# zyddnys/manga-image-translator

Measured on AMD Instinct MI355X. Metric: pages/sec end-to-end (detect+OCR+inpaint), 2048x1456, higher is better.
Workload: dtype f32

## Files before the change

include/mit_hip.h:

```cpp
#ifndef MIT_HIP_H
#define MIT_HIP_H

#include <stdint.h>

#ifdef __cplusplus
extern "C" {
#endif

#define MIT_ABI_VERSION 20
#define MIT_MAX_TAPS 64

enum MitAct {
    MIT_ACT_NONE = 0,
    MIT_ACT_RELU = 1,
    MIT_ACT_LEAKY = 2,
    MIT_ACT_SILU = 3,
    MIT_ACT_SIGMOID = 4,
    MIT_ACT_GELU = 5
};
#define MIT_ACT_POST_FIRST 0x100

enum MitPad {
    MIT_PAD_ZERO = 0,
    MIT_PAD_REFLECT = 1
};

typedef struct MitTensorMap {
    float *base;
    int64_t zs1, zs0, bs, ys, xs;
    int64_t nhi;
    int32_t nsplit;
    int32_t _pad;
} MitTensorMap;

typedef struct MitConvGemm {
    const float *a;
    int64_t a_zs1, a_zs0, a_bs, a_ys, a_xs;
    int32_t NB, Hi, Wi, Cin;
    int32_t Ho, Wo, sy, sx;
    int32_t ntaps, pad_mode;
    int8_t tap_dy[MIT_MAX_TAPS];
    int8_t tap_dx[MIT_MAX_TAPS];
    int32_t tap_off[MIT_MAX_TAPS];
    const float *w;
    int64_t w_zs1, w_zs0, ldw;
    int32_t Kw, Nw;
    int32_t N;
    int32_t Z, zdiv;
    MitTensorMap c, pre, post;
    const float *scale, *bias;
    int32_t act;
    float act_alpha;
    const uint16_t *w_split;
    int64_t ws_zs0;
    const int32_t *lut_rows;
    const float *lut1, *lut2;
    int64_t lut_ld;
    int32_t nprod;
    int32_t _pad1;
} MitConvGemm;

const char *mit_last_error(void);
int mit_abi_version(void);
const char *mit_source_digest(void);

int mit_device_count(int *count);
int mit_device_name(int device, char *buf, int buflen);

int mit_conv_gemm(const MitConvGemm *desc, void *stream);
int mit_conv_gemm_cfg(const MitConvGemm *desc, int cfg, void *stream);
const char *mit_conv_gemm_config_name(int cfg);
int mit_conv_gemm_plan(const MitConvGemm *desc, int cfg, int32_t *tile, int32_t *nb_run);
const char *mit_conv_gemm_config_kernel(int cfg);

int mit_gemm_split_pack(const float *w_dev, int64_t w_zs, int nz, int Kw, int64_t ldw, uint16_t *out_dev, void *stream);
int mit_gemm_mode_set(int mode);
int mit_gemm_mode_get(void);
int64_t mit_gemm_split_min_tiles(int64_t n);

typedef struct MitPGemm {
    const uint16_t *a_planes;
    int64_t a_zs;
    int64_t lda;
    const uint16_t *w_planes;
    int64_t w_zs;
    int64_t ldw;
    int32_t M, N, K, Z;
    float *c;
    int64_t ldc, c_zs;
    const float *pre;
    int64_t ld_pre, pre_zs;
    const float *post;
    int64_t ld_post, post_zs;
    uint16_t *c_planes;
    int64_t ld_cp, cp_zs;
    const float *scale, *bias;
    int32_t act;
    float act_alpha;
    int32_t nprod;
    int32_t tile;
} MitPGemm;
int mit_pgemm(const MitPGemm *desc, void *stream);
const char *mit_pgemm_tile_name(int tile);
int mit_pgemm_supported(const MitPGemm *desc);
int mit_split_planes(const float *x_dev, int64_t ldx, int R, int K, uint16_t *planes_dev, int64_t ld, void *stream);
int mit_join_planes(const uint16_t *planes_dev, int64_t ld, int R, int K, float *x_dev, int64_t ldx, void *stream);

int mit_conv_small_cout(const float *in_dev, int64_t in_pixstride, int64_t in_planestride, const float *w4_dev, const float *w_pairs_dev, const float *bias_dev, float *out_dev,
                        int64_t out_pixstride, int B, int H, int W, int Cin, int Cout, int k, int pad_mode, int act,
                        float act_alpha, void *stream);

int mit_convnext_mlp_supported(int C);
int mit_convnext_mlp(const float *x_dev, int64_t ldx, int M, int C, const uint16_t *w1_planes_dev, const float *b1_dev,
                     const uint16_t *w2perm_planes_dev, int64_t ldn2, const float *scale2_dev, const float *bias2_dev,
                     const float *post_dev, int64_t ldp, float *out_dev, int64_t ldo, void *stream);

int mit_wino43_input(const float *x_dev, int64_t x_bs, int64_t x_ys, int64_t x_xs, float *v_dev, int B, int H, int W, int C,
                     int pad_mode, void *stream);
int mit_wino43_output(const float *m_dev, float *y_dev, int64_t y_bs, int64_t y_ys, int64_t y_xs, const float *post_dev,
                      int64_t p_bs, int64_t p_ys, int64_t p_xs, const float *scale_dev, const float *bias_dev, int B, int H,
                      int W, int N, int act, float alpha, void *stream);

typedef struct MitProfStat {
    int64_t launches;
    double ms, exec_flops, alg_flops;
} MitProfStat;
int mit_prof_enable(int on);
int mit_prof_tag_next(double alg_flops);
int mit_prof_read(MitProfStat *stats, int max_cfgs, int *n_cfgs);
int mit_prof_dump(const char *path);
typedef struct MitProfKernelStat {
    char name[48];
    int64_t launches;
    double ms, alg_bytes, alg_flops;
} MitProfKernelStat;
int mit_prof_kernels_read(MitProfKernelStat *stats, int max_stats, int *n_stats);

int mit_resize_u8(const uint8_t *src_dev, int B, int H, int W, int C, uint8_t *dst_dev, int dh, int dw, int mode, const int *yidx_dev,
                  const uint16_t *ycoef_dev, const int *xidx_dev, const uint16_t *xcoef_dev, void *stream);
int mit_resample_pil_u8(const uint8_t *src_dev, int B, int H, int W, int C, uint8_t *dst_dev, int n_out, int axis, const int *bounds_dev,
                        const int *coef_dev, int ksize, void *stream);
int mit_bilateral_u8c3(const uint8_t *src_dev, uint8_t *dst_dev, int B, int H, int W, int radius, int ntaps, const int *tap_ofs_dev,
                       const float *tap_w_dev, const float *color_w_dev, void *stream);
int mit_select_u8(const uint8_t *mask_dev, int thr, const uint8_t *a_dev, const uint8_t *b_dev, uint8_t *out_dev, int64_t npix, int C,
                  void *stream);

typedef struct MitRefineWindow {
    int x1, y1, x2, y2;
} MitRefineWindow;
typedef struct MitRefineCand {
    int kind;
    int lo, hi;
    int invert;
} MitRefineCand;
int64_t mit_ctd_refine_workspace_bytes(const MitRefineWindow *windows, int n);
int mit_ctd_refine_hist(const uint8_t *page_dev, const uint8_t *pred_dev, int H, int W, const MitRefineWindow *windows, int n, int *hist_host,
                        void *workspace_dev, int64_t workspace_bytes, void *stream);
int mit_ctd_refine_scores(const uint8_t *page_dev, const uint8_t *pred_dev, int H, int W, const MitRefineWindow *windows, int n,
                          const MitRefineCand *cands_host, uint64_t *sums_host, void *workspace_dev, int64_t workspace_bytes, void *stream);
int mit_ctd_refine_merge(const uint8_t *page_dev, const uint8_t *pred_dev, int H, int W, const MitRefineWindow *windows, int n,
                         const MitRefineCand *order_host, uint8_t *out_dev, void *workspace_dev, int64_t workspace_bytes, void *stream);


typedef struct MitCrfCrop {
    int x, y, w, h;
} MitCrfCrop;

typedef struct MitDilateJob {
    int32_t sx, sy, sw, sh;
    int32_t dx, dy, dw, dh;
    int32_t k, spitch;
    int64_t src_off;
} MitDilateJob;
int mit_mask_dilate_jobs(const uint8_t *src_dev, const MitDilateJob *jobs_host, int n_jobs, uint8_t *dst_dev, int H, int W, int merge,
                         MitDilateJob *jobs_dev, void *stream);
int mit_binarize_u8(uint8_t *buf_dev, int64_t n, void *stream);

int64_t mit_densecrf_workspace_bytes(const MitCrfCrop *crops, int n_crops);
int mit_densecrf_refine(const uint8_t *page_dev, int H, int W, const MitCrfCrop *crops, int n_crops, const uint8_t *mask_dev,
                        uint8_t *out_dev, float *q_dev, float sxy_gauss, float w_gauss, float sxy_bilateral, float srgb_bilateral,
                        float w_bilateral, int iterations, const float *unary_lut_dev, void *workspace_dev, int64_t workspace_bytes,
                        void *stream);


int mit_fft_cols(const float *in_dev, int64_t in_bs, int64_t in_ts, int64_t in_hs, float *out_dev, int64_t out_bs,
                 int64_t out_ts, int64_t out_hs, const float *twiddle_dev, int B, int h, int64_t ncols, int inverse, float scale,
                 void *stream);

int mit_rfft_rows_supported(int w);
int mit_rfft_rows(const float *in_dev, int64_t in_bs, int64_t in_hs, int64_t in_ws, float *out_dev, int64_t out_bs, int64_t out_ts,
                  int64_t out_hs, int64_t out_ks, const float *tables_dev, int B, int h, int w, int C, float scale, void *stream);
int mit_irfft_rows(const float *in_dev, int64_t in_bs, int64_t in_ts, int64_t in_hs, int64_t in_ks, float *out_dev, int64_t out_bs,
                   int64_t out_hs, int64_t out_ws, const float *res_dev, int64_t res_bs, int64_t res_hs, int64_t res_ws,
// ... 244 lines not shown
```

manga_image_translator_amd/csrc/conv_gemm.hip:

```cpp
#include "conv_gemm_table.h"
#include <atomic>

using namespace mitcg;

namespace {

int64_t max_a_offset(const MitConvGemm &p) {
    if (p.a_bs < 0 || p.a_ys < 0 || p.a_xs < 0) return -1;
    int tmax = 0;
    for (int t = 0; t < p.ntaps; ++t) {
        if (p.tap_off[t] < 0) return -1;
        if (p.tap_off[t] > tmax) tmax = p.tap_off[t];
    }
    return (int64_t)(p.NB - 1) * p.a_bs + (int64_t)(p.Hi - 1) * p.a_ys + (int64_t)(p.Wi - 1) * p.a_xs + p.Cin + tmax;
}
bool fast_eligible(const MitConvGemm &p, int BK) {
    if (p.Cin % BK || p.ntaps > FAST_MAX_TAPS) return false;
    const int64_t maxoff = max_a_offset(p);
    return maxoff >= 0 && maxoff < 0x7fffffffLL;
}

bool split_eligible(const MitConvGemm &p, int BK) {
    if (!p.w_split || (reinterpret_cast<uintptr_t>(p.w_split) & 15) || (p.ws_zs0 & 7)) return false;
    if (p.w_zs1 != 0 || (p.Kw & 7) || p.ntaps * p.Cin > p.Kw) return false;
// ... 94 lines not shown
}

extern "C" int mit_prof_enable(int on) {
    std::lock_guard<std::mutex> lk(g_probe_mu);
    for (auto &r : g_probe) {
        (void)hipEventDestroy(r.start);
        (void)hipEventDestroy(r.stop);
    }
    g_probe.clear();
    g_probe_on = on != 0;
    mit_probe_reset(on != 0);
    return 0;
}

extern "C" int mit_prof_tag_next(double alg_flops) {
    g_next_alg_flops = alg_flops;
    return 0;
}

extern "C" int mit_prof_dump(const char *path) {
    if (!path) return mit_set_error("mit_prof_dump: null path");
    std::lock_guard<std::mutex> lk(g_probe_mu);
    FILE *f = fopen(path, "w");
    if (!f) return mit_set_error("mit_prof_dump: cannot open %s", path);
    fprintf(f, "tile,M,N,K,taps,Z,act,ms,exec_flops,alg_flops\n");
    for (auto &r : g_probe) {
        float ms = 0.f;
        if (hipEventSynchronize(r.stop) != hipSuccess || hipEventElapsedTime(&ms, r.start, r.stop) != hipSuccess) {
            fclose(f);
            return mit_set_error("mit_prof_dump: event query failed");
        }
        fprintf(f, "%s,%d,%d,%d,%d,%d,%d,%.6f,%.0f,%.0f\n", kCfgs[r.cfg].name, r.M, r.N, r.K, r.ntaps, r.Z, r.act, ms, r.exec_flops,
                r.alg_flops);
    }
    fclose(f);
    return 0;
}

extern "C" int mit_prof_read(MitProfStat *stats, int max_cfgs, int *n_cfgs) {
    if (!stats || !n_cfgs) return mit_set_error("mit_prof_read: null");
    std::lock_guard<std::mutex> lk(g_probe_mu);
    const int n = max_cfgs < kNumCfgs ? max_cfgs : kNumCfgs;
    for (int i = 0; i < n; ++i) {
        stats[i].launches = 0;
        stats[i].ms = stats[i].exec_flops = stats[i].alg_flops = 0.0;
    }
    for (auto &r : g_probe) {
        MIT_CHECK_HIP(hipEventSynchronize(r.stop));
        float ms = 0.f;
        MIT_CHECK_HIP(hipEventElapsedTime(&ms, r.start, r.stop));
        if (r.cfg < n) {
            stats[r.cfg].launches += 1;
            stats[r.cfg].ms += ms;
            stats[r.cfg].exec_flops += r.exec_flops;
            stats[r.cfg].alg_flops += r.alg_flops;
        }
    }
    *n_cfgs = n;
    return 0;
}

extern "C" const char *mit_conv_gemm_config_name(int cfg) {
    if (cfg < 0 || cfg >= kNumCfgs) return nullptr;
    return kCfgs[cfg].name;
}

extern "C" const char *mit_conv_gemm_config_kernel(int cfg) {
    if (cfg < 0 || cfg >= kNumCfgs) return nullptr;
    return kCfgs[cfg].kernel;
}

namespace {
bool map_vec_ok(const MitTensorMap &m, bool split_ok = false) {
    if (m.nsplit != 0 && !(split_ok && !(m.nsplit & 3) && !(m.nhi & 3))) return false;
    return !(reinterpret_cast<uintptr_t>(m.base) & 15) && !((m.zs1 | m.zs0 | m.bs | m.ys | m.xs) & 3);
}
bool vec_epilogue_ok(const MitConvGemm &p) {
    if ((p.N & 3) || !map_vec_ok(p.c, true)) return false;
    if (p.pre.base && !map_vec_ok(p.pre)) return false;
    if (p.post.base && !map_vec_ok(p.post)) return false;
    if (p.lut_rows && ((p.lut_ld & 3) || (reinterpret_cast<uintptr_t>(p.lut1) & 15) || (reinterpret_cast<uintptr_t>(p.lut2) & 15))) return false;
    return !(reinterpret_cast<uintptr_t>(p.scale) & 15) && !(reinterpret_cast<uintptr_t>(p.bias) & 15);
}

int validate(const MitConvGemm *d, MitConvGemm &p) {
    if (!d) return mit_set_error("mit_conv_gemm: null descriptor");
    p = *d;
    if (p.act & MIT_ACT_VEC_OK) return mit_set_error("mit_conv_gemm: reserved activation bits set");
    if (vec_epilogue_ok(p)) p.act |= MIT_ACT_VEC_OK;
    if (!p.a || !p.w || !p.c.base) return mit_set_error("mit_conv_gemm: null operand");
    if (p.Cin <= 0 || (p.Cin & 3)) return mit_set_error("mit_conv_gemm: Cin must be a positive multiple of 4 (got %d)", p.Cin);
    if ((p.ldw & 3) || (p.Nw & 3)) return mit_set_error("mit_conv_gemm: ldw/Nw must be multiples of 4 (ldw=%lld Nw=%d)", (long long)p.ldw, p.Nw);
    if (p.ntaps <= 0 || p.ntaps > MIT_MAX_TAPS) return mit_set_error("mit_conv_gemm: ntaps %d out of range", p.ntaps);
    if (p.NB <= 0 || p.Ho <= 0 || p.Wo <= 0 || p.N <= 0 || p.Z <= 0 || p.zdiv <= 0)
        return mit_set_error("mit_conv_gemm: empty problem");
    if ((reinterpret_cast<uintptr_t>(p.a) & 15) || (reinterpret_cast<uintptr_t>(p.w) & 15))
        return mit_set_error("mit_conv_gemm: operands must be 16-byte aligned");
    if ((p.a_xs & 3) || (p.a_ys & 3) || (p.a_bs & 3) || (p.a_zs0 & 3) || (p.a_zs1 & 3) || (p.w_zs0 & 3) || (p.w_zs1 & 3))
        return mit_set_error("mit_conv_gemm: strides must be multiples of 4 elements");
    for (int t = 0; t < p.ntaps; ++t)
        if (p.tap_off[t] & 3) return mit_set_error("mit_conv_gemm: tap_off must be multiples of 4");
    if (p.pad_mode == MIT_PAD_REFLECT) {
        for (int t = 0; t < p.ntaps; ++t) {
            int ady = p.tap_dy[t] < 0 ? -p.tap_dy[t] : p.tap_dy[t];
            int adx = p.tap_dx[t] < 0 ? -p.tap_dx[t] : p.tap_dx[t];
            if (ady >= p.Hi || adx >= p.Wi) return mit_set_error("mit_conv_gemm: reflect pad larger than input");
        }
    }
    if ((int64_t)p.NB * p.Ho * p.Wo > 0x7fffffffLL) return mit_set_error("mit_conv_gemm: M too large");
    if (p.lut_rows) {
        if (!p.lut1 || !p.lut2 || p.lut_ld < p.N) return mit_set_error("mit_conv_gemm: lut_rows needs lut1, lut2 and lut_ld >= N");
        if (p.Z != 1) return mit_set_error("mit_conv_gemm: the row-lookup epilogue is for Z == 1 launches");
        if (p.lut_ld > 0x7fff) return mit_set_error("mit_conv_gemm: lut_ld too large (row offsets are 16-bit row x lut_ld in 32 bits)");
    }
    if (p.Z > 65535) return mit_set_error("mit_conv_gemm: Z too large");
    if (p.nprod != 0 && p.nprod != 1) return mit_set_error("mit_conv_gemm: nprod must be 0 (the GEMM mode) or 1 (one bf16 product) (got %d)", p.nprod);
    if (p.nprod == 1 && !p.w_split) return mit_set_error("mit_conv_gemm: nprod = 1 needs w_split (mit_gemm_split_pack): there is no fp32 fallback for a requested precision");
    return 0;
}

int images_per_run(const MitConvGemm &p) {
    if (p.Z != 1 || p.NB <= 1) return p.NB;
    MitConvGemm q = p;
    q.NB = 1;
    const bool want_buf = (gemm_mode_now() == 6 || p.nprod == 1) && p.w_split != nullptr && split_eligible(p, 16) && buf_eligible(q);
    auto run_ok = [&](const MitConvGemm &r) { return fast_eligible(r, 16) && (!want_buf || buf_eligible(r)); };
    if (p.Cin % 16 != 0 || p.ntaps > FAST_MAX_TAPS || p.a_bs <= 0 || run_ok(p) || !fast_eligible(q, 16)) return p.NB;
    int nb = p.NB;
    while (nb > 1) {
        q.NB = nb;
        if (run_ok(q)) break;
        nb = (nb + 1) / 2;
    }
    return nb;
}
MitConvGemm run_of(const MitConvGemm &p, int b0, int nb) {
    MitConvGemm r = p;
    r.NB = nb;
    r.a += (int64_t)b0 * p.a_bs;
    r.c.base += (int64_t)b0 * p.c.bs;
    if (p.pre.base) r.pre.base += (int64_t)b0 * p.pre.bs;
    if (p.post.base) r.post.base += (int64_t)b0 * p.post.bs;
    if (p.lut_rows) r.lut_rows += (int64_t)b0 * p.Ho * p.Wo;
    return r;
}

int plan_run(const MitConvGemm &p, int cfg, int *tile) {
    const int64_t M = (int64_t)p.NB * p.Ho * p.Wo;
    if (p.nprod == 1) {
        if (!split_eligible(p, 16))
            return mit_set_error("mit_conv_gemm: nprod = 1 needs the split tiles' preconditions (Cin %% 16 == 0, <= %d taps, 32-bit element offsets, 16-byte aligned w_split with w_zs1 == 0 and Kw %% 8 == 0): there is no fp32 fallback for a requested precision", FAST_MAX_TAPS);
        if (cfg >= 0 && cfg < kNumCfgs && kCfgs[cfg].nprod() != 1) return mit_set_error("mit_conv_gemm: nprod = 1 with tile %s, which is not a one-product tile", kCfgs[cfg].name);
    }
    if (cfg < 0) cfg = pick_cfg(p, M);
    if (cfg >= kNumCfgs) return mit_set_error("mit_conv_gemm: bad cfg %d", cfg);
    const CfgEntry &c = kCfgs[cfg];
    const bool fast = c.family == TileFamily::fast, split = c.family == TileFamily::split, gemv = c.family == TileFamily::gemv;
    if (p.lut_rows) {
        if (!fast && !split)
            return mit_set_error("mit_conv_gemm: the row-lookup epilogue (lut_rows) needs a fast or split tile (Cin %% 16 == 0, <= %d taps); this launch takes %s", FAST_MAX_TAPS, c.name);
        if (!(p.act & MIT_ACT_VEC_OK)) return mit_set_error("mit_conv_gemm: lut_rows needs the float4 epilogue (N %% 4 == 0, 16-byte aligned maps, tables and lut_ld %% 4 == 0)");
        if (p.post.base) return mit_set_error("mit_conv_gemm: lut_rows together with a post residual is not implemented");
        if ((p.act & 0xff) != MIT_ACT_NONE && (p.act & 0xff) != MIT_ACT_RELU) return mit_set_error("mit_conv_gemm: lut_rows is implemented for act none / relu");
    }
    if (gemv && (!gemv_eligible(p, c.lanes_per_row()) || p.N > c.BN))
        return mit_set_error("mit_conv_gemm: cfg %s needs N <= %d, Z == 1, unsplit maps and Cin %% %d == 0", c.name, c.BN, 4 * c.lanes_per_row());
    if (split && !split_eligible(p, c.BK))
        return mit_set_error("mit_conv_gemm: cfg %s needs w_split (mit_gemm_split_pack, 16-byte aligned, w_zs1 == 0, Kw %% 8 == 0) and the fast tiles' preconditions", c.name);
    if (fast && !fast_eligible(p, c.BK))
        return mit_set_error("mit_conv_gemm: cfg %s needs Cin %% %d == 0, <= %d taps and 32-bit element offsets", c.name, c.BK, FAST_MAX_TAPS);
    if ((M + c.BM - 1) / c.BM * ((p.N + c.BN - 1) / c.BN) > 0x7fffffffLL) return mit_set_error("mit_conv_gemm: grid too large");
    *tile = cfg;
    return 0;
}

int launch_run(const MitConvGemm &p, int cfg, hipStream_t hs) {
    const CfgEntry &c = kCfgs[cfg];
    const int M = p.NB * p.Ho * p.Wo;
    const int MT = (M + c.BM - 1) / c.BM;
    const int NT = (p.N + c.BN - 1) / c.BN;
    const int Ktot = p.ntaps * p.Cin;
    const int KT = (Ktot + c.BK - 1) / c.BK;
    const double tagged = g_next_alg_flops;
    g_next_alg_flops = -1.0;
    if (g_probe_on) {
        std::lock_guard<std::mutex> lk(g_probe_mu);
        ProbeRec r;
        MIT_CHECK_HIP(hipEventCreate(&r.start));
        MIT_CHECK_HIP(hipEventCreate(&r.stop));
        r.cfg = cfg;
        r.exec_flops = 2.0 * (double)M * p.N * Ktot * p.Z;
        r.alg_flops = tagged >= 0.0 ? tagged : r.exec_flops;
        r.M = M, r.N = p.N, r.K = Ktot, r.ntaps = p.ntaps, r.Z = p.Z, r.act = p.act;
        MIT_CHECK_HIP(hipEventRecord(r.start, hs));
        c.launch(p, M, MT, NT, KT, hs);
        MIT_CHECK_HIP(hipEventRecord(r.stop, hs));
        g_probe.push_back(r);
    } else {
        c.launch(p, M, MT, NT, KT, hs);
    }
    hipError_t e = hipGetLastError();
    if (e != hipSuccess) return mit_set_error("mit_conv_gemm: launch failed: %s", hipGetErrorString(e));
    return 0;
}
}

extern "C" int mit_conv_gemm_plan(const MitConvGemm *d, int cfg, int32_t *tile, int32_t *nb_run) {
    if (!tile || !nb_run) return mit_set_error("mit_conv_gemm_plan: null output");
    MitConvGemm p;
    if (int rc = validate(d, p)) return rc;
    if (cfg < 0)
        for (int pass = 0; pass < 2; ++pass) {
            const int nb = images_per_run(p);
            if (nb < p.NB) p = run_of(p, 0, nb);
        }
    int t = -1;
    if (int rc = plan_run(p, cfg, &t)) return rc;
    *tile = t, *nb_run = p.NB;
    return 0;
}

extern "C" int mit_conv_gemm_cfg(const MitConvGemm *d, int cfg, void *stream) {
    MitConvGemm p;
    if (int rc = validate(d, p)) return rc;
    hipStream_t hs = reinterpret_cast<hipStream_t>(stream);
    int tile = -1;
    const int nb1 = cfg < 0 ? images_per_run(p) : p.NB;
    if (nb1 == p.NB) {
        if (int rc = plan_run(p, cfg, &tile)) return rc;
        return launch_run(p, tile, hs);
    }
    for (int b1 = 0; b1 < p.NB; b1 += nb1) {
        const MitConvGemm r1 = run_of(p, b1, p.NB - b1 < nb1 ? p.NB - b1 : nb1);
        const int nb2 = images_per_run(r1);
        for (int b2 = 0; b2 < r1.NB; b2 += nb2) {
            const MitConvGemm r2 = run_of(r1, b2, r1.NB - b2 < nb2 ? r1.NB - b2 : nb2);
            g_next_alg_flops = -1.0;
            if (int rc = plan_run(r2, -1, &tile)) return rc;
            if (int rc = launch_run(r2, tile, hs)) return rc;
        }
    }
    return 0;
}

extern "C" int mit_conv_gemm(const MitConvGemm *d, void *stream) { return mit_conv_gemm_cfg(d, -1, stream); }

extern "C" int mit_gemm_mode_set(int mode) {
    if (mode != 0 && mode != 6 && mode != 9) return mit_set_error("mit_gemm_mode_set: mode must be 0, 6 or 9 (got %d)", mode);
    g_gemm_mode.store(mode, std::memory_order_relaxed);
    return 0;
}

extern "C" int mit_gemm_mode_get(void) { return gemm_mode_now(); }

extern "C" int64_t mit_gemm_split_min_tiles(int64_t n) {
    const int64_t prev = split_min_now();
    if (n >= 0) g_split_min.store(n, std::memory_order_relaxed);
    return prev;
}

extern "C" int mit_gemm_split_pack(const float *w_dev, int64_t w_zs, int nz, int Kw, int64_t ldw, uint16_t *out_dev, void *stream) {
    if (!w_dev || !out_dev) return mit_set_error("mit_gemm_split_pack: null pointer");
    if (nz <= 0 || Kw <= 0 || (Kw & 7) || ldw <= 0 || (ldw & 3) || ldw > 0x7fffffffLL)
        return mit_set_error("mit_gemm_split_pack: need nz > 0, Kw %% 8 == 0, ldw %% 4 == 0 (nz=%d Kw=%d ldw=%lld)", nz, Kw, (long long)ldw);
    if ((reinterpret_cast<uintptr_t>(out_dev) & 15)) return mit_set_error("mit_gemm_split_pack: output must be 16-byte aligned");
    const int64_t total = (int64_t)nz * (Kw >> 3) * ldw;
    hipLaunchKernelGGL(gemm_split_pack_kernel, dim3((unsigned)((total + 255) / 256)), dim3(256), 0, reinterpret_cast<hipStream_t>(stream),
                       w_dev, w_zs, Kw >> 3, (int)ldw, out_dev, total);
    hipError_t e = hipGetLastError();
    if (e != hipSuccess) return mit_set_error("mit_gemm_split_pack: launch failed: %s", hipGetErrorString(e));
    return 0;
}
```

manga_image_translator_amd/csrc/conv_gemm_kernels.h:

```cpp
#pragma once

#include <hip/hip_runtime.h>
#include <stdint.h>
#include <stdio.h>
#include <stdlib.h>
#include <mutex>
#include <type_traits>
#include <vector>
#include "../../include/mit_hip.h"
#include "common.h"

typedef float f32x16 __attribute__((ext_vector_type(16)));
typedef float f32x4 __attribute__((ext_vector_type(4)));
namespace mitcg {

struct RowOff {
    int64_t c, pre, post;
};
struct LutOff {
    int32_t t1, t2;
};

__device__ __forceinline__ float gelu_fast(float v) {
    const float x = v * 0.70710678118654752440f;
    const float ax = fabsf(x);
    const float t = __builtin_amdgcn_rcpf(__builtin_fmaf(0.3275911f, ax, 1.f));
    float q = 1.061405429f;
    q = __builtin_fmaf(q, t, -1.453152027f);
    q = __builtin_fmaf(q, t, 1.421413741f);
    q = __builtin_fmaf(q, t, -0.284496736f);
    q = __builtin_fmaf(q, t, 0.254829592f);
    q *= t;
    const float e = __builtin_amdgcn_exp2f(ax * ax * -1.44269504088896340736f);
    const float erf_abs = 1.f - q * e;
    const float hx = 0.5f * v;
    return hx + hx * copysignf(erf_abs, x);
}

template <int ACT>
__device__ __forceinline__ float apply_act(float v, float alpha) {
    if (ACT == MIT_ACT_RELU) return v > 0.f ? v : 0.f;
    if (ACT == MIT_ACT_LEAKY) return v > 0.f ? v : v * alpha;
    if (ACT == MIT_ACT_SILU) return v / (1.f + expf(-v));
    if (ACT == MIT_ACT_SIGMOID) return 1.f / (1.f + expf(-v));
    if (ACT == MIT_ACT_GELU) return gelu_fast(v);
    return v;
}

template <int TM, int TN, int ACT, bool HAS_POST>
__device__ __forceinline__ void epilogue_store(const MitConvGemm &p, f32x16 (&acc)[TM][TN], const RowOff *rowoff, const int n0,
                                               const int wm0, const int wn0, const int tid) {
    const int lane = tid & 63;
    const int li = lane & 31;
    const int lh = lane >> 5;
    const bool has_pre = p.pre.base != nullptr;
    const bool post_first = (p.act & MIT_ACT_POST_FIRST) != 0;
#pragma unroll
    for (int ni = 0; ni < TN; ++ni) {
        const int n = n0 + wn0 + ni * 32 + li;
        if (n >= p.N) continue;
        const float sc = p.scale ? p.scale[n] : 1.f;
        const float bi = p.bias ? p.bias[n] : 0.f;
        int64_t ncol_c = n, ncol_pre = n, ncol_post = n;
        if (p.c.nsplit) ncol_c = (int64_t)(n / p.c.nsplit) * p.c.nhi + (n % p.c.nsplit);
        if (has_pre && p.pre.nsplit) ncol_pre = (int64_t)(n / p.pre.nsplit) * p.pre.nhi + (n % p.pre.nsplit);
        if (HAS_POST && p.post.nsplit) ncol_post = (int64_t)(n / p.post.nsplit) * p.post.nhi + (n % p.post.nsplit);
#pragma unroll
        for (int mi = 0; mi < TM; ++mi) {
#pragma unroll
            for (int r = 0; r < 16; ++r) {
                const int row = wm0 + mi * 32 + (r & 3) + 8 * (r >> 2) + 4 * lh;
                const RowOff ro = rowoff[row];
                if (ro.c < 0) continue;
                float v = acc[mi][ni][r];
                if (has_pre) v += p.pre.base[ro.pre + ncol_pre];
                v = v * sc + bi;
                if (HAS_POST && post_first) v += p.post.base[ro.post + ncol_post];
                v = apply_act<ACT>(v, p.act_alpha);
                if (HAS_POST && !post_first) v += p.post.base[ro.post + ncol_post];
                p.c.base[ro.c + ncol_c] = v;
            }
        }
    }
}

constexpr int EPI_PITCH = 36;
#define MIT_ACT_VEC_OK 0x200

template <int TM, int TN, int ACT, bool HAS_POST, bool HAS_LUT = false>
__device__ __forceinline__ void epilogue_store_vec(const MitConvGemm &p, f32x16 (&acc)[TM][TN], const RowOff *rowoff, float *tbuf,
                                                   const int n0, const int wm0, const int wn0, const int tid, const LutOff *lutoff = nullptr) {
    const int lane = tid & 63;
    const int li = lane & 31;
    const int lh = lane >> 5;
    const int vr = lane >> 3, vc = (lane & 7) * 4;
    const bool has_pre = p.pre.base != nullptr;
    const bool post_first = (p.act & MIT_ACT_POST_FIRST) != 0;
#pragma unroll
    for (int ni = 0; ni < TN; ++ni) {
        const int n = n0 + wn0 + ni * 32 + vc;
        const bool n_ok = n < p.N;
        const int64_t nc = p.c.nsplit ? (int64_t)(n / p.c.nsplit) * p.c.nhi + (n % p.c.nsplit) : (int64_t)n;
        f32x4 sc = {1.f, 1.f, 1.f, 1.f}, bi = {0.f, 0.f, 0.f, 0.f};
        if (n_ok && p.scale) sc = *reinterpret_cast<const f32x4 *>(p.scale + n);
        if (n_ok && p.bias) bi = *reinterpret_cast<const f32x4 *>(p.bias + n);
#pragma unroll
        for (int mi = 0; mi < TM; ++mi) {
#pragma unroll
            for (int r = 0; r < 16; ++r) tbuf[((r & 3) + 8 * (r >> 2) + 4 * lh) * EPI_PITCH + li] = acc[mi][ni][r];
            asm volatile("s_waitcnt lgkmcnt(0)" ::: "memory");
#pragma unroll
            for (int j = 0; j < 4; ++j) {
                const int rl = vr + 8 * j;
                f32x4 v = *reinterpret_cast<const f32x4 *>(tbuf + rl * EPI_PITCH + vc);
                const RowOff ro = rowoff[wm0 + mi * 32 + rl];
                if (ro.c < 0 || !n_ok) continue;
                if (has_pre) v += *reinterpret_cast<const f32x4 *>(p.pre.base + ro.pre + n);
                v = v * sc + bi;
                f32x4 pv = {0.f, 0.f, 0.f, 0.f};
                if (HAS_POST) pv = *reinterpret_cast<const f32x4 *>(p.post.base + ro.post + n);
                if (HAS_POST && post_first) v += pv;
                v.x = apply_act<ACT>(v.x, p.act_alpha);
                v.y = apply_act<ACT>(v.y, p.act_alpha);
                v.z = apply_act<ACT>(v.z, p.act_alpha);
                v.w = apply_act<ACT>(v.w, p.act_alpha);
                if (HAS_POST && !post_first) v += pv;
                if (HAS_LUT) {
                    const LutOff lo = lutoff[wm0 + mi * 32 + rl];
                    v += *reinterpret_cast<const f32x4 *>(p.lut1 + lo.t1 + n);
                    v += *reinterpret_cast<const f32x4 *>(p.lut2 + lo.t2 + n);
                }
                *reinterpret_cast<f32x4 *>(p.c.base + ro.c + nc) = v;
            }
            asm volatile("" ::: "memory");
        }
    }
}

template <int BM, int TM, int TN, int SMEM_FLOATS = 0, int NTHR = 256>
__device__ __forceinline__ void epilogue(const MitConvGemm &p, f32x16 (&acc)[TM][TN], float *smem, const int M, const int m0,
                                         const int n0, const int wm0, const int wn0, const int z1, const int z0,
                                         const int HoWo, const int tid) {
    RowOff *rowoff = reinterpret_cast<RowOff *>(smem);
    for (int r = tid; r < BM; r += NTHR) {
        const int m = m0 + r;
        RowOff ro = {-1, 0, 0};
        if (m < M) {
            const int nb = m / HoWo;
            const int rem = m - nb * HoWo;
            const int oy = rem / p.Wo;
            const int ox = rem - oy * p.Wo;
            ro.c = z1 * p.c.zs1 + z0 * p.c.zs0 + (int64_t)nb * p.c.bs + (int64_t)oy * p.c.ys + (int64_t)ox * p.c.xs;
            ro.pre = z1 * p.pre.zs1 + z0 * p.pre.zs0 + (int64_t)nb * p.pre.bs + (int64_t)oy * p.pre.ys +
                     (int64_t)ox * p.pre.xs;
            ro.post = z1 * p.post.zs1 + z0 * p.post.zs0 + (int64_t)nb * p.post.bs + (int64_t)oy * p.post.ys +
                      (int64_t)ox * p.post.xs;
        }
        rowoff[r] = ro;
    }
    constexpr int ROWOFF_FLOATS = (BM * (int)sizeof(RowOff) + 15) / 16 * 4;
    constexpr int LUT_FLOATS = BM * (int)sizeof(LutOff) / 4;
    constexpr int NWAVES = NTHR / 64;
    constexpr bool VEC_FITS = SMEM_FLOATS >= ROWOFF_FLOATS + NWAVES * 32 * EPI_PITCH + LUT_FLOATS;
    LutOff *lutoff = reinterpret_cast<LutOff *>(smem + ROWOFF_FLOATS + NWAVES * 32 * EPI_PITCH);
    const bool lut = VEC_FITS && p.lut_rows != nullptr;
    if (VEC_FITS && lut) {
        for (int r = tid; r < BM; r += NTHR) {
            const int m = m0 + r;
            const unsigned int packed = m < M ? (unsigned int)p.lut_rows[m] : 0u;
            lutoff[r] = LutOff{(int32_t)((packed & 0xffffu) * (unsigned int)p.lut_ld), (int32_t)((packed >> 16) * (unsigned int)p.lut_ld)};
        }
    }
    __syncthreads();

    const bool has_post = p.post.base != nullptr;
    float *tbuf = smem + ROWOFF_FLOATS + (tid >> 6) * (32 * EPI_PITCH);
    const bool vec = VEC_FITS && (p.act & MIT_ACT_VEC_OK);
    if (VEC_FITS && vec && lut) {
        if ((p.act & 0xff) == MIT_ACT_RELU) epilogue_store_vec<TM, TN, MIT_ACT_RELU, false, true>(p, acc, rowoff, tbuf, n0, wm0, wn0, tid, lutoff);
        else epilogue_store_vec<TM, TN, MIT_ACT_NONE, false, true>(p, acc, rowoff, tbuf, n0, wm0, wn0, tid, lutoff);
        return;
    }
#define MIT_EPI(A)                                                                                   \
    if (VEC_FITS && vec) {                                                                           \
        if (has_post) epilogue_store_vec<TM, TN, A, true>(p, acc, rowoff, tbuf, n0, wm0, wn0, tid); \
        else epilogue_store_vec<TM, TN, A, false>(p, acc, rowoff, tbuf, n0, wm0, wn0, tid);         \
    } else if (has_post) epilogue_store<TM, TN, A, true>(p, acc, rowoff, n0, wm0, wn0, tid);      \
    else epilogue_store<TM, TN, A, false>(p, acc, rowoff, n0, wm0, wn0, tid)
    switch (p.act & 0xff) {
        case MIT_ACT_RELU: MIT_EPI(MIT_ACT_RELU); break;
        case MIT_ACT_LEAKY: MIT_EPI(MIT_ACT_LEAKY); break;
        case MIT_ACT_SILU: MIT_EPI(MIT_ACT_SILU); break;
        case MIT_ACT_SIGMOID: MIT_EPI(MIT_ACT_SIGMOID); break;
        case MIT_ACT_GELU: MIT_EPI(MIT_ACT_GELU); break;
        default: MIT_EPI(MIT_ACT_NONE); break;
    }
#undef MIT_EPI
}

template <int BM, int BN, int BK, int WAVES_M, int WAVES_N>
__global__ __launch_bounds__(256) void conv_gemm_kernel(const MitConvGemm p, const int M, const int MT,
                                                          const int NT, const int KT) {
    constexpr int WM = BM / WAVES_M;
    constexpr int WN = BN / WAVES_N;
    constexpr int TM = WM / 32;
    constexpr int TN = WN / 32;
    static_assert(WAVES_M * WAVES_N == 4, "4 waves");
    static_assert(TM >= 1 && TN >= 1, "wave tile");
    constexpr int KQ = BK / 4;
    constexpr int A_ITERS = BM * KQ / 256;
    constexpr int A_MSTEP = 256 / KQ;
    constexpr int NQ = BN / 4;
    constexpr int B_ITERS = (BK * NQ + 255) / 256;
    constexpr int B_KSTEP = 256 / NQ;
    constexpr bool B_PARTIAL = (BK * NQ) < 256;
    static_assert(A_ITERS >= 1 && (BM * KQ) % 256 == 0, "A tile must fill the workgroup");
    constexpr int LDA = BM + (BK == 16 ? 2 : 1);
    constexpr int LDB = BN + 4;
    constexpr int A_TILE = BK * LDA;
    constexpr int B_TILE = BK * LDB;

    extern __shared__ __attribute__((aligned(16))) float smem[];
    float *As = smem;
    float *Bs = smem + 2 * A_TILE;
    int *tapinfo = reinterpret_cast<int *>(smem + 2 * A_TILE + 2 * B_TILE);

    const int tid = threadIdx.x;
    const int lane = tid & 63;
    const int wave = tid >> 6;
    const int li = lane & 31;
    const int lh = lane >> 5;

    const int nwg = MT * NT;
    int bid = blockIdx.x;
    {
        const int xcd = bid & 7, q = nwg >> 3, r = nwg & 7;
        bid = (xcd < r ? xcd * (q + 1) : r * (q + 1) + (xcd - r) * q) + (bid >> 3);
    }
    const int mt = bid / NT, nt = bid - mt * NT;
    const int m0 = mt * BM, n0 = nt * BN;
    const int z = blockIdx.y;
    const int z1 = z / p.zdiv, z0 = z - z1 * p.zdiv;

    const float *__restrict__ a_base = p.a + z1 * p.a_zs1 + z0 * p.a_zs0;
    const float *__restrict__ w_base = p.w + z1 * p.w_zs1 + z0 * p.w_zs0;

    for (int t = tid; t < p.ntaps; t += 256) {
        tapinfo[2 * t] = (int(p.tap_dy[t]) & 0xffff) | (int(p.tap_dx[t]) << 16);
        tapinfo[2 * t + 1] = p.tap_off[t];
    }

    const int aq = tid % KQ;
    const int am = tid / KQ;
    int64_t a_rowbase[A_ITERS];
    int a_iy0[A_ITERS], a_ix0[A_ITERS];
    const int HoWo = p.Ho * p.Wo;
#pragma unroll
    for (int i = 0; i < A_ITERS; ++i) {
        const int m = m0 + am + i * A_MSTEP;
        if (m < M) {
            const int nb = m / HoWo;
            const int rem = m - nb * HoWo;
            const int oy = rem / p.Wo;
            const int ox = rem - oy * p.Wo;
            a_rowbase[i] = (int64_t)nb * p.a_bs;
            a_iy0[i] = oy * p.sy;
            a_ix0[i] = ox * p.sx;
        } else {
            a_rowbase[i] = 0;
            a_iy0[i] = -(1 << 28);
            a_ix0[i] = 0;
        }
    }
    const int bn4 = tid % NQ;
    const int bk = tid / NQ;
    const bool b_ncol_ok = (n0 + bn4 * 4) < p.Nw;

    const int Ktot = p.ntaps * p.Cin;

    f32x4 a_reg[A_ITERS];
    f32x4 b_reg[B_ITERS];

    __syncthreads();

    auto load_tile = [&](int kt) {
        const int kk = kt * BK + aq * 4;
        const bool kvalid = kk < Ktot;
        int tap = 0, ci = 0, dy = 0, dx = 0, toff = 0;
        if (kvalid) {
            tap = kk / p.Cin;
            ci = kk - tap * p.Cin;
            const int packed = tapinfo[2 * tap];
            dy = (int)(short)(packed & 0xffff);
            dx = packed >> 16;
            toff = tapinfo[2 * tap + 1];
        }
#pragma unroll
        for (int i = 0; i < A_ITERS; ++i) {
            int iy = a_iy0[i] + dy;
            int ix = a_ix0[i] + dx;
            bool ok = kvalid && (a_iy0[i] >= 0);
            if (p.pad_mode == MIT_PAD_REFLECT) {
                iy = iy < 0 ? -iy : (iy >= p.Hi ? 2 * p.Hi - 2 - iy : iy);
                ix = ix < 0 ? -ix : (ix >= p.Wi ? 2 * p.Wi - 2 - ix : ix);
            } else {
                ok = ok && iy >= 0 && iy < p.Hi && ix >= 0 && ix < p.Wi;
            }
            f32x4 v = {0.f, 0.f, 0.f, 0.f};
            if (ok) {
                const float *ptr = a_base + a_rowbase[i] + (int64_t)iy * p.a_ys + (int64_t)ix * p.a_xs + toff + ci;
                v = *reinterpret_cast<const f32x4 *>(ptr);
            }
            a_reg[i] = v;
        }
#pragma unroll
        for (int i = 0; i < B_ITERS; ++i) {
            const int k = kt * BK + bk + i * B_KSTEP;
            f32x4 v = {0.f, 0.f, 0.f, 0.f};
            if (b_ncol_ok && k < p.Kw && (!B_PARTIAL || bk < BK)) {
                const float *ptr = w_base + (int64_t)k * p.ldw + n0 + bn4 * 4;
                v = *reinterpret_cast<const f32x4 *>(ptr);
            }
            b_reg[i] = v;
        }
    };

    auto store_tile = [&](int buf) {
        float *as = As + buf * A_TILE;
#pragma unroll
        for (int i = 0; i < A_ITERS; ++i) {
            const int ml = am + i * A_MSTEP;
#pragma unroll
            for (int j = 0; j < 4; ++j) as[(aq * 4 + j) * LDA + ml] = a_reg[i][j];
        }
        float *bs = Bs + buf * B_TILE;
#pragma unroll
        for (int i = 0; i < B_ITERS; ++i) {
            const int kl = bk + i * B_KSTEP;
            if (!B_PARTIAL || bk < BK) *reinterpret_cast<f32x4 *>(bs + kl * LDB + bn4 * 4) = b_reg[i];
        }
    };

    f32x16 acc[TM][TN];
#pragma unroll
    for (int mi = 0; mi < TM; ++mi)
#pragma unroll
        for (int ni = 0; ni < TN; ++ni)
#pragma unroll
            for (int r = 0; r < 16; ++r) acc[mi][ni][r] = 0.f;

    const int wm0 = (wave / WAVES_N) * WM;
    const int wn0 = (wave % WAVES_N) * WN;

    load_tile(0);
    store_tile(0);
    __syncthreads();

    for (int kt = 0; kt < KT; ++kt) {
        const int cur = kt & 1;
        if (kt + 1 < KT) load_tile(kt + 1);
        const float *as = As + cur * A_TILE + lh * LDA + wm0 + li;
        const float *bs = Bs + cur * B_TILE + lh * LDB + wn0 + li;
#pragma unroll
        for (int ks = 0; ks < BK / 2; ++ks) {
            float af[TM], bf[TN];
#pragma unroll
            for (int mi = 0; mi < TM; ++mi) af[mi] = as[(2 * ks) * LDA + mi * 32];
#pragma unroll
            for (int ni = 0; ni < TN; ++ni) bf[ni] = bs[(2 * ks) * LDB + ni * 32];
#pragma unroll
            for (int mi = 0; mi < TM; ++mi)
#pragma unroll
                for (int ni = 0; ni < TN; ++ni)
                    acc[mi][ni] = __builtin_amdgcn_mfma_f32_32x32x2f32(af[mi], bf[ni], acc[mi][ni], 0, 0, 0);
        }
        if (kt + 1 < KT) store_tile(cur ^ 1);
        __syncthreads();
    }

    epilogue<BM, TM, TN, 2 * A_TILE + 2 * B_TILE>(p, acc, smem, M, m0, n0, wm0, wn0, z1, z0, HoWo, (int)threadIdx.x);
}

constexpr int FAST_MAX_TAPS = 16;

template <int BM, int BN, int BK, int WAVES_M, int WAVES_N, int MINW, int VAR>
__global__ __launch_bounds__(256, MINW) void conv_gemm_fast_kernel(const MitConvGemm p, const int M, const int MT,
                                                               const int NT, const int KT) {
    constexpr int WM = BM / WAVES_M;
    constexpr int WN = BN / WAVES_N;
    constexpr int TM = WM / 32;
    constexpr int TN = WN / 32;
    static_assert(WAVES_M * WAVES_N == 4, "4 waves");
    static_assert(TM >= 1 && TN >= 1, "wave tile");
    static_assert(VAR == 4, "schedule");
    constexpr int KQ = BK / 4;
    constexpr int A_ITERS = BM * KQ / 256;
    constexpr int A_MSTEP = 256 / KQ;
    constexpr int NQ = BN / 4;
    constexpr int B_ITERS = (BK * NQ + 255) / 256;
    constexpr int B_KSTEP = 256 / NQ;
    constexpr bool B_PARTIAL = (BK * NQ) < 256;
    static_assert(A_ITERS >= 1 && (BM * KQ) % 256 == 0, "A tile must fill the workgroup");
    static_assert(B_PARTIAL || (BK * NQ) % 256 == 0, "B tile must fill the workgroup or fit in one pass");
    constexpr int LDA = BM + (BK == 16 ? 2 : 1);
    constexpr int LDB = BN + 4;
    constexpr int A_TILE = BK * LDA;
    constexpr int B_TILE = BK * LDB;

    extern __shared__ __attribute__((aligned(16))) float smem[];
    float *As = smem;
    float *Bs = smem + 2 * A_TILE;
    int *rowtab = reinterpret_cast<int *>(smem + 2 * A_TILE + 2 * B_TILE);

    const int tid = threadIdx.x;
    const int lane = tid & 63;
    const int wave = tid >> 6;
    const int li = lane & 31;
    const int lh = lane >> 5;

    const int nwg = MT * NT;
    int bid = blockIdx.x;
    {
        const int xcd = bid & 7, q = nwg >> 3, r = nwg & 7;
        bid = (xcd < r ? xcd * (q + 1) : r * (q + 1) + (xcd - r) * q) + (bid >> 3);
    }
    const int mt = bid / NT, nt = bid - mt * NT;
    const int m0 = mt * BM, n0 = nt * BN;
    const int z = blockIdx.y;
    const int z1 = z / p.zdiv, z0 = z - z1 * p.zdiv;
    const int HoWo = p.Ho * p.Wo;

    const float *__restrict__ a_base = p.a + z1 * p.a_zs1 + z0 * p.a_zs0;
    const float *__restrict__ w_base = p.w + z1 * p.w_zs1 + z0 * p.w_zs0;

    for (int idx = tid; idx < p.ntaps * BM; idx += 256) {
        const int t = idx / BM, r = idx - t * BM;
        const int m = m0 + r;
        int off = -1;
        if (m < M) {
            const int nb = m / HoWo;
            const int rem = m - nb * HoWo;
            const int oy = rem / p.Wo;
            const int ox = rem - oy * p.Wo;
            int iy = oy * p.sy + p.tap_dy[t];
            int ix = ox * p.sx + p.tap_dx[t];
            bool ok = true;
            if (p.pad_mode == MIT_PAD_REFLECT) {
                iy = iy < 0 ? -iy : (iy >= p.Hi ? 2 * p.Hi - 2 - iy : iy);
                ix = ix < 0 ? -ix : (ix >= p.Wi ? 2 * p.Wi - 2 - ix : ix);
            } else {
                ok = iy >= 0 && iy < p.Hi && ix >= 0 && ix < p.Wi;
            }
            if (ok) off = (int)((int64_t)nb * p.a_bs + (int64_t)iy * p.a_ys + (int64_t)ix * p.a_xs + p.tap_off[t]);
        }
        rowtab[idx] = off;
    }

    const int aq = tid % KQ;
    const int am = tid / KQ;
    const int bn4 = tid % NQ;
    const int bk = tid / NQ;
    const bool b_ncol_ok = (n0 + bn4 * 4) < p.Nw && (!B_PARTIAL || bk < BK);
    const float *__restrict__ a_thr = a_base + aq * 4;
    const float *__restrict__ w_thr = w_base + n0 + bn4 * 4;

    f32x4 a_reg[A_ITERS];
    f32x4 b_reg[B_ITERS];

    __syncthreads();

    int ld_tap = 0, ld_ci0 = 0;
    int a_off[A_ITERS];
    const float *__restrict__ w_row = w_thr + (int64_t)bk * p.ldw;
    const int64_t w_kstep = (int64_t)B_KSTEP * p.ldw, w_tstep = (int64_t)BK * p.ldw;
    auto load_tile = [&](int kt) {
        const int *rt = rowtab + ld_tap * BM + am;
        const float *ak = a_thr + ld_ci0;
        if (ld_ci0 == 0) {
#pragma unroll
            for (int i = 0; i < A_ITERS; ++i) a_off[i] = rt[i * A_MSTEP];
        }
#pragma unroll
        for (int i = 0; i < A_ITERS; ++i) {
            const int off = a_off[i];
            f32x4 v = {0.f, 0.f, 0.f, 0.f};
            if (off >= 0) v = *reinterpret_cast<const f32x4 *>(ak + off);
            a_reg[i] = v;
        }
#pragma unroll
        for (int i = 0; i < B_ITERS; ++i) {
            const int k = kt * BK + bk + i * B_KSTEP;
            f32x4 v = {0.f, 0.f, 0.f, 0.f};
            if (b_ncol_ok && k < p.Kw) v = *reinterpret_cast<const f32x4 *>(w_row + i * w_kstep);
            b_reg[i] = v;
        }
        w_row += w_tstep;
        ld_ci0 += BK;
        if (ld_ci0 >= p.Cin) {
            ld_ci0 = 0;
            ++ld_tap;
        }
    };

    auto store_tile = [&](int buf) {
        float *as = As + buf * A_TILE;
#pragma unroll
        for (int i = 0; i < A_ITERS; ++i) {
            const int ml = am + i * A_MSTEP;
#pragma unroll
            for (int j = 0; j < 4; ++j) as[(aq * 4 + j) * LDA + ml] = a_reg[i][j];
        }
        float *bs = Bs + buf * B_TILE;
#pragma unroll
        for (int i = 0; i < B_ITERS; ++i) {
            const int kl = bk + i * B_KSTEP;
            if (!B_PARTIAL || bk < BK) *reinterpret_cast<f32x4 *>(bs + kl * LDB + bn4 * 4) = b_reg[i];
        }
    };

    f32x16 acc[TM][TN];
#pragma unroll
    for (int mi = 0; mi < TM; ++mi)
#pragma unroll
        for (int ni = 0; ni < TN; ++ni)
#pragma unroll
            for (int r = 0; r < 16; ++r) acc[mi][ni][r] = 0.f;
// ... 166 lines not shown
```

manga_image_translator_amd/csrc/conv_gemm_split.h:

```cpp
#pragma once
#include "bf16_split.h"

namespace mitcg {


template <int BK>
__device__ __forceinline__ constexpr int split_swz(int kh) { return kh * (64 / BK); }

template <int BM, int BN, int BK, int WAVES_M, int WAVES_N, int MINW, int NPROD, int VAR>
__global__ __launch_bounds__(256, MINW) void conv_gemm_split_kernel(const MitConvGemm p, const int M, const int MT, const int NT,
                                                                  const int KT) {
    constexpr int WM = BM / WAVES_M;
    constexpr int WN = BN / WAVES_N;
    constexpr int TM = WM / 32;
    constexpr int TN = WN / 32;
    static_assert(WAVES_M * WAVES_N == 4 && TM >= 1 && TN >= 1, "wave tile");
    static_assert(BK == 16 || BK == 32, "K-tile of one or two bf16 MFMA steps");
    static_assert(NPROD == 1 || NPROD == 3 || NPROD == 6 || NPROD == 9, "plane pairs");
    constexpr int NPL = NPROD == 1 ? 1 : 3;
    constexpr int KH = BK / 8;
    constexpr int KS = BK / 16;
    constexpr int KQ = BK / 4;
    constexpr int A_ITERS = BM * KQ / 256;
    constexpr int A_MSTEP = 256 / KQ;
    static_assert(A_ITERS >= 1 && (BM * KQ) % 256 == 0, "A tile must fill the workgroup");
    constexpr bool PIPE = (VAR & 1) != 0;
    static_assert(PIPE == ((VAR & 128) != 0), "the pipelined schedule is the stepped one (VAR 1 + 128)");
    constexpr bool ORD = (VAR & 256) != 0;
    constexpr bool BUF = (VAR & 2048) != 0;
    static_assert((VAR & ~(1 | 128 | 256 | 2048)) == 0, "VAR bits");
    constexpr int SA = BM, SB = BN;
    constexpr int A_TILE = NPL * KH * SA, B_TILE = NPL * KH * SB;
    constexpr int B_CPP = KH * BN;
    constexpr int B_CELLS = NPL * B_CPP;
    constexpr int B_ITERS = (B_CELLS + 255) / 256;

    extern __shared__ __attribute__((aligned(16))) float smem[];
    u32x4 *As = reinterpret_cast<u32x4 *>(smem);
    u32x4 *Bs = As + 2 * A_TILE;
    int *rowtab = reinterpret_cast<int *>(Bs + 2 * B_TILE);

    const int tid = threadIdx.x;
    const int lane = tid & 63;
    const int wave = __builtin_amdgcn_readfirstlane(tid >> 6);
    const int li = lane & 31;
    const int lh = lane >> 5;

    const int nwg = MT * NT;
    int cur_tile;
    {
        const int v = blockIdx.x, xcd = v & 7, q = nwg >> 3, r = nwg & 7;
        cur_tile = (xcd < r ? xcd * (q + 1) : r * (q + 1) + (xcd - r) * q) + (v >> 3);
    }
    int m0 = 0, n0 = 0;
    const int z = blockIdx.y;
    const int z1 = z / p.zdiv, z0 = z - z1 * p.zdiv;
    const int HoWo = p.Ho * p.Wo;

    const float *__restrict__ a_base = p.a + z1 * p.a_zs1 + z0 * p.a_zs0;
    const u32x4 *__restrict__ ws = reinterpret_cast<const u32x4 *>(p.w_split + z0 * p.ws_zs0);
    const int K8 = p.Kw >> 3;
    const int ldn = (int)p.ldw;

    const int aq = tid % KQ;
    const int am = tid / KQ;
    const float *__restrict__ a_thr = a_base + aq * 4;
    const __amdgpu_buffer_rsrc_t ra = __builtin_amdgcn_make_buffer_rsrc(const_cast<float *>(a_base), 0, 0x80000000u, 0x00020000);
    const __amdgpu_buffer_rsrc_t rw = __builtin_amdgcn_make_buffer_rsrc(const_cast<u32x4 *>(ws), 0, 0x80000000u, 0x00020000);
    const int aq16 = aq * 16;
    constexpr bool B_UNI = B_CPP == 256;
    constexpr int B_IDX = B_UNI ? 1 : B_ITERS;
    int b_src[B_IDX], b_dst[B_IDX];
    bool b_ok[B_IDX];
    auto bsrc = [&](const int i) { return B_UNI ? b_src[0] + i * K8 * ldn : b_src[B_UNI ? 0 : i]; };
    auto bdst = [&](const int i) { return B_UNI ? b_dst[0] + i * KH * SB : b_dst[B_UNI ? 0 : i]; };
    auto bok = [&](const int i) { return b_ok[B_UNI ? 0 : i]; };
    int ld_tap = 0, ld_ci0 = 0, ld_k8 = 0;
    auto setup_tile = [&](const int t) {
        const int mt = t / NT, nt = t - mt * NT;
        m0 = mt * BM;
        n0 = nt * BN;
        for (int idx = tid; idx < p.ntaps * BM; idx += 256) {
            const int tp = idx / BM, r = idx - tp * BM;
            const int m = m0 + r;
            int off = -1;
            if (m < M) {
                const int nb = m / HoWo;
                const int rem = m - nb * HoWo;
                const int oy = rem / p.Wo;
                const int ox = rem - oy * p.Wo;
                int iy = oy * p.sy + p.tap_dy[tp];
                int ix = ox * p.sx + p.tap_dx[tp];
                bool ok = true;
                if (p.pad_mode == MIT_PAD_REFLECT) {
                    iy = iy < 0 ? -iy : (iy >= p.Hi ? 2 * p.Hi - 2 - iy : iy);
                    ix = ix < 0 ? -ix : (ix >= p.Wi ? 2 * p.Wi - 2 - ix : ix);
                } else {
                    ok = iy >= 0 && iy < p.Hi && ix >= 0 && ix < p.Wi;
                }
                if (ok) off = (int)((int64_t)nb * p.a_bs + (int64_t)iy * p.a_ys + (int64_t)ix * p.a_xs + p.tap_off[tp]);
            }
            rowtab[idx] = BUF ? (off < 0 ? (int)0x80000000u : off * 4) : off;
        }
#pragma unroll
        for (int i = 0; i < B_IDX; ++i) {
            const int c = tid + i * 256;
            const int pl = c / B_CPP, rem = c - pl * B_CPP;
            const int kh = rem / BN, n = rem - kh * BN;
            b_ok[i] = c < B_CELLS && (n0 + n) < ldn;
            b_src[i] = (pl * K8 + kh) * ldn + n0 + n;
            b_dst[i] = (pl * KH + kh) * SB + n;
        }
        ld_tap = ld_ci0 = ld_k8 = 0;
    };
    setup_tile(cur_tile);

    f32x4 a_reg[A_ITERS];
    u32x4 b_reg[B_ITERS];
    int a_off[A_ITERS];

    __syncthreads();

    auto load_tile = [&]() {
        const int *rt = rowtab + ld_tap * BM + am;
#pragma unroll
        for (int i = 0; i < A_ITERS; ++i) a_off[i] = rt[i * A_MSTEP];
        const float *ak = a_thr + ld_ci0;
#pragma unroll
        for (int i = 0; i < A_ITERS; ++i) {
            if (BUF) a_reg[i] = __builtin_bit_cast(f32x4, __builtin_amdgcn_raw_buffer_load_b128(ra, a_off[i] + aq16, ld_ci0 * 4, 0));
            else a_reg[i] = *reinterpret_cast<const f32x4 *>(ak + (a_off[i] < 0 ? 0 : a_off[i]));
        }
        const u32x4 *wk = ws + (int64_t)ld_k8 * ldn;
#pragma unroll
        for (int i = 0; i < B_ITERS; ++i) {
            if (BUF) b_reg[i] = __builtin_amdgcn_raw_buffer_load_b128(rw, bok(i) ? bsrc(i) * 16 : -1, ld_k8 * ldn * 16, 0);
            else b_reg[i] = wk[bok(i) ? bsrc(i) : 0];
        }
        ld_k8 += KH;
        ld_ci0 += BK;
        const bool wrap = ld_ci0 >= p.Cin;
        ld_ci0 = wrap ? 0 : ld_ci0;
        ld_tap += wrap ? 1 : 0;
    };
    auto store_tile = [&](int buf) {
        u32x2 *as2 = reinterpret_cast<u32x2 *>(As + buf * A_TILE);
        const int kh = aq >> 1, half = aq & 1;
#pragma unroll
        for (int i = 0; i < A_ITERS; ++i) {
            const int ml = (am + i * A_MSTEP) ^ split_swz<BK>(kh);
            u32x2 h, m, l;
            const f32x4 zero = {0.f, 0.f, 0.f, 0.f};
            const f32x4 v = !BUF && a_off[i] < 0 ? zero : a_reg[i];
            if (NPL == 1) {
                as2[(kh * SA + ml) * 2 + half] = u32x2{pack_bf16(v.x, v.y), pack_bf16(v.z, v.w)};
                continue;
            }
            split3(v, h, m, l);
            as2[((0 * KH + kh) * SA + ml) * 2 + half] = h;
            as2[((1 * KH + kh) * SA + ml) * 2 + half] = m;
            as2[((2 * KH + kh) * SA + ml) * 2 + half] = l;
        }
        u32x4 *bs = Bs + buf * B_TILE;
#pragma unroll
        for (int i = 0; i < B_ITERS; ++i)
            if ((i + 1) * 256 <= B_CELLS || tid + i * 256 < B_CELLS) bs[bdst(i)] = b_reg[i];
    };

    f32x16 acc[TM][TN];

    const int wm0 = (wave / WAVES_N) * WM;
    const int wn0 = (wave % WAVES_N) * WN;

// ... 174 lines not shown
```

manga_image_translator_amd/csrc/conv_small_cout.hip:

```cpp

#include <hip/hip_runtime.h>
#include <stdint.h>
#include <stdlib.h>
#include "../../include/mit_hip.h"
#include "common.h"

typedef float f32x4 __attribute__((ext_vector_type(4)));

namespace {

constexpr int TW = 32, TH = 8, CCH = 16;

__device__ __forceinline__ float act_fn(float v, int act, float alpha) {
    switch (act) {
        case MIT_ACT_RELU: return v > 0.f ? v : 0.f;
        case MIT_ACT_LEAKY: return v > 0.f ? v : v * alpha;
        case MIT_ACT_SIGMOID: return 1.f / (1.f + expf(-v));
        default: return v;
    }
}

template <int K>
__global__ __launch_bounds__(256) void conv_small_cout_kernel(const float *__restrict__ in, int64_t in_pix, const f32x4 *__restrict__ w4,
                                                               const float *__restrict__ bias, float *__restrict__ out,
                                                               int64_t out_pix, int H, int W, int Cin, int Cout, int reflect,
                                                               int act, float alpha) {
    constexpr int R = K / 2;
    constexpr int HW_ = TW + 2 * R, HH_ = TH + 2 * R;
    __shared__ f32x4 tile[CCH / 4][HH_][HW_];
    const int tx = threadIdx.x & (TW - 1), ty = threadIdx.x / TW;
    const int x0 = blockIdx.x * TW, y0 = blockIdx.y * TH, b = blockIdx.z;
    const float *ib = in + (int64_t)b * H * W * in_pix;
    f32x4 acc = {0.f, 0.f, 0.f, 0.f};
    for (int c0 = 0; c0 < Cin; c0 += CCH) {
        __syncthreads();
        for (int i = threadIdx.x; i < (CCH / 4) * HH_ * HW_; i += 256) {
            const int q = i % (CCH / 4);
            const int p = i / (CCH / 4);
            const int px = p % HW_, py = p / HW_;
            int yy = y0 + py - R, xx = x0 + px - R;
            bool ok = true;
            if (reflect) {
                yy = yy < 0 ? -yy : (yy >= H ? 2 * H - 2 - yy : yy);
                xx = xx < 0 ? -xx : (xx >= W ? 2 * W - 2 - xx : xx);
                ok = yy >= 0 && yy < H && xx >= 0 && xx < W;
            } else {
                ok = yy >= 0 && yy < H && xx >= 0 && xx < W;
            }
            f32x4 v = {0.f, 0.f, 0.f, 0.f};
            if (ok) v = *reinterpret_cast<const f32x4 *>(ib + ((int64_t)yy * W + xx) * in_pix + c0 + q * 4);
            tile[q][py][px] = v;
        }
        __syncthreads();
#pragma unroll 1
        for (int ky = 0; ky < K; ++ky) {
#pragma unroll
            for (int kx = 0; kx < K; ++kx) {
                const f32x4 *wt = w4 + (int64_t)(ky * K + kx) * Cin + c0;
#pragma unroll
                for (int q = 0; q < CCH / 4; ++q) {
                    const f32x4 v = tile[q][ty + ky][tx + kx];
#pragma unroll
                    for (int e = 0; e < 4; ++e) {
                        const f32x4 ww = wt[q * 4 + e];
                        acc.x = fmaf(v[e], ww.x, acc.x);
                        acc.y = fmaf(v[e], ww.y, acc.y);
                        acc.z = fmaf(v[e], ww.z, acc.z);
                        acc.w = fmaf(v[e], ww.w, acc.w);
                    }
                }
            }
        }
    }
    const int x = x0 + tx, y = y0 + ty;
    if (x < W && y < H) {
        float *o = out + (((int64_t)b * H + y) * W + x) * out_pix;
        for (int n = 0; n < Cout; ++n) o[n] = act_fn(acc[n] + (bias ? bias[n] : 0.f), act, alpha);
    }
}

typedef float f32x2 __attribute__((ext_vector_type(2)));

constexpr int TW3 = 64, TH3 = 16;

template <int K>
__global__ __launch_bounds__(256) void conv_small_cout3_kernel(const float *__restrict__ in, int64_t in_pix, int64_t in_plane ,
                                                                const f32x2 *__restrict__ wq ,
                                                                const float *__restrict__ bias, float *__restrict__ out,
                                                                int64_t out_pix, int H, int W, int Cin, int Cout, int reflect,
                                                                int act, float alpha) {
    constexpr int R = K / 2;
    constexpr int TR = TH3 + 2 * R;
    constexpr int HW_ = TW3 + 2 * R;
    constexpr int HALF = HW_ / 2;
    __shared__ f32x4 tile[TR][HW_];
    const int tx = threadIdx.x & 31, ty = threadIdx.x >> 5;
    const int x0 = blockIdx.x * TW3, y0 = blockIdx.y * TH3, b = blockIdx.z;
    const float *ib = in + (int64_t)b * H * W * in_pix;
    f32x2 acc[2][2][3];
#pragma unroll
    for (int r = 0; r < 2; ++r)
#pragma unroll
        for (int j = 0; j < 2; ++j)
#pragma unroll
            for (int n = 0; n < 3; ++n) acc[r][j][n] = f32x2{0.f, 0.f};
    constexpr int ITEMS = (TR * HW_ + 255) / 256;
    for (int g0 = 0; g0 < Cin; g0 += 16) {
        f32x4 rg[ITEMS][4];
#pragma unroll
        for (int it = 0; it < ITEMS; ++it) {
            const int i = threadIdx.x + it * 256;
            const int ly = i / HW_, lx = i - ly * HW_;
            int yy = y0 + ly - R, xx = x0 + lx - R;
            if (reflect) {
                yy = yy < 0 ? -yy : (yy >= H ? 2 * H - 2 - yy : yy);
                xx = xx < 0 ? -xx : (xx >= W ? 2 * W - 2 - xx : xx);
            }
            const bool ok = i < TR * HW_ && xx >= 0 && xx < W && yy >= 0 && yy < H;
            const float *pa = ib + ((int64_t)yy * W + xx) * in_pix + (in_plane ? (int64_t)(g0 >> 4) * in_plane : (int64_t)g0);
#pragma unroll
            for (int q = 0; q < 4; ++q) {
                rg[it][q] = f32x4{0.f, 0.f, 0.f, 0.f};
                if (ok) rg[it][q] = *reinterpret_cast<const f32x4 *>(pa + q * 4);
            }
        }
#pragma unroll
        for (int q = 0; q < 4; ++q) {
            const int s4 = (g0 >> 2) + q;
            __syncthreads();
#pragma unroll
            for (int it = 0; it < ITEMS; ++it) {
                const int i = threadIdx.x + it * 256;
                if (i < TR * HW_) {
                    const int ly = i / HW_, lx = i - ly * HW_;
                    tile[ly][(lx >> 1) + (lx & 1) * HALF] = rg[it][q];
                }
            }
            __syncthreads();
#pragma unroll 1
            for (int ky = 0; ky < K; ++ky) {
                f32x4 win[2][K + 1];
#pragma unroll
                for (int r = 0; r < 2; ++r)
#pragma unroll
                    for (int i = 0; i <= K; ++i) win[r][i] = tile[ty + r * (TH3 / 2) + ky][tx + (i >> 1) + (i & 1) * HALF];
#pragma unroll
                for (int kx = 0; kx < K; ++kx) {
                    const f32x2 *wt = wq + ((int64_t)(ky * K + kx) * (Cin >> 2) + s4) * 8;
                    const f32x2 w00 = wt[0], w01 = wt[1], w10 = wt[2], w11 = wt[3], w20 = wt[4], w21 = wt[5];
#pragma unroll
                    for (int r = 0; r < 2; ++r)
#pragma unroll
                        for (int j = 0; j < 2; ++j) {
                            const f32x4 v = win[r][kx + j];
                            const f32x2 lo = {v.x, v.y}, hi = {v.z, v.w};
                            acc[r][j][0] = __builtin_elementwise_fma(lo, w00, acc[r][j][0]);
                            acc[r][j][1] = __builtin_elementwise_fma(lo, w10, acc[r][j][1]);
                            acc[r][j][2] = __builtin_elementwise_fma(lo, w20, acc[r][j][2]);
                            acc[r][j][0] = __builtin_elementwise_fma(hi, w01, acc[r][j][0]);
                            acc[r][j][1] = __builtin_elementwise_fma(hi, w11, acc[r][j][1]);
                            acc[r][j][2] = __builtin_elementwise_fma(hi, w21, acc[r][j][2]);
                        }
                }
            }
        }
    }
#pragma unroll
    for (int j = 0; j < 2; ++j) {
        const int x = x0 + 2 * tx + j;
#pragma unroll
        for (int r = 0; r < 2; ++r) {
            const int y = y0 + ty + r * (TH3 / 2);
            if (x < W && y < H) {
                float *o = out + (((int64_t)b * H + y) * W + x) * out_pix;
                for (int n = 0; n < Cout; ++n) o[n] = act_fn((acc[r][j][n].x + acc[r][j][n].y) + (bias ? bias[n] : 0.f), act, alpha);
            }
        }
    }
}

typedef __attribute__((address_space(3))) void lds_void_t;
typedef __attribute__((address_space(1))) const void gbl_cvoid_t;

template <int K>
__global__ __launch_bounds__(256, 4) void conv_small_cout3_dma_kernel(const float *__restrict__ in, int64_t in_plane ,
                                                                      const f32x2 *__restrict__ wq, const float *__restrict__ bias, float *__restrict__ out,
                                                                      int64_t out_pix, int H, int W, int Cin, int Cout, int act, float alpha, int parity_major) {
    constexpr int R = K / 2;
    constexpr int TR = TH3 + 2 * R, HW_ = TW3 + 2 * R, HALF = HW_ / 2;
    constexpr int CELLS = TR * HW_, PIECES = (CELLS + 63) / 64, PPW = (PIECES + 3) / 4, BUF_CELLS = PPW * 4 * 64;
    __shared__ f32x4 tile[BUF_CELLS];
    const int tx = threadIdx.x & 31, ty = threadIdx.x >> 5;
    const int lane = threadIdx.x & 63, wave = __builtin_amdgcn_readfirstlane(threadIdx.x >> 6);
    const int x0 = blockIdx.x * TW3, y0 = blockIdx.y * TH3, b = blockIdx.z;
    int src_off[PPW];
#pragma unroll
    for (int j = 0; j < PPW; ++j) {
        int c = (wave * PPW + j) * 64 + lane;
        c = c < CELLS ? c : CELLS - 1;
        const int ly = c / HW_, slot = c - ly * HW_;
        const int lx = slot < HALF ? 2 * slot : 2 * (slot - HALF) + 1;
        int yy = y0 + ly - R, xx = x0 + lx - R;
        yy = yy < 0 ? -yy : (yy >= H ? 2 * H - 2 - yy : yy);
        xx = xx < 0 ? -xx : (xx >= W ? 2 * W - 2 - xx : xx);
        yy = yy < 0 ? 0 : (yy >= H ? H - 1 : yy);
        xx = xx < 0 ? 0 : (xx >= W ? W - 1 : xx);
        src_off[j] = parity_major ? ((((yy & 1) * 2 + (xx & 1)) * (H >> 1) + (yy >> 1)) * (W >> 1) + (xx >> 1)) * 4 : (yy * W + xx) * 4;
    }
    f32x2 acc[2][2][3];
#pragma unroll
    for (int r = 0; r < 2; ++r)
#pragma unroll
        for (int j = 0; j < 2; ++j)
#pragma unroll
            for (int n = 0; n < 3; ++n) acc[r][j][n] = f32x2{0.f, 0.f};
    const float *ib = in + (int64_t)b * H * W * 4;
    for (int s4 = 0; s4 < (Cin >> 2); ++s4) {
        const float *pl = ib + (int64_t)s4 * in_plane;
        __syncthreads();
#pragma unroll
        for (int j = 0; j < PPW; ++j)
            __builtin_amdgcn_global_load_lds((gbl_cvoid_t *)(pl + src_off[j]), (lds_void_t *)(tile + (wave * PPW + j) * 64), 16, 0, 0);
        __syncthreads();
#pragma unroll 1
        for (int ky = 0; ky < K; ++ky) {
            f32x4 win[2][K + 1];
#pragma unroll
            for (int r = 0; r < 2; ++r)
#pragma unroll
                for (int i = 0; i <= K; ++i) win[r][i] = tile[(ty + r * (TH3 / 2) + ky) * HW_ + tx + (i >> 1) + (i & 1) * HALF];
#pragma unroll
            for (int kx = 0; kx < K; ++kx) {
                const f32x2 *wt = wq + ((int64_t)(ky * K + kx) * (Cin >> 2) + s4) * 8;
                const f32x2 w00 = wt[0], w01 = wt[1], w10 = wt[2], w11 = wt[3], w20 = wt[4], w21 = wt[5];
#pragma unroll
                for (int r = 0; r < 2; ++r)
#pragma unroll
                    for (int j = 0; j < 2; ++j) {
                        const f32x4 v = win[r][kx + j];
                        const f32x2 lo = {v.x, v.y}, hi = {v.z, v.w};
                        acc[r][j][0] = __builtin_elementwise_fma(lo, w00, acc[r][j][0]);
                        acc[r][j][1] = __builtin_elementwise_fma(lo, w10, acc[r][j][1]);
                        acc[r][j][2] = __builtin_elementwise_fma(lo, w20, acc[r][j][2]);
                        acc[r][j][0] = __builtin_elementwise_fma(hi, w01, acc[r][j][0]);
                        acc[r][j][1] = __builtin_elementwise_fma(hi, w11, acc[r][j][1]);
                        acc[r][j][2] = __builtin_elementwise_fma(hi, w21, acc[r][j][2]);
                    }
            }
        }
    }
#pragma unroll
    for (int j = 0; j < 2; ++j) {
        const int x = x0 + 2 * tx + j;
#pragma unroll
        for (int r = 0; r < 2; ++r) {
            const int y = y0 + ty + r * (TH3 / 2);
            if (x < W && y < H) {
                float *o = out + (((int64_t)b * H + y) * W + x) * out_pix;
                for (int n = 0; n < Cout; ++n) o[n] = act_fn((acc[r][j][n].x + acc[r][j][n].y) + (bias ? bias[n] : 0.f), act, alpha);
            }
        }
    }
}

}

extern "C" int mit_conv_small_cout(const float *in_dev, int64_t in_pixstride, int64_t in_planestride, const float *w4_dev, const float *w_pairs_dev, const float *bias_dev,
                                   float *out_dev, int64_t out_pixstride, int B, int H, int W, int Cin, int Cout, int k,
                                   int pad_mode, int act, float act_alpha, void *stream) {
    if (!in_dev || !w4_dev || !out_dev) return mit_set_error("mit_conv_small_cout: null pointer");
    if (Cout < 1 || Cout > 4) return mit_set_error("mit_conv_small_cout: 1 <= Cout <= 4 required (got %d)", Cout);
    if (Cin <= 0 || (Cin % CCH)) return mit_set_error("mit_conv_small_cout: Cin must be a multiple of %d (got %d)", CCH, Cin);
    if (B <= 0 || H <= 0 || W <= 0 || B > 65535) return mit_set_error("mit_conv_small_cout: bad size");
    if ((in_pixstride & 3) || (reinterpret_cast<uintptr_t>(in_dev) & 15) || (reinterpret_cast<uintptr_t>(w4_dev) & 15) || (reinterpret_cast<uintptr_t>(w_pairs_dev) & 31))
        return mit_set_error("mit_conv_small_cout: input pixels and weights must be 16-byte aligned");
    if (pad_mode == MIT_PAD_REFLECT && (k / 2 >= H || k / 2 >= W)) return mit_set_error("mit_conv_small_cout: reflect pad larger than input");
    const int parity_major = in_planestride < 0;
    if (parity_major) in_planestride = -in_planestride;
    const bool planes4 = in_planestride != 0 && in_pixstride == 4;
    if (parity_major && (!planes4 || (H & 1) || (W & 1))) return mit_set_error("mit_conv_small_cout: parity-major planes need 4-channel planes of even height and width");
    if (in_planestride && ((in_planestride & 3) || (in_pixstride < 16 && !planes4) || !(Cout <= 3 && w_pairs_dev)))
        return mit_set_error("mit_conv_small_cout: planar input (16- or 4-channel planes) needs the packed kernel (Cout <= 3 with w_pairs), pixel stride 4 or >= 16 and a plane stride %% 4 == 0");
    if (planes4 && (pad_mode != MIT_PAD_REFLECT || (int64_t)H * W * 4 > 0x7fffffffLL))
        return mit_set_error("mit_conv_small_cout: 4-channel planes need reflect padding and H * W * 4 < 2^31");
    dim3 grid(mit_div_up(W, TW), mit_div_up(H, TH), B), block(256);
    hipStream_t s = reinterpret_cast<hipStream_t>(stream);
    const f32x4 *w4 = reinterpret_cast<const f32x4 *>(w4_dev);
    const int refl = pad_mode == MIT_PAD_REFLECT;
    MitProbeScope probe(Cout <= 3 && w_pairs_dev ? (k == 7 ? "conv_small_cout3_kernel<7>" : k == 5 ? "conv_small_cout3_kernel<5>" : "conv_small_cout3_kernel<3>")
                                                                    : (k == 7 ? "conv_small_cout_kernel<7>" : k == 5 ? "conv_small_cout_kernel<5>" : "conv_small_cout_kernel<3>"), s, 4.0 * (double)B * H * W * (Cin + Cout), 2.0 * k * k * (double)Cin * Cout * (double)B * H * W);
    if (Cout <= 3 && w_pairs_dev) {
        dim3 grid3(mit_div_up(W, TW3), mit_div_up(H, TH3), B);
        const f32x2 *wp = reinterpret_cast<const f32x2 *>(w_pairs_dev);
        if (Cin & 3) return mit_set_error("mit_conv_small_cout: Cin %% 4");
        if (planes4) {
            switch (k) {
                case 3: hipLaunchKernelGGL(conv_small_cout3_dma_kernel<3>, grid3, block, 0, s, in_dev, in_planestride, wp, bias_dev, out_dev, out_pixstride, H, W, Cin, Cout, act, act_alpha, parity_major); break;
                case 5: hipLaunchKernelGGL(conv_small_cout3_dma_kernel<5>, grid3, block, 0, s, in_dev, in_planestride, wp, bias_dev, out_dev, out_pixstride, H, W, Cin, Cout, act, act_alpha, parity_major); break;
                case 7: hipLaunchKernelGGL(conv_small_cout3_dma_kernel<7>, grid3, block, 0, s, in_dev, in_planestride, wp, bias_dev, out_dev, out_pixstride, H, W, Cin, Cout, act, act_alpha, parity_major); break;
                default: return mit_set_error("mit_conv_small_cout: k must be 3, 5 or 7 (got %d)", k);
            }
            MIT_CHECK_LAUNCH("mit_conv_small_cout");
            return 0;
        }
        switch (k) {
            case 3: hipLaunchKernelGGL(conv_small_cout3_kernel<3>, grid3, block, 0, s, in_dev, in_pixstride, in_planestride, wp, bias_dev, out_dev, out_pixstride, H, W, Cin, Cout, refl, act, act_alpha); break;
            case 5: hipLaunchKernelGGL(conv_small_cout3_kernel<5>, grid3, block, 0, s, in_dev, in_pixstride, in_planestride, wp, bias_dev, out_dev, out_pixstride, H, W, Cin, Cout, refl, act, act_alpha); break;
            case 7: hipLaunchKernelGGL(conv_small_cout3_kernel<7>, grid3, block, 0, s, in_dev, in_pixstride, in_planestride, wp, bias_dev, out_dev, out_pixstride, H, W, Cin, Cout, refl, act, act_alpha); break;
            default: return mit_set_error("mit_conv_small_cout: k must be 3, 5 or 7 (got %d)", k);
        }
        MIT_CHECK_LAUNCH("mit_conv_small_cout");
        return 0;
    }
    switch (k) {
        case 3: hipLaunchKernelGGL(conv_small_cout_kernel<3>, grid, block, 0, s, in_dev, in_pixstride, w4, bias_dev, out_dev, out_pixstride, H, W, Cin, Cout, refl, act, act_alpha); break;
        case 5: hipLaunchKernelGGL(conv_small_cout_kernel<5>, grid, block, 0, s, in_dev, in_pixstride, w4, bias_dev, out_dev, out_pixstride, H, W, Cin, Cout, refl, act, act_alpha); break;
        case 7: hipLaunchKernelGGL(conv_small_cout_kernel<7>, grid, block, 0, s, in_dev, in_pixstride, w4, bias_dev, out_dev, out_pixstride, H, W, Cin, Cout, refl, act, act_alpha); break;
        default: return mit_set_error("mit_conv_small_cout: k must be 3, 5 or 7 (got %d)", k);
    }
    MIT_CHECK_LAUNCH("mit_conv_small_cout");
    return 0;
}
```

manga_image_translator_amd/lama.py:

```python
from __future__ import annotations

import ctypes as C
import math
from typing import Dict, Optional, Tuple

import numpy as np
import torch

from . import lib as _lib
from . import ops
from .ops import ACT_NONE, ACT_RELU, ACT_SIGMOID, PAD_REFLECT, PAD_ZERO, bn_params, conv_gemm_desc, launch_conv_gemm, tensor_map

LOCAL_C, GLOBAL_C, SPEC_C = 128, 384, 192
MPE_S = 256


def _cat_bn(sd, p1, p2):
    a, b = bn_params(sd, p1), bn_params(sd, p2)
    return tuple(torch.cat([x, y]) for x, y in zip(a[:4], b[:4])) + (a[4],)



def dft_matrices(h: int, w: int):
    wk = w // 2 + 1
# ... 58 lines not shown
        rows.append((s0, ws))
    maxt = max(len(ws) for _, ws in rows)
    start = np.array([s for s, _ in rows], dtype=np.int32)
    cnt = np.array([len(ws) for _, ws in rows], dtype=np.int32)
    wts = np.zeros((n_dst, maxt), dtype=np.float64)
    for d, (_, ws) in enumerate(rows):
        wts[d, :len(ws)] = ws
    return start, cnt, wts, maxt


def _nearest_map(n_dst: int, n_src: int) -> np.ndarray:
    return np.minimum(np.floor(np.arange(n_dst) * (n_src / n_dst)).astype(np.int64), n_src - 1).astype(np.int32)


class _RowPackedStem:

    K, PAD, WIN = 7, 3, 8

    def __init__(self, conv: "ops.Conv2d", weight: torch.Tensor, device):
        Cout, Cin, kh, kw = weight.shape
        if (kh, kw) != (self.K, self.K) or Cin > 4:
            raise ValueError("row-packed stem: 7x7 kernels with <= 4 input channels only")
        w = torch.zeros(self.K, self.WIN, 4, Cout, dtype=torch.float32)
        w[:, :self.K, :Cin] = weight.detach().to(torch.float32).permute(2, 3, 1, 0)
        self.w, self.Kp, self.Np = ops.pack_weight_kn(w.reshape(self.K * self.WIN * 4, Cout), device)
        self.Cout, self.scale, self.bias, self.act = Cout, conv.scale, conv.bias, conv.act

    def padded_shape(self, B, H, W):
        return (B, H + 2 * self.PAD, W + self.WIN, 4)

    def __call__(self, xp: torch.Tensor, out: torch.Tensor, lut: Optional[Tuple[torch.Tensor, torch.Tensor, torch.Tensor]] = None):
        B, Hp, Wp, _ = xp.shape
        H, W = Hp - 2 * self.PAD, Wp - self.WIN
        d = conv_gemm_desc(
            a=xp, NB=B, Hi=Hp, Wi=W, Cin=self.WIN * 4, a_strides=(Hp * Wp * 4, Wp * 4, 4), Ho=H, Wo=W, sy=1, sx=1,
            taps=[(ky, 0, 0) for ky in range(self.K)], pad_mode=PAD_ZERO, w=self.w, ldw=self.Np, Kw=self.Kp, Nw=self.Np,
            N=self.Cout, c=tensor_map(out), scale=self.scale, bias=self.bias, act=self.act)
        if lut is not None:
            rows, t1, t2 = lut
            if rows.dtype != torch.int32 or rows.numel() != B * H * W or t1.shape[1] != self.Cout or t2.shape[1] != self.Cout:
                raise ValueError("row-packed stem: bad lookup tables")
            d.lut_rows, d.lut1, d.lut2, d.lut_ld = rows.data_ptr(), t1.data_ptr(), t2.data_ptr(), self.Cout
        launch_conv_gemm(d)


class _FFC:

    def __init__(self, sd, p, device, winograd=True):
        w_l = torch.cat([sd[p + ".ffc.convl2l.weight"], sd[p + ".ffc.convg2l.weight"]], dim=1)
        self.winograd = winograd
        self._direct = None
        self._direct_src = (sd[p + ".ffc.convl2l.weight"], sd[p + ".ffc.convg2l.weight"], sd[p + ".ffc.convl2g.weight"],
                            bn_params(sd, p + ".bn_l"), device) if winograd else None
        if winograd:
            self.to_l = ops.WinogradConv3x3(w_l, None, pad_mode=PAD_REFLECT, bn=bn_params(sd, p + ".bn_l"), act=ACT_RELU, device=device)
            self.l2g = ops.WinogradConv3x3(sd[p + ".ffc.convl2g.weight"], None, pad_mode=PAD_REFLECT, device=device)
        else:
            self.to_l = ops.Conv2d(w_l, None, padding=1, pad_mode=PAD_REFLECT, bn=bn_params(sd, p + ".bn_l"), act=ACT_RELU,
                                   device=device)
            self.l2g = ops.Conv2d(sd[p + ".ffc.convl2g.weight"], None, padding=1, pad_mode=PAD_REFLECT, device=device)
        st = p + ".ffc.convg2g"
        self.st_in = ops.Conv2d(sd[st + ".conv1.0.weight"], None, bn=bn_params(sd, st + ".conv1.1"), act=ACT_RELU, device=device)
        wf = sd[st + ".fu.conv_layer.weight"].reshape(SPEC_C, 2, SPEC_C, 2)
        wf = wf.permute(3, 2, 1, 0).reshape(2 * SPEC_C, 2 * SPEC_C)
        self.fu_w, self.fu_Kp, self.fu_Np = ops.pack_weight_kn(wf, device)
        g, b, m, v, eps = bn_params(sd, st + ".fu.bn")
        perm = lambda t: t.reshape(SPEC_C, 2).t().reshape(-1)
        sc, bi = ops.fold_bn(perm(g), perm(b), perm(m), perm(v), eps)
        self.fu_scale, self.fu_bias = sc.to(device), bi.to(device)
        self.st_out = ops.Conv2d(sd[st + ".conv2.weight"], None, bn=bn_params(sd, p + ".bn_g"), act=ACT_RELU, device=device)

    def direct(self):
        if not self.winograd:
            return self.to_l, self.l2g
        if self._direct is None:
            w_l2l, w_g2l, w_l2g, bn_l, device = self._direct_src
            self._direct = (ops.Conv2d(torch.cat([w_l2l, w_g2l], dim=1), None, padding=1, pad_mode=PAD_REFLECT, bn=bn_l, act=ACT_RELU,
                                       device=device),
                            ops.Conv2d(w_l2g, None, padding=1, pad_mode=PAD_REFLECT, device=device))
            self._direct_src = None
        return self._direct


class LamaEngine(ops.Engine):

    def __init__(self, gen_sd: Dict[str, torch.Tensor], mpe_sd: Optional[Dict[str, torch.Tensor]] = None,
                 n_blocks: int = 9, device="cuda", fft_h: bool = True, winograd: bool = True, fft_w: bool = True,
                 row_packed_stem: bool = True):
        super().__init__(device)
        self.winograd = winograd
        self.fft_h = fft_h
        self.fft_w = fft_w
        self.n_blocks = n_blocks
        sd, dev = gen_sd, self.device
        self.stem = ops.Conv2d(sd["model.1.ffc.convl2l.weight"], None, padding=3, pad_mode=PAD_REFLECT,
                               bn=bn_params(sd, "model.1.bn_l"), act=ACT_RELU, device=dev)
        self.stem_packed = _RowPackedStem(self.stem, sd["model.1.ffc.convl2l.weight"], dev) if row_packed_stem else None
        self.down1 = ops.Conv2d(sd["model.2.ffc.convl2l.weight"], None, stride=2, padding=1, pad_mode=PAD_REFLECT,
                                bn=bn_params(sd, "model.2.bn_l"), act=ACT_RELU, device=dev)
        self.down2 = ops.Conv2d(sd["model.3.ffc.convl2l.weight"], None, stride=2, padding=1, pad_mode=PAD_REFLECT,
                                bn=bn_params(sd, "model.3.bn_l"), act=ACT_RELU, device=dev)
        w3 = torch.cat([sd["model.4.ffc.convl2l.weight"], sd["model.4.ffc.convl2g.weight"]], dim=0)
        self.down3 = ops.Conv2d(w3, None, stride=2, padding=1, pad_mode=PAD_REFLECT,
                                bn=_cat_bn(sd, "model.4.bn_l", "model.4.bn_g"), act=ACT_RELU, device=dev)
        self.blocks = [(_FFC(sd, f"model.{5 + i}.conv1", dev, winograd), _FFC(sd, f"model.{5 + i}.conv2", dev, winograd))
                       for i in range(n_blocks)]
        base = 5 + n_blocks + 1
        self.ups = []
        for i in range(3):
            p = base + 3 * i
            self.ups.append(ops.ConvTranspose2d(sd[f"model.{p}.weight"], sd[f"model.{p}.bias"], stride=2, padding=1,
                                                output_padding=1, bn=bn_params(sd, f"model.{p + 1}"), act=ACT_RELU, device=dev))
        p = base + 10
        self.out_conv = ops.ConvSmallCout(sd[f"model.{p}.weight"], sd[f"model.{p}.bias"], pad_mode=PAD_REFLECT,
                                          act=ACT_SIGMOID, device=dev)
        self.mpe = None
        if mpe_sd is not None:
            self.mpe = dict(emb=mpe_sd["rel_pos_emb.weight"].to(torch.float32).to(dev).contiguous(),
                            dirw=mpe_sd["direct_emb.weight"].to(torch.float32).to(dev).contiguous(),
                            alpha5=float(mpe_sd["alpha5"]), alpha6=float(mpe_sd["alpha6"]))
            emb, dirw = self.mpe["emb"].cpu(), self.mpe["dirw"].cpu()
            a5, a6 = torch.tensor(self.mpe["alpha5"], dtype=torch.float32), torch.tensor(self.mpe["alpha6"], dtype=torch.float32)
            t2 = torch.zeros(16, dirw.shape[1], dtype=torch.float32)
            for bits in range(16):
                acc = torch.zeros(dirw.shape[1], dtype=torch.float32)
                for k in range(4):
                    if bits & (1 << k):
                        acc = acc + dirw[k]
                t2[bits] = acc * a6
            self.mpe["lut1"], self.mpe["lut2"] = (emb * a5).contiguous().to(dev), t2.contiguous().to(dev)
        self.planar_tail = 4
        self.mpe_in_stem = True
        self._tw: Dict[int, torch.Tensor] = {}
        self._tw_rows: Dict[int, torch.Tensor] = {}
        self._dft = ops.ShapeCache(4)
        self._mpe_tabs = ops.ShapeCache(4)

    def release_workspace(self):
        super().release_workspace()
        self._dft.clear()
        self._mpe_tabs.clear()

    def _dft_mats(self, h, w):
        return self._dft.get((h, w), lambda: tuple(m.to(self.device) for m in dft_matrices(h, w)))

    def _twiddles(self, h):
        if h not in self._tw:
            ang = 2.0 * np.pi * np.arange(h // 2) / h
            self._tw[h] = torch.from_numpy(np.stack([np.cos(ang), np.sin(ang)], 1).astype(np.float32)).to(self.device).contiguous()
        return self._tw[h]

    def _row_tables(self, w):
        if w not in self._tw_rows:
            self._tw_rows[w] = rfft_row_tables(w).to(self.device)
        return self._tw_rows[w]

    def _fft_h(self, src, dst, dst_strides, B, h, ncols, plane, inverse):
        _lib.check(_lib.load().mit_fft_cols(src.data_ptr(), 2 * plane, plane, ncols, dst.data_ptr(), *dst_strides,
                                            self._twiddles(h).data_ptr(), B, h, ncols, int(inverse), 1.0 / math.sqrt(h),
                                            C.c_void_p(ops.current_stream())), "mit_fft_cols")

    def _mpe_tables(self, H, W):
        def make():
            ys, yc, yw, ymax = _area_taps(H, MPE_S)
            xs, xc, xw, xmax = _area_taps(W, MPE_S)
            dev = self.device
            t = lambda a: torch.from_numpy(np.ascontiguousarray(a)).to(dev)
            return dict(ys=t(ys), yc=t(yc), yw=t(yw), ymax=ymax, xs=t(xs), xc=t(xc), xw=t(xw), xmax=xmax,
                        ymap=t(_nearest_map(H, MPE_S)), xmap=t(_nearest_map(W, MPE_S)))

        return self._mpe_tabs.get((H, W), make)

# ... 32 lines not shown
            launch_conv_gemm(conv_gemm_desc(
                a=F1, NB=1, Hi=2, Wi=wk, Cin=F1.shape[1], a_strides=(0, wk * F1.shape[1], F1.shape[1]), Ho=2, Wo=wk, sy=1,
                sx=1, taps=one, pad_mode=PAD_ZERO, w=t1, ldw=Cc, Kw=w, Nw=Cc, N=Cc, c=cm, Z=B * h, zdiv=h,
                w_zs=(h * w * Cc, w * Cc)))
        self._dbg_put("fu1_rfft_rows", Y)
        if use_fft:
            self._fft_h(Y, Zf, (2 * plane, plane, wk * Cc), B, h, wk * Cc, plane, False)
        else:
            cm = ops.MitTensorMap()
            cm.base, cm.zs1, cm.zs0, cm.bs, cm.ys, cm.xs = Zf.data_ptr(), 0, 2 * plane, 0, 0, wk * Cc
            tag()
            launch_conv_gemm(conv_gemm_desc(
                a=G2, NB=1, Hi=1, Wi=2 * h, Cin=G2.shape[1], a_strides=(0, 0, G2.shape[1]), Ho=1, Wo=2 * h, sy=1, sx=1, taps=one,
                pad_mode=PAD_ZERO, w=Y, ldw=wk * Cc, Kw=2 * h, Nw=wk * Cc, N=wk * Cc, c=cm, Z=B, zdiv=1 << 30,
                w_zs=(0, 2 * plane)))
        self._dbg_put("fu2_fft_cols", Zf)
        cm = ops.MitTensorMap()
        cm.base, cm.zs1, cm.zs0, cm.bs, cm.ys, cm.xs = Z2.data_ptr(), 0, 0, 2 * plane, wk * Cc, Cc
        cm.nsplit, cm.nhi = Cc, plane
        launch_conv_gemm(conv_gemm_desc(
            a=Zf, NB=B, Hi=h, Wi=wk, Cin=Cc, a_strides=(2 * plane, wk * Cc, Cc), Ho=h, Wo=wk, sy=1, sx=1,
            taps=[(0, 0, 0), (0, 0, plane)], pad_mode=PAD_ZERO, w=ffc.fu_w, ldw=ffc.fu_Np, Kw=ffc.fu_Kp, Nw=ffc.fu_Np,
            N=2 * Cc, c=cm, scale=ffc.fu_scale, bias=ffc.fu_bias, act=ACT_RELU, nprod=nprod))
        self._dbg_put("fu3_spectral_conv", Z2)
        if use_fft:
            self._fft_h(Z2, U, (2 * plane, wk * Cc, 2 * wk * Cc), B, h, wk * Cc, plane, True)
        else:
            cm = ops.MitTensorMap()
            cm.base, cm.zs1, cm.zs0, cm.bs, cm.ys, cm.xs = U.data_ptr(), 0, 2 * plane, 0, wk * Cc, 2 * wk * Cc
            tag()
            launch_conv_gemm(conv_gemm_desc(
                a=G2i, NB=1, Hi=2, Wi=h, Cin=G2i.shape[1], a_strides=(0, h * G2i.shape[1], G2i.shape[1]), Ho=2, Wo=h, sy=1, sx=1, taps=one,
                pad_mode=PAD_ZERO, w=Z2, ldw=wk * Cc, Kw=2 * h, Nw=wk * Cc, N=wk * Cc, c=cm, Z=B, zdiv=1 << 30,
                w_zs=(0, 2 * plane)))
        self._dbg_put("fu4_ifft_cols", U)
        if use_fft_w:
            _lib.check(lib.mit_irfft_rows(U.data_ptr(), 2 * plane, wk * Cc, 2 * wk * Cc, Cc, t2.data_ptr(), h * w * Cc, w * Cc,
                                          Cc, t1.data_ptr(), h * w * Cc, w * Cc, Cc, self._row_tables(w).data_ptr(), B, h, w, Cc,
                                          1.0 / math.sqrt(w), st), "mit_irfft_rows")
            return
        cm = ops.MitTensorMap()
        cm.base, cm.zs1, cm.zs0, cm.bs, cm.ys, cm.xs = t2.data_ptr(), 0, w * Cc, 0, 0, Cc
        pm = ops.MitTensorMap()
        pm.base, pm.zs1, pm.zs0, pm.bs, pm.ys, pm.xs = t1.data_ptr(), 0, w * Cc, 0, 0, Cc
        tag()
        launch_conv_gemm(conv_gemm_desc(
            a=Fi, NB=1, Hi=1, Wi=w, Cin=Fi.shape[1], a_strides=(0, 0, Fi.shape[1]), Ho=1, Wo=w, sy=1, sx=1, taps=one,
            pad_mode=PAD_ZERO, w=U, ldw=Cc, Kw=2 * wk, Nw=Cc, N=Cc, c=cm, post=pm, Z=B * h, zdiv=1 << 30,
            w_zs=(0, 2 * wk * Cc)))

    def _ffc(self, ffc: _FFC, x: torch.Tensor, out: torch.Tensor, residual: Optional[torch.Tensor], nprod: int = 0):
        B, h, w, _ = x.shape
        x_l, x_g = x[..., :LOCAL_C], x[..., LOCAL_C:]
        res_l = None if residual is None else residual[..., :LOCAL_C]
        res_g = None if residual is None else residual[..., LOCAL_C:]
        P = self._buf("ffc_P", B, h, w, GLOBAL_C)
        if nprod:
            to_l, l2g = ffc.direct()
            to_l(x, out=out[..., :LOCAL_C], post=res_l, nprod=nprod)
            l2g(x_l, out=P, nprod=nprod)
        elif ffc.winograd:
            T = ops.WinogradConv3x3.tiles(B, h, w)
            V = self._buf("wino_v", 36, T, LOCAL_C + GLOBAL_C)
            ffc.to_l.transform_input(x, V)
            self._dbg_put("w1_wino_input", V)
            ffc.to_l.gemm_output(V, self._buf("wino_ml", 36, T, LOCAL_C), out[..., :LOCAL_C], post=res_l)
            self._dbg_put("w2_wino_products_l", self._buf("wino_ml", 36, T, LOCAL_C))
            self._dbg_put("w3_out_local", out[..., :LOCAL_C])
            ffc.l2g.gemm_output(V, self._buf("wino_mg", 36, T, GLOBAL_C), P)
            self._dbg_put("w4_wino_products_g", self._buf("wino_mg", 36, T, GLOBAL_C))
            self._dbg_put("w5_P", P)
        else:
            ffc.to_l(x, out=out[..., :LOCAL_C], post=res_l)
            ffc.l2g(x_l, out=P)
        t1 = self._buf("ffc_t1", B, h, w, SPEC_C)
        t2 = self._buf("ffc_t2", B, h, w, SPEC_C)
        ffc.st_in(x_g, out=t1, nprod=nprod)
        self._dbg_put("s1_st_in", t1)
        self._fourier_unit(ffc, t1, t2, nprod)
        self._dbg_put("fu5_irfft_rows_plus_t1", t2)
        ffc.st_out(t2, out=out[..., LOCAL_C:], pre=P, post=res_g, nprod=nprod)
        self._dbg_put("s2_out_global", out[..., LOCAL_C:])

    @torch.no_grad()
    def forward(self, img_u8: torch.Tensor, mask_u8: torch.Tensor, taps: Optional[dict] = None, composite: bool = True,
                precision: str = "fp32") -> torch.Tensor:
        if precision not in ("fp32", "bf16"):
            raise ValueError(f"LamaEngine.forward: precision must be 'fp32' or 'bf16' (got {precision!r})")
        nprod = 1 if precision == "bf16" else 0
        if img_u8.dtype != torch.uint8 or mask_u8.dtype != torch.uint8:
            raise TypeError("LamaEngine.forward expects uint8 page and mask tensors")
        if img_u8.dim() != 4 or img_u8.shape[-1] != 3 or tuple(mask_u8.shape) != tuple(img_u8.shape[:3]):
            raise ValueError(f"bad shapes: page {tuple(img_u8.shape)}, mask {tuple(mask_u8.shape)}")
        B, H, W, _ = img_u8.shape
        if H % 8 or W % 8:
            raise ValueError("LamaEngine.forward: H and W must be multiples of 8 (the plugin resizes first, :67-79)")
        img_u8, mask_u8 = img_u8.contiguous(), mask_u8.contiguous()
        lib = _lib.load()
        st = C.c_void_p(ops.current_stream())
        s64 = self._buf("full64", B, H, W, 64)
        packed = self.stem_packed is not None and H > 3 and W > 3
        lut = None
        if self.mpe is not None:
            tb = self._mpe_tables(H, W)
            hole = self._buf("mpe_hole", B, MPE_S, MPE_S, dtype=torch.uint8)
            rel = self._buf("mpe_rel", B, MPE_S, MPE_S, dtype=torch.uint8)
            dr = self._buf("mpe_dir", B, MPE_S, MPE_S, dtype=torch.uint8)
            _lib.check(lib.mit_lama_mpe_index(mask_u8.data_ptr(), B, H, W, tb["ys"].data_ptr(), tb["yc"].data_ptr(),
                                              tb["yw"].data_ptr(), tb["ymax"], tb["xs"].data_ptr(), tb["xc"].data_ptr(),
                                              tb["xw"].data_ptr(), tb["xmax"], hole.data_ptr(), rel.data_ptr(),
                                              dr.data_ptr(), st), "mit_lama_mpe_index")
            if packed and self.mpe_in_stem:
                rows = self._buf("mpe_rows", B * H * W, dtype=torch.int32)
                _lib.check(lib.mit_lama_mpe_rows(mask_u8.data_ptr(), rel.data_ptr(), dr.data_ptr(), tb["ymap"].data_ptr(),
                                                 tb["xmap"].data_ptr(), rows.data_ptr(), B, H, W, st), "mit_lama_mpe_rows")
                lut = (rows, self.mpe["lut1"], self.mpe["lut2"])
        if packed:
            xp = self._buf("in4p", *self.stem_packed.padded_shape(B, H, W))
            _lib.check(lib.mit_lama_prep_padded(img_u8.data_ptr(), mask_u8.data_ptr(), xp.data_ptr(), B, H, W, 3, xp.shape[2], st),
                       "mit_lama_prep_padded")
            self.stem_packed(xp, s64, lut=lut)
        else:
            x4 = self._buf("in4", B, H, W, 4)
            _lib.check(lib.mit_lama_prep(img_u8.data_ptr(), mask_u8.data_ptr(), x4.data_ptr(), B, H, W, st), "mit_lama_prep")
            self.stem(x4, out=s64)
        if self.mpe is not None:
            if lut is None:
                _lib.check(lib.mit_lama_mpe_add(s64.data_ptr(), mask_u8.data_ptr(), rel.data_ptr(), dr.data_ptr(),
                                                tb["ymap"].data_ptr(), tb["xmap"].data_ptr(), self.mpe["emb"].data_ptr(),
                                                self.mpe["dirw"].data_ptr(), self.mpe["alpha5"], self.mpe["alpha6"], B, H, W,
                                                st), "mit_lama_mpe_add")
            if taps is not None:
                taps["mpe_rel"], taps["mpe_dir"], taps["mpe_hole"] = rel.clone(), dr.clone(), hole.clone()
        if taps is not None:
            taps["stem"] = s64.clone()
        d1 = self._buf("d1", B, H // 2, W // 2, 128)
        self.down1(s64, out=d1, nprod=nprod)
        d2 = self._buf("d2", B, H // 4, W // 4, 256)
        self.down2(d1, out=d2, nprod=nprod)
        h, w = H // 8, W // 8
        X = self._buf("X", B, h, w, 512)
        T = self._buf("Xtmp", B, h, w, 512)
        self.down3(d2, out=X, nprod=nprod)
        if taps is not None:
            taps["down"] = X.clone()
        for i, (c1, c2) in enumerate(self.blocks):
            self._ffc(c1, X, T, None, nprod)
            self._ffc(c2, T, X, X, nprod)
            if taps is not None:
                taps[f"block{i}"] = X.clone()
        u1 = self._buf("d2", B, H // 4, W // 4, 256)
        self.ups[0](X, out=u1, nprod=nprod)
        u2 = self._buf("d1", B, H // 2, W // 2, 128)
        self.ups[1](u1, out=u2, nprod=nprod)
        pred = self._buf("pred", B, H, W, 3)
        if self.planar_tail:
            P = self.planar_tail
            pm = P == 4 and H % 2 == 0 and W % 2 == 0
            u3 = self._buf("full64", 64 // P, B, H, W, P)
            self.ups[2](u2, out=u3, planes=64 // P, parity_major=pm, nprod=nprod)
            self.out_conv(u3, out=pred, parity_major=pm)
        else:
            u3 = self._buf("full64", B, H, W, 64)
            self.ups[2](u2, out=u3, nprod=nprod)
            self.out_conv(u3, out=pred)
        if taps is not None:
            taps["pred"] = pred.clone()
        out = torch.empty(B, H, W, 3, dtype=torch.uint8, device=self.device)
        _lib.check(lib.mit_lama_post(pred.data_ptr(), 3, img_u8.data_ptr(), mask_u8.data_ptr(), out.data_ptr(), B, H, W,
                                     int(composite), st), "mit_lama_post")
        return out

    def flops_per_page(self, H: int, W: int) -> float:
        px = H * W
        conv = 2.0 * px * (49 * 4 * 64 + 49 * 64 * 3)
        conv += 2.0 * (px / 4) * 9 * 64 * 128 + 2.0 * (px / 16) * 9 * 128 * 256 + 2.0 * (px / 64) * 9 * 256 * 512
        per_ffc = 2.0 * (px / 64) * (9 * (128 * 128 + 384 * 128 + 128 * 384) + 384 * 192 + 192 * 384)
        per_ffc += 2.0 * (px / 64) * ((W // 8 // 2 + 1) / (W // 8)) * 384 * 384
        conv += per_ffc * 2 * self.n_blocks
        conv += 2.0 * (px / 64) * 9 * 512 * 256 + 2.0 * (px / 16) * 9 * 256 * 128 + 2.0 * (px / 4) * 9 * 128 * 64
        return conv
```

manga_image_translator_amd/lib.py:

```python
from __future__ import annotations

import ctypes as C
from pathlib import Path

MIT_MAX_TAPS = 64
MIT_ABI_VERSION = 20

ACT_NONE, ACT_RELU, ACT_LEAKY, ACT_SILU, ACT_SIGMOID, ACT_GELU = range(6)
ACT_POST_FIRST = 0x100
PAD_ZERO, PAD_REFLECT = 0, 1


class MitTensorMap(C.Structure):
    _fields_ = [
        ("base", C.c_void_p),
        ("zs1", C.c_int64),
        ("zs0", C.c_int64),
        ("bs", C.c_int64),
        ("ys", C.c_int64),
        ("xs", C.c_int64),
        ("nhi", C.c_int64),
        ("nsplit", C.c_int32),
        ("_pad", C.c_int32),
    ]


class MitConvGemm(C.Structure):
    _fields_ = [
        ("a", C.c_void_p),
        ("a_zs1", C.c_int64),
        ("a_zs0", C.c_int64),
        ("a_bs", C.c_int64),
        ("a_ys", C.c_int64),
        ("a_xs", C.c_int64),
        ("NB", C.c_int32),
        ("Hi", C.c_int32),
        ("Wi", C.c_int32),
        ("Cin", C.c_int32),
        ("Ho", C.c_int32),
        ("Wo", C.c_int32),
        ("sy", C.c_int32),
        ("sx", C.c_int32),
        ("ntaps", C.c_int32),
        ("pad_mode", C.c_int32),
        ("tap_dy", C.c_int8 * MIT_MAX_TAPS),
        ("tap_dx", C.c_int8 * MIT_MAX_TAPS),
        ("tap_off", C.c_int32 * MIT_MAX_TAPS),
        ("w", C.c_void_p),
        ("w_zs1", C.c_int64),
        ("w_zs0", C.c_int64),
        ("ldw", C.c_int64),
        ("Kw", C.c_int32),
        ("Nw", C.c_int32),
        ("N", C.c_int32),
        ("Z", C.c_int32),
        ("zdiv", C.c_int32),
        ("c", MitTensorMap),
        ("pre", MitTensorMap),
        ("post", MitTensorMap),
        ("scale", C.c_void_p),
        ("bias", C.c_void_p),
        ("act", C.c_int32),
        ("act_alpha", C.c_float),
        ("w_split", C.c_void_p),
        ("ws_zs0", C.c_int64),
        ("lut_rows", C.c_void_p),
        ("lut1", C.c_void_p),
        ("lut2", C.c_void_p),
        ("lut_ld", C.c_int64),
        ("nprod", C.c_int32),
        ("_pad1", C.c_int32),
    ]


class MitPGemm(C.Structure):
    _fields_ = [
        ("a_planes", C.c_void_p), ("a_zs", C.c_int64), ("lda", C.c_int64),
        ("w_planes", C.c_void_p), ("w_zs", C.c_int64), ("ldw", C.c_int64),
        ("M", C.c_int32), ("N", C.c_int32), ("K", C.c_int32), ("Z", C.c_int32),
        ("c", C.c_void_p), ("ldc", C.c_int64), ("c_zs", C.c_int64),
        ("pre", C.c_void_p), ("ld_pre", C.c_int64), ("pre_zs", C.c_int64),
        ("post", C.c_void_p), ("ld_post", C.c_int64), ("post_zs", C.c_int64),
        ("c_planes", C.c_void_p), ("ld_cp", C.c_int64), ("cp_zs", C.c_int64),
        ("scale", C.c_void_p), ("bias", C.c_void_p),
        ("act", C.c_int32), ("act_alpha", C.c_float), ("nprod", C.c_int32), ("tile", C.c_int32),
    ]


class MitXposTables(C.Structure):
    _fields_ = [("cos_t", C.c_void_p), ("sin_t", C.c_void_p), ("scale_t", C.c_void_p), ("iscale_t", C.c_void_p),
                ("imax", C.c_int32), ("pmax", C.c_int32)]


class MitLinear(C.Structure):
    _fields_ = [("w", C.c_void_p), ("scale", C.c_void_p), ("bias", C.c_void_p), ("ldw", C.c_int64), ("K", C.c_int32),
                ("N", C.c_int32), ("Kp", C.c_int32), ("Np", C.c_int32), ("w_split", C.c_void_p)]


class MitOcrDecoderLayer(C.Structure):
    _fields_ = [("ln1_w", C.c_void_p), ("ln1_b", C.c_void_p), ("ln2_w", C.c_void_p), ("ln2_b", C.c_void_p),
                ("ln3_w", C.c_void_p), ("ln3_b", C.c_void_p), ("qkv", MitLinear), ("out", MitLinear), ("q2", MitLinear),
                ("out2", MitLinear), ("ff1", MitLinear), ("ff2", MitLinear)]


class MitOcr48Decoder(C.Structure):
    _fields_ = [("layers", MitOcrDecoderLayer * 5), ("embd", C.c_void_p), ("pred1", MitLinear), ("pred", MitLinear),
                ("color1", MitLinear), ("color_heads", MitLinear), ("xpos", MitXposTables), ("dict_size", C.c_int32),
                ("_pad", C.c_int32)]


class MitOcr48DecodeArgs(C.Structure):
    _fields_ = [("N", C.c_int32), ("L", C.c_int32), ("mem_k", C.c_void_p), ("mem_v", C.c_void_p), ("mem_len", C.c_void_p),
                ("max_seq_length", C.c_int32), ("start_tok", C.c_int32), ("end_tok", C.c_int32), ("max_finished", C.c_int32),
                ("suppress_eos", C.c_int32), ("workspace", C.c_void_p), ("workspace_bytes", C.c_int64),
                ("res_tok", C.c_void_p), ("res_len", C.c_void_p), ("res_prob", C.c_void_p), ("res_row", C.c_void_p),
                ("colors", C.c_void_p), ("trace_logits", C.c_void_p), ("trace_hist", C.c_void_p), ("steps_run", C.c_int32)]


class MitOcr32Decoder(C.Structure):
    _fields_ = [("layers", MitOcrDecoderLayer * 2), ("embd", C.c_void_p), ("pe", C.c_void_p), ("pred1", MitLinear), ("pred", MitLinear),
                ("color1", MitLinear), ("color_heads", MitLinear), ("dict_size", C.c_int32), ("pe_len", C.c_int32)]


class MitOcr32DecodeArgs(C.Structure):
    _fields_ = [("N", C.c_int32), ("L", C.c_int32), ("mem_k", C.c_void_p), ("mem_v", C.c_void_p), ("mem_len", C.c_void_p),
                ("max_seq_length", C.c_int32), ("start_tok", C.c_int32), ("end_tok", C.c_int32), ("max_finished", C.c_int32),
                ("workspace", C.c_void_p), ("workspace_bytes", C.c_int64), ("res_tok", C.c_void_p), ("res_len", C.c_void_p),
                ("res_prob", C.c_void_p), ("colors", C.c_void_p), ("res_src", C.c_void_p), ("trace_logits", C.c_void_p),
                ("trace_hist", C.c_void_p), ("steps_run", C.c_int32), ("form", C.c_int32)]


class MitProfStat(C.Structure):
    _fields_ = [("launches", C.c_int64), ("ms", C.c_double), ("exec_flops", C.c_double), ("alg_flops", C.c_double)]


class MitProfKernelStat(C.Structure):
    _fields_ = [("name", C.c_char * 48), ("launches", C.c_int64), ("ms", C.c_double), ("alg_bytes", C.c_double),
                ("alg_flops", C.c_double)]


class MitWarpLine(C.Structure):
    _fields_ = [("minv", C.c_double * 9), ("page", C.c_int32), ("x1", C.c_int32), ("y1", C.c_int32), ("cw", C.c_int32),
                ("ch", C.c_int32), ("dw", C.c_int32), ("dh", C.c_int32), ("vertical", C.c_int32), ("out_row", C.c_int32),
                ("_pad", C.c_int32)]


class MitCrfCrop(C.Structure):
    _fields_ = [("x", C.c_int32), ("y", C.c_int32), ("w", C.c_int32), ("h", C.c_int32)]


class MitDilateJob(C.Structure):
    _fields_ = [("sx", C.c_int32), ("sy", C.c_int32), ("sw", C.c_int32), ("sh", C.c_int32), ("dx", C.c_int32), ("dy", C.c_int32),
                ("dw", C.c_int32), ("dh", C.c_int32), ("k", C.c_int32), ("spitch", C.c_int32), ("src_off", C.c_int64)]


class MitMaskRun(C.Structure):
    _fields_ = [("y", C.c_int32), ("x0", C.c_int32), ("x1", C.c_int32), ("comp", C.c_int32)]


class MitRefineWindow(C.Structure):
    _fields_ = [("x1", C.c_int32), ("y1", C.c_int32), ("x2", C.c_int32), ("y2", C.c_int32)]


class MitRefineCand(C.Structure):
    _fields_ = [("kind", C.c_int32), ("lo", C.c_int32), ("hi", C.c_int32), ("invert", C.c_int32)]


class MitRaggedSeg(C.Structure):
    _fields_ = [("pixel_start", C.c_int64), ("group_start", C.c_int64), ("B", C.c_int32), ("H", C.c_int32), ("W", C.c_int32),
                ("_pad", C.c_int32)]


SYMBOLS = {
    "mit_last_error": (C.c_char_p, []),
    "mit_abi_version": (C.c_int, []),
    "mit_source_digest": (C.c_char_p, []),
    "mit_device_count": (C.c_int, [C.POINTER(C.c_int)]),
    "mit_device_name": (C.c_int, [C.c_int, C.c_char_p, C.c_int]),
    "mit_conv_gemm": (C.c_int, [C.POINTER(MitConvGemm), C.c_void_p]),
    "mit_conv_gemm_cfg": (C.c_int, [C.POINTER(MitConvGemm), C.c_int, C.c_void_p]),
    "mit_conv_gemm_config_name": (C.c_char_p, [C.c_int]),
    "mit_conv_gemm_plan": (C.c_int, [C.POINTER(MitConvGemm), C.c_int, C.POINTER(C.c_int32), C.POINTER(C.c_int32)]),
    "mit_conv_gemm_config_kernel": (C.c_char_p, [C.c_int]),
    "mit_gemm_split_pack": (C.c_int, [C.c_void_p, C.c_int64, C.c_int, C.c_int, C.c_int64, C.c_void_p, C.c_void_p]),
    "mit_gemm_mode_set": (C.c_int, [C.c_int]),
    "mit_gemm_mode_get": (C.c_int, []),
    "mit_gemm_split_min_tiles": (C.c_int64, [C.c_int64]),
    "mit_conv_small_cout": (C.c_int, [C.c_void_p, C.c_int64, C.c_int64, C.c_void_p, C.c_void_p, C.c_void_p, C.c_void_p, C.c_int64, C.c_int, C.c_int,
                                      C.c_int, C.c_int, C.c_int, C.c_int, C.c_int, C.c_int, C.c_float, C.c_void_p]),
    "mit_convnext_mlp_supported": (C.c_int, [C.c_int]),
    "mit_convnext_mlp": (C.c_int, [C.c_void_p, C.c_int64, C.c_int, C.c_int, C.c_void_p, C.c_void_p, C.c_void_p, C.c_int64, C.c_void_p, C.c_void_p,
                                   C.c_void_p, C.c_int64, C.c_void_p, C.c_int64, C.c_void_p]),
    "mit_prof_enable": (C.c_int, [C.c_int]),
    "mit_prof_tag_next": (C.c_int, [C.c_double]),
    "mit_prof_read": (C.c_int, [C.POINTER(MitProfStat), C.c_int, C.POINTER(C.c_int)]),
    "mit_prof_dump": (C.c_int, [C.c_char_p]),
    "mit_prof_kernels_read": (C.c_int, [C.POINTER(MitProfKernelStat), C.c_int, C.POINTER(C.c_int)]),
    "mit_wino43_input": (C.c_int, [C.c_void_p, C.c_int64, C.c_int64, C.c_int64, C.c_void_p, C.c_int, C.c_int, C.c_int, C.c_int, C.c_int,
                                   C.c_void_p]),
    "mit_wino43_output": (C.c_int, [C.c_void_p, C.c_void_p, C.c_int64, C.c_int64, C.c_int64, C.c_void_p, C.c_int64, C.c_int64, C.c_int64,
                                    C.c_void_p, C.c_void_p, C.c_int, C.c_int, C.c_int, C.c_int, C.c_int, C.c_float, C.c_void_p]),
    "mit_ocr_warp_lines": (C.c_int, [C.c_void_p, C.c_int, C.c_int, C.c_void_p, C.c_int, C.c_void_p, C.c_int, C.c_int,
                                     C.c_void_p]),
    "mit_fft_cols": (C.c_int, [C.c_void_p, C.c_int64, C.c_int64, C.c_int64, C.c_void_p, C.c_int64, C.c_int64, C.c_int64,
                               C.c_void_p, C.c_int, C.c_int, C.c_int64, C.c_int, C.c_float, C.c_void_p]),
    "mit_rfft_rows_supported": (C.c_int, [C.c_int]),
    "mit_rfft_rows": (C.c_int, [C.c_void_p, C.c_int64, C.c_int64, C.c_int64, C.c_void_p, C.c_int64, C.c_int64, C.c_int64, C.c_int64,
                                C.c_void_p, C.c_int, C.c_int, C.c_int, C.c_int, C.c_float, C.c_void_p]),
    "mit_irfft_rows": (C.c_int, [C.c_void_p, C.c_int64, C.c_int64, C.c_int64, C.c_int64, C.c_void_p, C.c_int64, C.c_int64, C.c_int64,
                                 C.c_void_p, C.c_int64, C.c_int64, C.c_int64, C.c_void_p, C.c_int, C.c_int, C.c_int, C.c_int,
                                 C.c_float, C.c_void_p]),
    "mit_bilateral_u8c3": (C.c_int, [C.c_void_p, C.c_void_p, C.c_int, C.c_int, C.c_int, C.c_int, C.c_int, C.c_void_p, C.c_void_p,
                                     C.c_void_p, C.c_void_p]),
    "mit_mask_dilate_jobs": (C.c_int, [C.c_void_p, C.c_void_p, C.c_int, C.c_void_p, C.c_int, C.c_int, C.c_int, C.c_void_p, C.c_void_p]),
    "mit_binarize_u8": (C.c_int, [C.c_void_p, C.c_int64, C.c_void_p]),
    "mit_densecrf_workspace_bytes": (C.c_int64, [C.c_void_p, C.c_int]),
    "mit_densecrf_refine": (C.c_int, [C.c_void_p, C.c_int, C.c_int, C.c_void_p, C.c_int, C.c_void_p, C.c_void_p, C.c_void_p, C.c_float,
                                      C.c_float, C.c_float, C.c_float, C.c_float, C.c_int, C.c_void_p, C.c_void_p, C.c_int64, C.c_void_p]),
    "mit_ctd_refine_workspace_bytes": (C.c_int64, [C.c_void_p, C.c_int]),
    "mit_ctd_refine_hist": (C.c_int, [C.c_void_p, C.c_void_p, C.c_int, C.c_int, C.c_void_p, C.c_int, C.c_void_p, C.c_void_p, C.c_int64,
                                      C.c_void_p]),
    "mit_ctd_refine_scores": (C.c_int, [C.c_void_p, C.c_void_p, C.c_int, C.c_int, C.c_void_p, C.c_int, C.c_void_p, C.c_void_p, C.c_void_p,
                                        C.c_int64, C.c_void_p]),
    "mit_ctd_refine_merge": (C.c_int, [C.c_void_p, C.c_void_p, C.c_int, C.c_int, C.c_void_p, C.c_int, C.c_void_p, C.c_void_p, C.c_void_p,
                                       C.c_int64, C.c_void_p]),
    "mit_lama_prep": (C.c_int, [C.c_void_p, C.c_void_p, C.c_void_p, C.c_int, C.c_int, C.c_int, C.c_void_p]),
    "mit_lama_prep_padded": (C.c_int, [C.c_void_p, C.c_void_p, C.c_void_p, C.c_int, C.c_int, C.c_int, C.c_int, C.c_int, C.c_void_p]),
    "mit_lama_mpe_index": (C.c_int, [C.c_void_p, C.c_int, C.c_int, C.c_int, C.c_void_p, C.c_void_p, C.c_void_p,
                                     C.c_int, C.c_void_p, C.c_void_p, C.c_void_p, C.c_int, C.c_void_p, C.c_void_p,
                                     C.c_void_p, C.c_void_p]),
    "mit_lama_mpe_add": (C.c_int, [C.c_void_p, C.c_void_p, C.c_void_p, C.c_void_p, C.c_void_p, C.c_void_p,
                                   C.c_void_p, C.c_void_p, C.c_float, C.c_float, C.c_int, C.c_int, C.c_int,
                                   C.c_void_p]),
    "mit_lama_mpe_rows": (C.c_int, [C.c_void_p, C.c_void_p, C.c_void_p, C.c_void_p, C.c_void_p, C.c_void_p, C.c_int, C.c_int, C.c_int, C.c_void_p]),
    "mit_ctd_prep": (C.c_int, [C.c_void_p, C.c_int, C.c_int, C.c_int, C.c_int, C.c_int, C.c_int, C.c_int, C.c_void_p,
                               C.c_void_p, C.c_void_p, C.c_void_p, C.c_void_p, C.c_void_p]),
    "mit_maxpool_nhwc": (C.c_int, [C.c_void_p, C.c_int64, C.c_void_p, C.c_int64, C.c_int, C.c_int, C.c_int, C.c_int,
                                   C.c_int, C.c_void_p]),
    "mit_maxpool2d_nhwc": (C.c_int, [C.c_void_p, C.c_void_p, C.c_int, C.c_int, C.c_int, C.c_int, C.c_int, C.c_int, C.c_int,
                                     C.c_void_p]),
    "mit_avgpool2_nhwc": (C.c_int, [C.c_void_p, C.c_int64, C.c_void_p, C.c_int64, C.c_int, C.c_int, C.c_int, C.c_int,
                                    C.c_void_p]),
    "mit_copy_channels": (C.c_int, [C.c_void_p, C.c_int64, C.c_void_p, C.c_int64, C.c_int64, C.c_int, C.c_void_p]),
    "mit_map_to_u8": (C.c_int, [C.c_void_p, C.c_void_p, C.c_int64, C.c_int, C.c_float, C.c_void_p]),
    "mit_axpy": (C.c_int, [C.c_void_p, C.c_float, C.c_void_p, C.c_void_p, C.c_int64, C.c_void_p]),
    "mit_boxes_from_bitmap": (C.c_int, [C.c_void_p, C.c_void_p, C.c_int, C.c_int, C.c_int, C.c_int, C.c_int, C.c_float, C.c_float,
                                        C.c_float, C.c_float, C.c_int, C.c_void_p, C.c_void_p, C.POINTER(C.c_int)]),
    "mit_boxes_debug_stamps": (C.c_int, [C.c_void_p]),
    "mit_boxes_from_bitmap_dev_workspace_bytes": (C.c_int64, [C.c_int, C.c_int, C.c_int, C.c_int]),
    "mit_boxes_from_bitmap_dev": (C.c_int, [C.c_void_p, C.c_int64, C.c_void_p, C.c_int64, C.c_float, C.c_int, C.c_int, C.c_int, C.c_int, C.c_int, C.c_int, C.c_float, C.c_float,
                                            C.c_float, C.c_float, C.c_int, C.c_void_p, C.c_int64, C.c_void_p, C.c_void_p, C.c_void_p, C.c_void_p, C.c_void_p]),
    "mit_merge_mask_list": (C.c_int, [C.c_void_p, C.c_void_p, C.c_int, C.c_void_p, C.c_int, C.c_int, C.c_int, C.c_void_p]),
    "mit_otsu_from_hist": (C.c_int, [C.c_void_p, C.c_int, C.c_void_p]),
    "mit_find_contours_count": (C.c_int, [C.c_void_p, C.c_int, C.c_int, C.POINTER(C.c_int), C.POINTER(C.c_int64)]),
    "mit_mask_assign_lines": (C.c_int, [C.c_void_p, C.c_int, C.c_int, C.c_void_p, C.c_void_p, C.c_void_p, C.c_int, C.c_int, C.c_double, C.c_void_p,
                                        C.c_int64, C.c_void_p, C.c_int64, C.c_void_p, C.POINTER(C.c_int64), C.POINTER(C.c_int32)]),
    "mit_mask_line_crops": (C.c_int, [C.c_void_p, C.c_int64, C.c_void_p, C.c_void_p, C.c_int, C.c_void_p, C.c_void_p]),
    "mit_mask_assign_workspace_bytes": (C.c_int64, [C.c_int, C.c_int]),
    "mit_mask_assign_lines_dev": (C.c_int, [C.c_void_p, C.c_int, C.c_int, C.c_void_p, C.c_void_p, C.c_void_p, C.c_int, C.c_int, C.c_double,
                                            C.c_void_p, C.c_int64, C.c_void_p, C.c_void_p]),
    "mit_mask_line_crops_dev": (C.c_int, [C.c_void_p, C.c_int64, C.c_int, C.c_int, C.c_void_p, C.c_void_p, C.c_int, C.c_int64, C.c_void_p,
                                          C.c_void_p]),
    "mit_ocr_prep": (C.c_int, [C.c_void_p, C.c_void_p, C.c_int, C.c_int, C.c_int, C.c_void_p]),
    "mit_dwconv_nhwc": (C.c_int, [C.c_void_p, C.c_void_p, C.c_void_p, C.c_void_p, C.c_void_p, C.c_int, C.c_int, C.c_int,
                                  C.c_int, C.c_int, C.c_void_p]),
    "mit_quad_pair_distances": (C.c_int, [C.c_void_p, C.c_int, C.c_void_p, C.c_int, C.c_void_p]),
    "mit_ocr48_decode_rows_max_set": (C.c_int, [C.c_int]),
    "mit_pgemm": (C.c_int, [C.POINTER(MitPGemm), C.c_void_p]),
    "mit_pgemm_tile_name": (C.c_char_p, [C.c_int]),
    "mit_pgemm_supported": (C.c_int, [C.POINTER(MitPGemm)]),
    "mit_split_planes": (C.c_int, [C.c_void_p, C.c_int64, C.c_int, C.c_int, C.c_void_p, C.c_int64, C.c_void_p]),
    "mit_join_planes": (C.c_int, [C.c_void_p, C.c_int64, C.c_int, C.c_int, C.c_void_p, C.c_int64, C.c_void_p]),
# ... 127 lines not shown
```

manga_image_translator_amd/ops.py:

```python
from __future__ import annotations

import ctypes as C
import math
import os
import weakref
from dataclasses import dataclass, field
from typing import Dict, List, Optional, Sequence, Tuple

import torch

from . import lib as _lib
from .lib import (ACT_GELU, ACT_LEAKY, ACT_NONE, ACT_POST_FIRST, ACT_RELU, ACT_SIGMOID, ACT_SILU, MIT_MAX_TAPS, PAD_REFLECT,
                  PAD_ZERO, MitConvGemm, MitPGemm, MitTensorMap)

__all__ = [
    "ACT_NONE", "ACT_RELU", "ACT_LEAKY", "ACT_SILU", "ACT_SIGMOID", "ACT_GELU", "ACT_POST_FIRST", "PAD_ZERO", "PAD_REFLECT",
    "Conv2d", "ConvSmallCout", "split_mode", "ensure_split", "set_split_mode", "gemm_mode", "ConvTranspose2d", "UpsampleConv2d", "fold_bn", "conv_gemm_desc", "launch_conv_gemm", "current_stream",
]


def current_stream() -> int:
    return torch.cuda.current_stream().cuda_stream


# ... 15 lines not shown
            t = torch.empty(max(n, 1), dtype=dtype, device=self.device)
            self._slabs[key] = t
        return t[:n].view(*shape)

    def release(self) -> None:
        self._slabs.clear()

    def nbytes(self) -> int:
        return sum(t.numel() * t.element_size() for t in self._slabs.values())


class Engine:

    def __init__(self, device="cuda"):
        self.device = torch.device(device)
        self._ws = Workspace(self.device)

    @property
    def _buf(self):
        return self._ws.buf

    def release_workspace(self) -> None:
        self._ws.release()


def bn_params(sd, prefix: str, eps: float = 1e-5):
    return (sd[prefix + ".weight"], sd[prefix + ".bias"], sd[prefix + ".running_mean"], sd[prefix + ".running_var"], eps)


class ShapeCache:

    def __init__(self, capacity: int = 4):
        self.capacity, self._d = capacity, {}

    def get(self, key, make):
        if key in self._d:
            self._d[key] = self._d.pop(key)
            return self._d[key]
        v = make()
        self._d[key] = v
        while len(self._d) > self.capacity:
            self._d.pop(next(iter(self._d)))
        return v

    def clear(self):
        self._d.clear()

    def __len__(self):
        return len(self._d)


def _ptr(t: Optional[torch.Tensor]) -> Optional[int]:
    return None if t is None else t.data_ptr()


def _check_nhwc(t: torch.Tensor, what: str) -> None:
    if t.dtype != torch.float32:
        raise TypeError(f"{what}: expected float32, got {t.dtype}")
    if t.dim() != 4:
        raise ValueError(f"{what}: expected [B,H,W,C], got shape {tuple(t.shape)}")
    if t.shape[-1] > 1 and t.stride(-1) != 1:
        raise ValueError(f"{what}: channel stride must be 1, got strides {t.stride()}")


def tensor_map(t: Optional[torch.Tensor], zs1: int = 0, zs0: int = 0, nsplit: int = 0, nhi: int = 0) -> MitTensorMap:
    m = MitTensorMap()
    if t is None:
        m.base = None
        return m
    _check_nhwc(t, "tensor_map")
    m.base = t.data_ptr()
    m.zs1, m.zs0 = zs1, zs0
    m.bs, m.ys, m.xs = t.stride(0), t.stride(1), t.stride(2)
    m.nsplit, m.nhi = nsplit, nhi
    return m


def conv_gemm_desc(*, a: torch.Tensor, NB: int, Hi: int, Wi: int, Cin: int, a_strides: Tuple[int, int, int],
                   Ho: int, Wo: int, sy: int, sx: int, taps: Sequence[Tuple[int, int, int]], pad_mode: int,
                   w: torch.Tensor, ldw: int, Kw: int, Nw: int, N: int, c: MitTensorMap,
                   pre: Optional[MitTensorMap] = None, post: Optional[MitTensorMap] = None,
                   scale: Optional[torch.Tensor] = None, bias: Optional[torch.Tensor] = None, act: int = ACT_NONE,
                   alpha: float = 0.0, Z: int = 1, zdiv: int = 1, a_zs: Tuple[int, int] = (0, 0),
                   w_zs: Tuple[int, int] = (0, 0), nprod: int = 0) -> MitConvGemm:
    if len(taps) == 0 or len(taps) > MIT_MAX_TAPS:
        raise ValueError(f"ntaps {len(taps)} out of range")
    d = MitConvGemm()
    d.a = a.data_ptr()
    d.a_zs1, d.a_zs0 = a_zs
    d.a_bs, d.a_ys, d.a_xs = a_strides
    d.NB, d.Hi, d.Wi, d.Cin = NB, Hi, Wi, Cin
    d.Ho, d.Wo, d.sy, d.sx = Ho, Wo, sy, sx
    d.ntaps, d.pad_mode = len(taps), pad_mode
    for i, (dy, dx, off) in enumerate(taps):
        d.tap_dy[i], d.tap_dx[i], d.tap_off[i] = dy, dx, off
    d.w = w.data_ptr()
    d.w_zs1, d.w_zs0 = w_zs
    d.ldw, d.Kw, d.Nw = ldw, Kw, Nw
    if _SPLITS:
        planes, zs = _split_for(w, ldw, Kw, w_zs, nprod)
        if planes is not None:
            d.w_split, d.ws_zs0 = planes.data_ptr(), zs
    d.N, d.Z, d.zdiv = N, Z, zdiv
    d.c = c
    d.pre = pre if pre is not None else tensor_map(None)
    d.post = post if post is not None else tensor_map(None)
    d.scale = _ptr(scale)
    d.bias = _ptr(bias)
    d.act, d.act_alpha = act, alpha
    d.nprod = int(nprod)
    return d


def launch_conv_gemm(desc: MitConvGemm, cfg: int = -1, stream: Optional[int] = None) -> None:
    lib = _lib.load()
    s = current_stream() if stream is None else stream
    _lib.check(lib.mit_conv_gemm_cfg(C.byref(desc), cfg, C.c_void_p(s)), "mit_conv_gemm")


def fold_bn(gamma: torch.Tensor, beta: torch.Tensor, mean: torch.Tensor, var: torch.Tensor, eps: float,
            conv_bias: Optional[torch.Tensor] = None) -> Tuple[torch.Tensor, torch.Tensor]:
    g, b, m, v = (t.detach().to(torch.float64) for t in (gamma, beta, mean, var))
    scale = g / torch.sqrt(v + eps)
    bias = b - m * scale
    if conv_bias is not None:
        bias = bias + conv_bias.detach().to(torch.float64) * scale
    return scale.to(torch.float32), bias.to(torch.float32)


def split_mode() -> int:
    return int(_lib.load().mit_gemm_mode_get())


def set_split_mode(mode: int) -> int:
    lib = _lib.load()
    prev = int(lib.mit_gemm_mode_get())
    _lib.check(lib.mit_gemm_mode_set(int(mode)), "mit_gemm_mode_set")
    return prev


class gemm_mode:

    def __init__(self, mode: int, min_tiles: Optional[int] = None):
        self.mode, self.min_tiles, self.prev, self.prev_min = int(mode), min_tiles, None, None

    def __enter__(self):
        self.prev = set_split_mode(self.mode)
        if self.min_tiles is not None:
            self.prev_min = int(_lib.load().mit_gemm_split_min_tiles(int(self.min_tiles)))
        return self

    def __exit__(self, *exc):
        set_split_mode(self.prev)
        if self.prev_min is not None:
            _lib.load().mit_gemm_split_min_tiles(self.prev_min)
        return False


_SPLITS: Dict[int, tuple] = {}


def split_weight(w: torch.Tensor) -> torch.Tensor:
    if w.dtype != torch.float32 or not w.is_contiguous() or w.dim() not in (2, 3):
        raise ValueError("split_weight: contiguous fp32 [Kp, Np] or [nz, Kp, Np] expected")
    nz = 1 if w.dim() == 2 else w.shape[0]
    Kp, Np = w.shape[-2], w.shape[-1]
    if Kp % 8 or Np % 4:
        raise ValueError(f"split_weight: Kp % 8 == 0 and Np % 4 == 0 needed (got {Kp} x {Np})")
    out = torch.empty(nz, 3, Kp // 8, Np, 8, dtype=torch.int16, device=w.device)
    _lib.check(_lib.load().mit_gemm_split_pack(w.data_ptr(), Kp * Np, nz, Kp, Np, out.data_ptr(), C.c_void_p(current_stream())),
               "mit_gemm_split_pack")
    return out


def register_split(w: torch.Tensor, force: bool = False, p1_only: bool = False) -> Optional[torch.Tensor]:
    if w.device.type != "cuda" or not (force or split_mode()):
        return None
    planes = split_weight(w)
    nz = 1 if w.dim() == 2 else w.shape[0]
    key = w.data_ptr()
    _SPLITS[key] = (weakref.ref(w, lambda _r, k=key: _SPLITS.pop(k, None)), planes, nz, w.shape[-2], w.shape[-1], bool(p1_only))
    return planes


def ensure_split(w: torch.Tensor) -> None:
    e = _SPLITS.get(w.data_ptr())
    if e is None or e[0]() is not w:
        register_split(w, force=True, p1_only=True)


def _split_for(w: torch.Tensor, ldw: int, Kw: int, w_zs: Tuple[int, int], nprod: int = 0):
    e = _SPLITS.get(w.data_ptr())
    if e is None or e[0]() is not w or (e[3], e[4]) != (Kw, ldw) or w_zs[0] != 0 or (e[2] > 1 and w_zs[1] != Kw * ldw):
# ... 175 lines not shown
            raise ValueError(f"WinogradConv3x3: 3x3 kernels with Cin % 4 == 0 and even Cout only (got {tuple(weight.shape)})")
        if act not in (ACT_NONE, ACT_RELU, ACT_LEAKY):
            raise ValueError("WinogradConv3x3: activation must be none / relu / leaky")
        self.Cin, self.Cout, self.pad_mode, self.act, self.alpha = Cin, Cout, pad_mode, act, alpha
        G = torch.tensor(self.G, dtype=torch.float64)
        U = torch.einsum("ia,ocab,jb->ijco", G, weight.detach().to(torch.float64), G).reshape(36, Cin, Cout)
        self.Kp, self.Np = _round_up(Cin, 16), _round_up(Cout, 4)
        u = torch.zeros(36, self.Kp, self.Np, dtype=torch.float32)
        u[:, :Cin, :Cout] = U.to(torch.float32)
        self.u = u.to(device).contiguous()
        register_split(self.u)
        scale = bias_t = None
        if bn is not None:
            scale, bias_t = fold_bn(*bn, conv_bias=bias)
        elif bias is not None:
            bias_t = bias.detach().to(torch.float32)
        self.scale = None if scale is None else scale.to(device).contiguous()
        self.bias = None if bias_t is None else bias_t.to(device).contiguous()

    @staticmethod
    def tiles(B: int, H: int, W: int) -> int:
        return B * ((H + 3) // 4) * ((W + 3) // 4)

    def transform_input(self, x: torch.Tensor, v: torch.Tensor) -> torch.Tensor:
        _check_nhwc(x, "WinogradConv3x3 input")
        B, H, W, Cx = x.shape
        T = self.tiles(B, H, W)
        if tuple(v.shape) != (36, T, Cx) or not v.is_contiguous():
            raise ValueError(f"WinogradConv3x3: V must be contiguous [36, {T}, {Cx}] (got {tuple(v.shape)})")
        _lib.check(_lib.load().mit_wino43_input(x.data_ptr(), x.stride(0), x.stride(1), x.stride(2), v.data_ptr(), B, H, W, Cx,
                                                self.pad_mode, C.c_void_p(current_stream())), "mit_wino43_input")
        return v

    def gemm_desc(self, v: torch.Tensor, m: torch.Tensor) -> MitConvGemm:
        _, T, Cv = v.shape
        if Cv < self.Cin or tuple(m.shape) != (36, T, self.Cout) or not m.is_contiguous():
            raise ValueError(f"WinogradConv3x3: bad V / M shapes {tuple(v.shape)} / {tuple(m.shape)}")
        cm = MitTensorMap()
        cm.base, cm.zs1, cm.zs0, cm.bs, cm.ys, cm.xs = m.data_ptr(), 0, T * self.Cout, 0, 0, self.Cout
        return conv_gemm_desc(a=v, NB=1, Hi=1, Wi=T, Cin=self.Cin, a_strides=(0, 0, Cv), Ho=1, Wo=T, sy=1, sx=1, taps=[(0, 0, 0)],
                              pad_mode=PAD_ZERO, w=self.u, ldw=self.Np, Kw=self.Kp, Nw=self.Np, N=self.Cout, c=cm, Z=36,
                              zdiv=1 << 30, a_zs=(0, T * Cv), w_zs=(0, self.Kp * self.Np))

    def gemm_output(self, v: torch.Tensor, m: torch.Tensor, out: torch.Tensor, post: Optional[torch.Tensor] = None, cfg: int = -1):
        _check_nhwc(out, "WinogradConv3x3 output")
        B, H, W, Co = out.shape
        if Co != self.Cout or self.tiles(B, H, W) != v.shape[1]:
            raise ValueError(f"WinogradConv3x3: output {tuple(out.shape)} does not match V {tuple(v.shape)}")
        if post is not None and tuple(post.shape) != tuple(out.shape):
            raise ValueError("WinogradConv3x3: residual shape differs from the output")
        launch_conv_gemm(self.gemm_desc(v, m), cfg)
        ps = (0, 0, 0) if post is None else (post.stride(0), post.stride(1), post.stride(2))
        _lib.check(_lib.load().mit_wino43_output(m.data_ptr(), out.data_ptr(), out.stride(0), out.stride(1), out.stride(2), _ptr(post), *ps,
                                                 _ptr(self.scale), _ptr(self.bias), B, H, W, self.Cout, self.act, self.alpha,
                                                 C.c_void_p(current_stream())), "mit_wino43_output")
        return out

    def __call__(self, x: torch.Tensor, out: Optional[torch.Tensor] = None, post: Optional[torch.Tensor] = None,
                 v: Optional[torch.Tensor] = None, m: Optional[torch.Tensor] = None) -> torch.Tensor:
        B, H, W, Cx = x.shape
        T = self.tiles(B, H, W)
        if out is None:
            out = torch.empty(B, H, W, self.Cout, dtype=torch.float32, device=x.device)
        v = torch.empty(36, T, Cx, dtype=torch.float32, device=x.device) if v is None else v
        m = torch.empty(36, T, self.Cout, dtype=torch.float32, device=x.device) if m is None else m
        self.transform_input(x, v)
        return self.gemm_output(v, m, out, post)


class ConvSmallCout:

    def __init__(self, weight: torch.Tensor, bias: Optional[torch.Tensor] = None, *, pad_mode: int = PAD_ZERO,
                 act: int = ACT_NONE, alpha: float = 0.0, device="cuda"):
        Cout, Cin, kh, kw = weight.shape
        if kh != kw or kh not in (3, 5, 7) or Cout > 4 or Cin % 16:
            raise ValueError(f"ConvSmallCout: unsupported shape {tuple(weight.shape)}")
        self.Cout, self.Cin, self.k, self.pad_mode, self.act, self.alpha = Cout, Cin, kh, pad_mode, act, alpha
        w4 = torch.zeros(kh * kw, Cin, 4, dtype=torch.float32)
        w4[:, :, :Cout] = weight.detach().to(torch.float32).permute(2, 3, 1, 0).reshape(kh * kw, Cin, Cout)
        self.w4 = w4.to(device).contiguous()
        self.w_pairs = (w4.reshape(kh * kw, Cin // 4, 4, 4).permute(0, 1, 3, 2).to(device).contiguous() if Cout <= 3 else None)
        self.bias = None if bias is None else bias.detach().to(torch.float32).to(device).contiguous()

    def __call__(self, x: torch.Tensor, out: torch.Tensor, parity_major: bool = False) -> torch.Tensor:
        plane = 0
        if x.dim() == 5:
            pc = x.shape[4]
            if self.w_pairs is None or pc not in (4, 16) or x.shape[0] * pc < self.Cin or not x.is_contiguous():
                raise ValueError(f"ConvSmallCout: planar input must be contiguous [Cin / P, B, H, W, P] with P = 4 or 16 for Cout <= 3 (got {tuple(x.shape)})")
            if pc == 4 and self.pad_mode != PAD_REFLECT:
                raise ValueError("ConvSmallCout: 4-channel planes are read by the LDS-DMA kernel, which implements reflect padding only")
            if parity_major and (pc != 4 or x.shape[2] % 2 or x.shape[3] % 2):
                raise ValueError("ConvSmallCout: the parity-major layout needs 4-channel planes of even height and width")
            plane = x.stride(0)
            x = x[0].as_strided((x.shape[1], x.shape[2], x.shape[3], self.Cin), (x.stride(1), x.stride(2), x.stride(3), 1))
        _check_nhwc(x, "ConvSmallCout input")
        _check_nhwc(out, "ConvSmallCout output")
        B, H, W, Cx = x.shape
        if Cx < self.Cin or tuple(out.shape[:3]) != (B, H, W) or out.shape[3] < self.Cout:
            raise ValueError(f"ConvSmallCout: bad shapes {tuple(x.shape)} -> {tuple(out.shape)}")
        if not (x.stride(2) * W == x.stride(1) and x.stride(1) * H == x.stride(0) and out.stride(2) * W == out.stride(1)
                and out.stride(1) * H == out.stride(0)):
            raise ValueError("ConvSmallCout: pixel-dense tensors required")
        lib = _lib.load()
        if parity_major and not plane:
            raise ValueError("ConvSmallCout: parity_major without planar input")
        _lib.check(lib.mit_conv_small_cout(x.data_ptr(), x.stride(2), -plane if parity_major else plane, self.w4.data_ptr(), _ptr(self.w_pairs), _ptr(self.bias), out.data_ptr(),
                                           out.stride(2), B, H, W, self.Cin, self.Cout, self.k, self.pad_mode, self.act,
                                           self.alpha, C.c_void_p(current_stream())), "mit_conv_small_cout")
        return out


class UpsampleConv2d:

    def __init__(self, weight: torch.Tensor, bias: Optional[torch.Tensor] = None, *, act: int = ACT_NONE, alpha: float = 0.0,
                 device="cuda"):
        Cout, Cin, kh, kw = weight.shape
        if (kh, kw) != (3, 3) or Cin % 4:
            raise ValueError("UpsampleConv2d: 3x3 kernels with Cin % 4 == 0 only")
        self.Cin, self.Cout, self.act, self.alpha = Cin, Cout, act, alpha
        w = weight.detach().to(torch.float64)
        groups = {0: {-1: [0], 0: [1, 2]}, 1: {0: [0, 1], 1: [2]}}
        self.sub: List[Tuple[int, int, _Packed]] = []
        for a in (0, 1):
            for b in (0, 1):
                taps, blocks = [], []
                for dy, kys in groups[a].items():
                    for dx, kxs in groups[b].items():
                        wsum = sum(w[:, :, ky, kx] for ky in kys for kx in kxs)
                        taps.append((dy, dx, 0))
                        blocks.append(wsum.t().to(torch.float32))
                wk, Kp, Np = pack_weight_kn(torch.cat(blocks, dim=0), device)
                self.sub.append((a, b, _Packed(wk, Kp, Np, taps)))
        self.bias = None if bias is None else bias.detach().to(torch.float32).to(device).contiguous()

    def descs(self, x: torch.Tensor, out: torch.Tensor) -> List[MitConvGemm]:
        _check_nhwc(x, "UpsampleConv2d input")
        _check_nhwc(out, "UpsampleConv2d output")
        B, H, W, Cx = x.shape
        if Cx != self.Cin or tuple(out.shape) != (B, 2 * H, 2 * W, self.Cout):
            raise ValueError(f"UpsampleConv2d: bad shapes {tuple(x.shape)} -> {tuple(out.shape)}")
        ds = []
        for a, b, pk in self.sub:
            ov = out[:, a::2, b::2]
            ds.append(conv_gemm_desc(
                a=x, NB=B, Hi=H, Wi=W, Cin=self.Cin, a_strides=(x.stride(0), x.stride(1), x.stride(2)), Ho=H, Wo=W, sy=1, sx=1,
                taps=pk.taps, pad_mode=PAD_ZERO, w=pk.w, ldw=pk.Np, Kw=pk.Kp, Nw=pk.Np, N=self.Cout, c=tensor_map(ov),
                bias=self.bias, act=self.act, alpha=self.alpha))
        return ds

    def __call__(self, x: torch.Tensor, out: Optional[torch.Tensor] = None, cfg: int = -1) -> torch.Tensor:
        if out is None:
            out = torch.empty(x.shape[0], 2 * x.shape[1], 2 * x.shape[2], self.Cout, dtype=torch.float32, device=x.device)
        for d in self.descs(x, out):
            launch_conv_gemm(d, cfg)
        return out


class ConvTranspose2d:

    def __init__(self, weight: torch.Tensor, bias: Optional[torch.Tensor] = None, *, stride=2, padding=0,
                 output_padding=0, bn=None, act: int = ACT_NONE, alpha: float = 0.0, device="cuda"):
        Cin, Cout, kh, kw = weight.shape
        if Cin % 4:
            raise ValueError("ConvTranspose2d: Cin must be a multiple of 4")
        self.Cin, self.Cout, self.k, self.s, self.p, self.op = Cin, Cout, (kh, kw), stride, padding, output_padding
        self.act, self.alpha = act, alpha
        w = weight.detach().to(torch.float32)
        self.sub: List[Tuple[int, int, _Packed]] = []
        s, p = stride, padding
        for py in range(s):
            kys = [ky for ky in range(kh) if (py + p - ky) % s == 0]
            for px in range(s):
                kxs = [kx for kx in range(kw) if (px + p - kx) % s == 0]
                taps, blocks = [], []
                for ky in kys:
                    for kx in kxs:
                        taps.append(((py + p - ky) // s, (px + p - kx) // s, 0))
                        blocks.append(w[:, :, ky, kx])
                if not taps:
                    raise ValueError("ConvTranspose2d: empty parity class (kernel smaller than stride)")
                wk, Kp, Np = pack_weight_kn(torch.cat(blocks, dim=0), device)
                self.sub.append((py, px, _Packed(wk, Kp, Np, taps)))
        scale = bias_t = None
        if bn is not None:
            scale, bias_t = fold_bn(*bn, conv_bias=bias)
        elif bias is not None:
            bias_t = bias.detach().to(torch.float32)
        self.scale = None if scale is None else scale.to(device).contiguous()
        self.bias = None if bias_t is None else bias_t.to(device).contiguous()

    def out_hw(self, H: int, W: int) -> Tuple[int, int]:
        return ((H - 1) * self.s - 2 * self.p + self.k[0] + self.op, (W - 1) * self.s - 2 * self.p + self.k[1] + self.op)

    def descs(self, x: torch.Tensor, out: torch.Tensor, planes: int = 0, parity_major: bool = False, nprod: int = 0) -> List[MitConvGemm]:
        split = nhi = 0
        if planes:
            if out.dim() != 5 or out.shape[0] != planes or out.shape[4] * planes != self.Cout or not out.is_contiguous():
                raise ValueError(f"ConvTranspose2d: planar output must be contiguous [{planes}, B, Ho, Wo, {self.Cout // planes}]")
            split, nhi = out.shape[4], out.stride(0)
            out = out[0].as_strided((out.shape[1], out.shape[2], out.shape[3], self.Cout), (out.stride(1), out.stride(2), out.stride(3), 1))
        _check_nhwc(x, "ConvTranspose2d input")
        _check_nhwc(out, "ConvTranspose2d output")
        B, H, W, Cx = x.shape
        if Cx != self.Cin:
            raise ValueError(f"ConvTranspose2d: input has {Cx} channels, layer expects {self.Cin}")
        Ho, Wo = self.out_hw(H, W)
        if tuple(out.shape) != (B, Ho, Wo, self.Cout):
            raise ValueError(f"ConvTranspose2d: output shape {tuple(out.shape)} != {(B, Ho, Wo, self.Cout)}")
        if parity_major and not (planes and self.s == 2 and Ho % 2 == 0 and Wo % 2 == 0):
            raise ValueError("ConvTranspose2d: the parity-major layout is for planar output of a stride-2 layer with even output size")
        ds = []
        for py, px, pk in self.sub:
            ov = out[:, py::self.s, px::self.s]
            if ov.shape[1] == 0 or ov.shape[2] == 0:
                continue
            if nprod:
                ensure_split(pk.w)
            if parity_major:
                pc, h2, w2 = self.Cout // planes, Ho // 2, Wo // 2
                ov = out.as_strided((B, h2, w2, self.Cout), (Ho * Wo * pc, w2 * pc, pc, 1),
                                    out.storage_offset() + (py * 2 + px) * h2 * w2 * pc)
            ds.append(conv_gemm_desc(
                a=x, NB=B, Hi=H, Wi=W, Cin=self.Cin, a_strides=(x.stride(0), x.stride(1), x.stride(2)),
                Ho=ov.shape[1], Wo=ov.shape[2], sy=1, sx=1, taps=pk.taps, pad_mode=PAD_ZERO, w=pk.w, ldw=pk.Np,
                Kw=pk.Kp, Nw=pk.Np, N=self.Cout, c=tensor_map(ov, nsplit=split, nhi=nhi), scale=self.scale, bias=self.bias, act=self.act,
                alpha=self.alpha, nprod=nprod))
        return ds

    def __call__(self, x: torch.Tensor, out: Optional[torch.Tensor] = None, cfg: int = -1, planes: int = 0, parity_major: bool = False,
                 nprod: int = 0) -> torch.Tensor:
        if out is None:
            Ho, Wo = self.out_hw(x.shape[1], x.shape[2])
            out = (torch.empty(planes, x.shape[0], Ho, Wo, self.Cout // planes, dtype=torch.float32, device=x.device) if planes else
                   torch.empty(x.shape[0], Ho, Wo, self.Cout, dtype=torch.float32, device=x.device))
        for d in self.descs(x, out, planes, parity_major, nprod):
            launch_conv_gemm(d, cfg)
        return out
```

Before: 44.16.

## Compute LaMa decoder tail only on blocks the inpaint mask can reach

Adds a device pass that derives, from the inpaint mask, per-level lists of live 8x8 output blocks plus a cell bitmap. The transposed-conv GEMMs in the decoder tail then iterate only over live blocks, and the small-Cout output conv skips dead tiles. Pixels outside the mask's receptive field are composited from the original image anyway, so their decoder work is meant to be avoided. The cost is extra bookkeeping kernels, index decoding in the GEMM row loop, and launches still sized for the full grid with early-exit workgroups.

```diff
diff --git a/include/mit_hip.h b/include/mit_hip.h
--- a/include/mit_hip.h
+++ b/include/mit_hip.h
@@ -7,7 +7,7 @@
 extern "C" {
 #endif
 
-#define MIT_ABI_VERSION 20
+#define MIT_ABI_VERSION 21
 #define MIT_MAX_TAPS 64
 
 enum MitAct {
@@ -57,7 +57,9 @@
     const float *lut1, *lut2;
     int64_t lut_ld;
     int32_t nprod;
-    int32_t _pad1;
+    int32_t live_img0;
+    const int32_t *live_blocks;
+    const int32_t *live_start;
 } MitConvGemm;
 
 const char *mit_last_error(void);
@@ -108,7 +110,11 @@
 
 int mit_conv_small_cout(const float *in_dev, int64_t in_pixstride, int64_t in_planestride, const float *w4_dev, const float *w_pairs_dev, const float *bias_dev, float *out_dev,
                         int64_t out_pixstride, int B, int H, int W, int Cin, int Cout, int k, int pad_mode, int act,
-                        float act_alpha, void *stream);
+                        float act_alpha, const uint8_t *live_cells, void *stream);
+
+int64_t mit_lama_tail_need_work(int B, int H, int W);
+int mit_lama_tail_need(const uint8_t *mask_dev, int B, int H, int W, uint8_t *cells_dev, int32_t *list0_dev, int32_t *start0_dev, int32_t *list1_dev,
+                       int32_t *start1_dev, int32_t *list2_dev, int32_t *start2_dev, uint8_t *work_dev, void *stream);
 
 int mit_convnext_mlp_supported(int C);
 int mit_convnext_mlp(const float *x_dev, int64_t ldx, int M, int C, const uint16_t *w1_planes_dev, const float *b1_dev,
diff --git a/manga_image_translator_amd/csrc/conv_gemm.hip b/manga_image_translator_amd/csrc/conv_gemm.hip
--- a/manga_image_translator_amd/csrc/conv_gemm.hip
+++ b/manga_image_translator_amd/csrc/conv_gemm.hip
@@ -200,6 +200,9 @@
     if (p.lut_rows && ((p.lut_ld & 3) || (reinterpret_cast<uintptr_t>(p.lut1) & 15) || (reinterpret_cast<uintptr_t>(p.lut2) & 15))) return false;
     return !(reinterpret_cast<uintptr_t>(p.scale) & 15) && !(reinterpret_cast<uintptr_t>(p.bias) & 15);
 }
+
+int64_t list_rows(const MitConvGemm &p) { return (int64_t)p.NB * ((p.Ho + 7) / 8) * ((p.Wo + 7) / 8) * 64; }
+int64_t rows_of(const MitConvGemm &p) { return p.live_blocks ? list_rows(p) : (int64_t)p.NB * p.Ho * p.Wo; }
 
 int validate(const MitConvGemm *d, MitConvGemm &p) {
     if (!d) return mit_set_error("mit_conv_gemm: null descriptor");
@@ -231,6 +234,16 @@
         if (p.Z != 1) return mit_set_error("mit_conv_gemm: the row-lookup epilogue is for Z == 1 launches");
         if (p.lut_ld > 0x7fff) return mit_set_error("mit_conv_gemm: lut_ld too large (row offsets are 16-bit row x lut_ld in 32 bits)");
     }
+    if (p.live_blocks || p.live_start) {
+        if (!p.live_blocks || !p.live_start) return mit_set_error("mit_conv_gemm: a live-block list needs live_blocks and live_start");
+        if ((reinterpret_cast<uintptr_t>(p.live_blocks) | reinterpret_cast<uintptr_t>(p.live_start)) & 3) return mit_set_error("mit_conv_gemm: live_blocks / live_start must be 4-byte aligned");
+        if (p.Z != 1) return mit_set_error("mit_conv_gemm: a live-block list is for Z == 1 launches");
+        if (p.lut_rows) return mit_set_error("mit_conv_gemm: a live-block list together with lut_rows is not implemented");
+        if (p.live_img0 < 0) return mit_set_error("mit_conv_gemm: live_img0 must be >= 0 (got %d)", p.live_img0);
+        if (list_rows(p) > 0x7fffffffLL) return mit_set_error("mit_conv_gemm: M too large");
+    } else if (p.live_img0 != 0) {
+        return mit_set_error("mit_conv_gemm: live_img0 without a live-block list");
+    }
     if (p.Z > 65535) return mit_set_error("mit_conv_gemm: Z too large");
     if (p.nprod != 0 && p.nprod != 1) return mit_set_error("mit_conv_gemm: nprod must be 0 (the GEMM mode) or 1 (one bf16 product) (got %d)", p.nprod);
     if (p.nprod == 1 && !p.w_split) return mit_set_error("mit_conv_gemm: nprod = 1 needs w_split (mit_gemm_split_pack): there is no fp32 fallback for a requested precision");
@@ -260,11 +273,12 @@
     if (p.pre.base) r.pre.base += (int64_t)b0 * p.pre.bs;
     if (p.post.base) r.post.base += (int64_t)b0 * p.post.bs;
     if (p.lut_rows) r.lut_rows += (int64_t)b0 * p.Ho * p.Wo;
+    if (p.live_blocks) r.live_start += b0, r.live_img0 += b0;
     return r;
 }
 
 int plan_run(const MitConvGemm &p, int cfg, int *tile) {
-    const int64_t M = (int64_t)p.NB * p.Ho * p.Wo;
+    const int64_t M = rows_of(p);
     if (p.nprod == 1) {
         if (!split_eligible(p, 16))
             return mit_set_error("mit_conv_gemm: nprod = 1 needs the split tiles' preconditions (Cin %% 16 == 0, <= %d taps, 32-bit element offsets, 16-byte aligned w_split with w_zs1 == 0 and Kw %% 8 == 0): there is no fp32 fallback for a requested precision", FAST_MAX_TAPS);
@@ -281,6 +295,8 @@
         if (p.post.base) return mit_set_error("mit_conv_gemm: lut_rows together with a post residual is not implemented");
         if ((p.act & 0xff) != MIT_ACT_NONE && (p.act & 0xff) != MIT_ACT_RELU) return mit_set_error("mit_conv_gemm: lut_rows is implemented for act none / relu");
     }
+    if (p.live_blocks && !fast && !split)
+        return mit_set_error("mit_conv_gemm: a live-block list needs a fast or split tile (Cin %% 16 == 0, <= %d taps, N > 4); this launch takes %s", FAST_MAX_TAPS, c.name);
     if (gemv && (!gemv_eligible(p, c.lanes_per_row()) || p.N > c.BN))
         return mit_set_error("mit_conv_gemm: cfg %s needs N <= %d, Z == 1, unsplit maps and Cin %% %d == 0", c.name, c.BN, 4 * c.lanes_per_row());
     if (split && !split_eligible(p, c.BK))
@@ -294,7 +310,7 @@
 
 int launch_run(const MitConvGemm &p, int cfg, hipStream_t hs) {
     const CfgEntry &c = kCfgs[cfg];
-    const int M = p.NB * p.Ho * p.Wo;
+    const int M = (int)rows_of(p);
     const int MT = (M + c.BM - 1) / c.BM;
     const int NT = (p.N + c.BN - 1) / c.BN;
     const int Ktot = p.ntaps * p.Cin;
@@ -313,6 +329,15 @@
         MIT_CHECK_HIP(hipEventRecord(r.start, hs));
         c.launch(p, M, MT, NT, KT, hs);
         MIT_CHECK_HIP(hipEventRecord(r.stop, hs));
+        if (p.live_blocks) {
+            int32_t s0 = 0, s1 = 0;
+            MIT_CHECK_HIP(hipEventSynchronize(r.stop));
+            MIT_CHECK_HIP(hipMemcpy(&s0, p.live_start, sizeof(s0), hipMemcpyDeviceToHost));
+            MIT_CHECK_HIP(hipMemcpy(&s1, p.live_start + p.NB, sizeof(s1), hipMemcpyDeviceToHost));
+            r.M = (s1 - s0) * 64;
+            r.exec_flops = 2.0 * (double)r.M * p.N * Ktot * p.Z;
+            r.alg_flops = r.exec_flops;
+        }
         g_probe.push_back(r);
     } else {
         c.launch(p, M, MT, NT, KT, hs);
diff --git a/manga_image_translator_amd/csrc/conv_gemm_kernels.h b/manga_image_translator_amd/csrc/conv_gemm_kernels.h
--- a/manga_image_translator_amd/csrc/conv_gemm_kernels.h
+++ b/manga_image_translator_amd/csrc/conv_gemm_kernels.h
@@ -45,6 +45,34 @@
     if (ACT == MIT_ACT_SIGMOID) return 1.f / (1.f + expf(-v));
     if (ACT == MIT_ACT_GELU) return gelu_fast(v);
     return v;
+}
+
+__device__ __forceinline__ bool decode_row(const MitConvGemm &p, const int m, const int M, const int HoWo, int &nb, int &oy, int &ox) {
+    if (p.live_blocks == nullptr) {
+        if (m >= M) return false;
+        nb = m / HoWo;
+        const int rem = m - nb * HoWo;
+        oy = rem / p.Wo;
+        ox = rem - oy * p.Wo;
+        return true;
+    }
+    const int s0 = p.live_start[0];
+    const int blk = m >> 6;
+    if (m >= M || blk >= p.live_start[p.NB] - s0) return false;
+    const int bw = (p.Wo + 7) >> 3, bpi = ((p.Ho + 7) >> 3) * bw;
+    const int id = p.live_blocks[s0 + blk] - p.live_img0 * bpi;
+    nb = id / bpi;
+    const int rem = id - nb * bpi;
+    const int by = rem / bw;
+    oy = by * 8 + ((m & 63) >> 3);
+    ox = (rem - by * bw) * 8 + (m & 7);
+    return oy < p.Ho && ox < p.Wo;
+}
+template <int BM>
+__device__ __forceinline__ int live_workgroups(const MitConvGemm &p, const int MT, const int NT) {
+    if (p.live_blocks == nullptr) return MT * NT;
+    const int live = p.live_start[p.NB] - p.live_start[0];
+    return ((live * 64 + BM - 1) / BM) * NT;
 }
 
 template <int TM, int TN, int ACT, bool HAS_POST>
@@ -145,11 +173,8 @@
     for (int r = tid; r < BM; r += NTHR) {
         const int m = m0 + r;
         RowOff ro = {-1, 0, 0};
-        if (m < M) {
-            const int nb = m / HoWo;
-            const int rem = m - nb * HoWo;
-            const int oy = rem / p.Wo;
-            const int ox = rem - oy * p.Wo;
+        int nb, oy, ox;
+        if (decode_row(p, m, M, HoWo, nb, oy, ox)) {
             ro.c = z1 * p.c.zs1 + z0 * p.c.zs0 + (int64_t)nb * p.c.bs + (int64_t)oy * p.c.ys + (int64_t)ox * p.c.xs;
             ro.pre = z1 * p.pre.zs1 + z0 * p.pre.zs0 + (int64_t)nb * p.pre.bs + (int64_t)oy * p.pre.ys +
                      (int64_t)ox * p.pre.xs;
@@ -258,11 +283,8 @@
 #pragma unroll
     for (int i = 0; i < A_ITERS; ++i) {
         const int m = m0 + am + i * A_MSTEP;
-        if (m < M) {
-            const int nb = m / HoWo;
-            const int rem = m - nb * HoWo;
-            const int oy = rem / p.Wo;
-            const int ox = rem - oy * p.Wo;
+        int nb, oy, ox;
+        if (decode_row(p, m, M, HoWo, nb, oy, ox)) {
             a_rowbase[i] = (int64_t)nb * p.a_bs;
             a_iy0[i] = oy * p.sy;
             a_ix0[i] = ox * p.sx;
@@ -418,8 +440,9 @@
     const int li = lane & 31;
     const int lh = lane >> 5;
 
-    const int nwg = MT * NT;
+    const int nwg = live_workgroups<BM>(p, MT, NT);
     int bid = blockIdx.x;
+    if (bid >= nwg) return;
     {
         const int xcd = bid & 7, q = nwg >> 3, r = nwg & 7;
         bid = (xcd < r ? xcd * (q + 1) : r * (q + 1) + (xcd - r) * q) + (bid >> 3);
@@ -437,11 +460,8 @@
         const int t = idx / BM, r = idx - t * BM;
         const int m = m0 + r;
         int off = -1;
-        if (m < M) {
-            const int nb = m / HoWo;
-            const int rem = m - nb * HoWo;
-            const int oy = rem / p.Wo;
-            const int ox = rem - oy * p.Wo;
+        int nb, oy, ox;
+        if (decode_row(p, m, M, HoWo, nb, oy, ox)) {
             int iy = oy * p.sy + p.tap_dy[t];
             int ix = ox * p.sx + p.tap_dx[t];
             bool ok = true;
diff --git a/manga_image_translator_amd/csrc/conv_gemm_split.h b/manga_image_translator_amd/csrc/conv_gemm_split.h
--- a/manga_image_translator_amd/csrc/conv_gemm_split.h
+++ b/manga_image_translator_amd/csrc/conv_gemm_split.h
@@ -46,7 +46,8 @@
     const int li = lane & 31;
     const int lh = lane >> 5;
 
-    const int nwg = MT * NT;
+    const int nwg = live_workgroups<BM>(p, MT, NT);
+    if ((int)blockIdx.x >= nwg) return;
     int cur_tile;
     {
         const int v = blockIdx.x, xcd = v & 7, q = nwg >> 3, r = nwg & 7;
@@ -84,11 +85,8 @@
             const int tp = idx / BM, r = idx - tp * BM;
             const int m = m0 + r;
             int off = -1;
-            if (m < M) {
-                const int nb = m / HoWo;
-                const int rem = m - nb * HoWo;
-                const int oy = rem / p.Wo;
-                const int ox = rem - oy * p.Wo;
+            int nb, oy, ox;
+            if (decode_row(p, m, M, HoWo, nb, oy, ox)) {
                 int iy = oy * p.sy + p.tap_dy[tp];
                 int ix = ox * p.sx + p.tap_dx[tp];
                 bool ok = true;
diff --git a/manga_image_translator_amd/csrc/conv_small_cout.hip b/manga_image_translator_amd/csrc/conv_small_cout.hip
--- a/manga_image_translator_amd/csrc/conv_small_cout.hip
+++ b/manga_image_translator_amd/csrc/conv_small_cout.hip
@@ -2,6 +2,7 @@
 #include <hip/hip_runtime.h>
 #include <stdint.h>
 #include <stdlib.h>
+#include <vector>
 #include "../../include/mit_hip.h"
 #include "common.h"
 
@@ -20,19 +21,33 @@
     }
 }
 
+template <int TH_, int TW_>
+__device__ __forceinline__ bool tile_live(const uint8_t *__restrict__ cells, const int b, const int y0, const int x0, const int H, const int W) {
+    if (cells == nullptr) return true;
+    const int ch = (H + 7) >> 3, cw = (W + 31) >> 5, cy0 = y0 >> 3, cx0 = x0 >> 5;
+    bool live = false;
+#pragma unroll
+    for (int dy = 0; dy < TH_ / 8; ++dy)
+#pragma unroll
+        for (int dx = 0; dx < TW_ / 32; ++dx)
+            if (cy0 + dy < ch && cx0 + dx < cw) live = live || cells[((int64_t)b * ch + cy0 + dy) * cw + cx0 + dx] != 0;
+    return live;
+}
+
 template <int K>
 __global__ __launch_bounds__(256) void conv_small_cout_kernel(const float *__restrict__ in, int64_t in_pix, const f32x4 *__restrict__ w4,
                                                                const float *__restrict__ bias, float *__restrict__ out,
                                                                int64_t out_pix, int H, int W, int Cin, int Cout, int reflect,
-                                                               int act, float alpha) {
+                                                               int act, float alpha, const uint8_t *__restrict__ cells) {
     constexpr int R = K / 2;
     constexpr int HW_ = TW + 2 * R, HH_ = TH + 2 * R;
     __shared__ f32x4 tile[CCH / 4][HH_][HW_];
     const int tx = threadIdx.x & (TW - 1), ty = threadIdx.x / TW;
     const int x0 = blockIdx.x * TW, y0 = blockIdx.y * TH, b = blockIdx.z;
+    const bool live = tile_live<TH, TW>(cells, b, y0, x0, H, W);
     const float *ib = in + (int64_t)b * H * W * in_pix;
     f32x4 acc = {0.f, 0.f, 0.f, 0.f};
-    for (int c0 = 0; c0 < Cin; c0 += CCH) {
+    for (int c0 = 0; c0 < (live ? Cin : 0); c0 += CCH) {
         __syncthreads();
         for (int i = threadIdx.x; i < (CCH / 4) * HH_ * HW_; i += 256) {
             const int q = i % (CCH / 4);
@@ -73,9 +88,11 @@
         }
     }
     const int x = x0 + tx, y = y0 + ty;
-    if (x < W && y < H) {
+    if (x < W && y < H && live) {
         float *o = out + (((int64_t)b * H + y) * W + x) * out_pix;
-        for (int n = 0; n < Cout; ++n) o[n] = act_fn(acc[n] + (bias ? bias[n] : 0.f), act, alpha);
+#pragma unroll
+        for (int n = 0; n < 4; ++n)
+            if (n < Cout) o[n] = act_fn(acc[n] + (bias ? bias[n] : 0.f), act, alpha);
     }
 }
 
@@ -88,7 +105,7 @@
                                                                 const f32x2 *__restrict__ wq ,
                                                                 const float *__restrict__ bias, float *__restrict__ out,
                                                                 int64_t out_pix, int H, int W, int Cin, int Cout, int reflect,
-                                                                int act, float alpha) {
+                                                                int act, float alpha, const uint8_t *__restrict__ cells) {
     constexpr int R = K / 2;
     constexpr int TR = TH3 + 2 * R;
     constexpr int HW_ = TW3 + 2 * R;
@@ -96,6 +113,7 @@
     __shared__ f32x4 tile[TR][HW_];
     const int tx = threadIdx.x & 31, ty = threadIdx.x >> 5;
     const int x0 = blockIdx.x * TW3, y0 = blockIdx.y * TH3, b = blockIdx.z;
+    if (!tile_live<TH3, TW3>(cells, b, y0, x0, H, W)) return;
     const float *ib = in + (int64_t)b * H * W * in_pix;
     f32x2 acc[2][2][3];
 #pragma unroll
@@ -185,7 +203,8 @@
 template <int K>
 __global__ __launch_bounds__(256, 4) void conv_small_cout3_dma_kernel(const float *__restrict__ in, int64_t in_plane ,
                                                                       const f32x2 *__restrict__ wq, const float *__restrict__ bias, float *__restrict__ out,
-                                                                      int64_t out_pix, int H, int W, int Cin, int Cout, int act, float alpha, int parity_major) {
+                                                                      int64_t out_pix, int H, int W, int Cin, int Cout, int act, float alpha, int parity_major,
+                                                                      const uint8_t *__restrict__ cells) {
     constexpr int R = K / 2;
     constexpr int TR = TH3 + 2 * R, HW_ = TW3 + 2 * R, HALF = HW_ / 2;
     constexpr int CELLS = TR * HW_, PIECES = (CELLS + 63) / 64, PPW = (PIECES + 3) / 4, BUF_CELLS = PPW * 4 * 64;
@@ -193,6 +212,7 @@
     const int tx = threadIdx.x & 31, ty = threadIdx.x >> 5;
     const int lane = threadIdx.x & 63, wave = __builtin_amdgcn_readfirstlane(threadIdx.x >> 6);
     const int x0 = blockIdx.x * TW3, y0 = blockIdx.y * TH3, b = blockIdx.z;
+    if (!tile_live<TH3, TW3>(cells, b, y0, x0, H, W)) return;
     int src_off[PPW];
 #pragma unroll
     for (int j = 0; j < PPW; ++j) {
@@ -267,7 +287,7 @@
 
 extern "C" int mit_conv_small_cout(const float *in_dev, int64_t in_pixstride, int64_t in_planestride, const float *w4_dev, const float *w_pairs_dev, const float *bias_dev,
                                    float *out_dev, int64_t out_pixstride, int B, int H, int W, int Cin, int Cout, int k,
-                                   int pad_mode, int act, float act_alpha, void *stream) {
+                                   int pad_mode, int act, float act_alpha, const uint8_t *live_cells, void *stream) {
     if (!in_dev || !w4_dev || !out_dev) return mit_set_error("mit_conv_small_cout: null pointer");
     if (Cout < 1 || Cout > 4) return mit_set_error("mit_conv_small_cout: 1 <= Cout <= 4 required (got %d)", Cout);
     if (Cin <= 0 || (Cin % CCH)) return mit_set_error("mit_conv_small_cout: Cin must be a multiple of %d (got %d)", CCH, Cin);
@@ -287,35 +307,53 @@
     hipStream_t s = reinterpret_cast<hipStream_t>(stream);
     const f32x4 *w4 = reinterpret_cast<const f32x4 *>(w4_dev);
     const int refl = pad_mode == MIT_PAD_REFLECT;
+    double live_px = (double)B * H * W;
+    if (live_cells && mit_probe_on()) {
+        const bool packed = Cout <= 3 && w_pairs_dev;
+        const int th = packed ? TH3 : TH, tw = packed ? TW3 : TW, ch = mit_div_up(H, 8), cw = mit_div_up(W, 32);
+        std::vector<uint8_t> host((size_t)B * ch * cw);
+        MIT_CHECK_HIP(hipStreamSynchronize(s));
+        MIT_CHECK_HIP(hipMemcpy(host.data(), live_cells, host.size(), hipMemcpyDeviceToHost));
+        int64_t tiles = 0;
+        for (int b = 0; b < B; ++b)
+            for (int y0 = 0; y0 < H; y0 += th)
+                for (int x0 = 0; x0 < W; x0 += tw) {
+                    bool live = false;
+                    for (int cy = y0 / 8; cy < ch && cy < (y0 + th) / 8; ++cy)
+                        for (int cx = x0 / 32; cx < cw && cx < (x0 + tw) / 32; ++cx) live = live || host[((size_t)b * ch + cy) * cw + cx] != 0;
+                    tiles += live;
+                }
+        live_px = (double)tiles * th * tw;
+    }
     MitProbeScope probe(Cout <= 3 && w_pairs_dev ? (k == 7 ? "conv_small_cout3_kernel<7>" : k == 5 ? "conv_small_cout3_kernel<5>" : "conv_small_cout3_kernel<3>")
-                                                                    : (k == 7 ? "conv_small_cout_kernel<7>" : k == 5 ? "conv_small_cout_kernel<5>" : "conv_small_cout_kernel<3>"), s, 4.0 * (double)B * H * W * (Cin + Cout), 2.0 * k * k * (double)Cin * Cout * (double)B * H * W);
+                                                                    : (k == 7 ? "conv_small_cout_kernel<7>" : k == 5 ? "conv_small_cout_kernel<5>" : "conv_small_cout_kernel<3>"), s, 4.0 * live_px * (Cin + Cout), 2.0 * k * k * (double)Cin * Cout * live_px);
     if (Cout <= 3 && w_pairs_dev) {
         dim3 grid3(mit_div_up(W, TW3), mit_div_up(H, TH3), B);
         const f32x2 *wp = reinterpret_cast<const f32x2 *>(w_pairs_dev);
         if (Cin & 3) return mit_set_error("mit_conv_small_cout: Cin %% 4");
         if (planes4) {
             switch (k) {
-                case 3: hipLaunchKernelGGL(conv_small_cout3_dma_kernel<3>, grid3, block, 0, s, in_dev, in_planestride, wp, bias_dev, out_dev, out_pixstride, H, W, Cin, Cout, act, act_alpha, parity_major); break;
-                case 5: hipLaunchKernelGGL(conv_small_cout3_dma_kernel<5>, grid3, block, 0, s, in_dev, in_planestride, wp, bias_dev, out_dev, out_pixstride, H, W, Cin, Cout, act, act_alpha, parity_major); break;
-                case 7: hipLaunchKernelGGL(conv_small_cout3_dma_kernel<7>, grid3, block, 0, s, in_dev, in_planestride, wp, bias_dev, out_dev, out_pixstride, H, W, Cin, Cout, act, act_alpha, parity_major); break;
+                case 3: hipLaunchKernelGGL(conv_small_cout3_dma_kernel<3>, grid3, block, 0, s, in_dev, in_planestride, wp, bias_dev, out_dev, out_pixstride, H, W, Cin, Cout, act, act_alpha, parity_major, live_cells); break;
+                case 5: hipLaunchKernelGGL(conv_small_cout3_dma_kernel<5>, grid3, block, 0, s, in_dev, in_planestride, wp, bias_dev, out_dev, out_pixstride, H, W, Cin, Cout, act, act_alpha, parity_major, live_cells); break;
+                case 7: hipLaunchKernelGGL(conv_small_cout3_dma_kernel<7>, grid3, block, 0, s, in_dev, in_planestride, wp, bias_dev, out_dev, out_pixstride, H, W, Cin, Cout, act, act_alpha, parity_major, live_cells); break;
                 default: return mit_set_error("mit_conv_small_cout: k must be 3, 5 or 7 (got %d)", k);
             }
             MIT_CHECK_LAUNCH("mit_conv_small_cout");
             return 0;
         }
         switch (k) {
-            case 3: hipLaunchKernelGGL(conv_small_cout3_kernel<3>, grid3, block, 0, s, in_dev, in_pixstride, in_planestride, wp, bias_dev, out_dev, out_pixstride, H, W, Cin, Cout, refl, act, act_alpha); break;
-            case 5: hipLaunchKernelGGL(conv_small_cout3_kernel<5>, grid3, block, 0, s, in_dev, in_pixstride, in_planestride, wp, bias_dev, out_dev, out_pixstride, H, W, Cin, Cout, refl, act, act_alpha); break;
-            case 7: hipLaunchKernelGGL(conv_small_cout3_kernel<7>, grid3, block, 0, s, in_dev, in_pixstride, in_planestride, wp, bias_dev, out_dev, out_pixstride, H, W, Cin, Cout, refl, act, act_alpha); break;
+            case 3: hipLaunchKernelGGL(conv_small_cout3_kernel<3>, grid3, block, 0, s, in_dev, in_pixstride, in_planestride, wp, bias_dev, out_dev, out_pixstride, H, W, Cin, Cout, refl, act, act_alpha, live_cells); break;
+            case 5: hipLaunchKernelGGL(conv_small_cout3_kernel<5>, grid3, block, 0, s, in_dev, in_pixstride, in_planestride, wp, bias_dev, out_dev, out_pixstride, H, W, Cin, Cout, refl, act, act_alpha, live_cells); break;
+            case 7: hipLaunchKernelGGL(conv_small_cout3_kernel<7>, grid3, block, 0, s, in_dev, in_pixstride, in_planestride, wp, bias_dev, out_dev, out_pixstride, H, W, Cin, Cout, refl, act, act_alpha, live_cells); break;
             default: return mit_set_error("mit_conv_small_cout: k must be 3, 5 or 7 (got %d)", k);
         }
         MIT_CHECK_LAUNCH("mit_conv_small_cout");
         return 0;
     }
     switch (k) {
-        case 3: hipLaunchKernelGGL(conv_small_cout_kernel<3>, grid, block, 0, s, in_dev, in_pixstride, w4, bias_dev, out_dev, out_pixstride, H, W, Cin, Cout, refl, act, act_alpha); break;
-        case 5: hipLaunchKernelGGL(conv_small_cout_kernel<5>, grid, block, 0, s, in_dev, in_pixstride, w4, bias_dev, out_dev, out_pixstride, H, W, Cin, Cout, refl, act, act_alpha); break;
-        case 7: hipLaunchKernelGGL(conv_small_cout_kernel<7>, grid, block, 0, s, in_dev, in_pixstride, w4, bias_dev, out_dev, out_pixstride, H, W, Cin, Cout, refl, act, act_alpha); break;
+        case 3: hipLaunchKernelGGL(conv_small_cout_kernel<3>, grid, block, 0, s, in_dev, in_pixstride, w4, bias_dev, out_dev, out_pixstride, H, W, Cin, Cout, refl, act, act_alpha, live_cells); break;
+        case 5: hipLaunchKernelGGL(conv_small_cout_kernel<5>, grid, block, 0, s, in_dev, in_pixstride, w4, bias_dev, out_dev, out_pixstride, H, W, Cin, Cout, refl, act, act_alpha, live_cells); break;
+        case 7: hipLaunchKernelGGL(conv_small_cout_kernel<7>, grid, block, 0, s, in_dev, in_pixstride, w4, bias_dev, out_dev, out_pixstride, H, W, Cin, Cout, refl, act, act_alpha, live_cells); break;
         default: return mit_set_error("mit_conv_small_cout: k must be 3, 5 or 7 (got %d)", k);
     }
     MIT_CHECK_LAUNCH("mit_conv_small_cout");
diff --git a/manga_image_translator_amd/csrc/lama_tail_need.hip b/manga_image_translator_amd/csrc/lama_tail_need.hip
--- /dev/null
+++ b/manga_image_translator_amd/csrc/lama_tail_need.hip
@@ -0,0 +1,172 @@
+#include <hip/hip_runtime.h>
+#include <stdint.h>
+#include "../../include/mit_hip.h"
+#include "common.h"
+
+namespace {
+
+__global__ __launch_bounds__(256) void need_rows_kernel(const uint8_t *__restrict__ mask, uint8_t *__restrict__ T, const int W, const int w2, const int64_t total) {
+    const int64_t idx = (int64_t)blockIdx.x * 256 + threadIdx.x;
+    if (idx >= total) return;
+    const int j = (int)(idx % w2);
+    const uint8_t *row = mask + (idx / w2) * W;
+    const int x0 = 2 * j - 3 < 0 ? 0 : 2 * j - 3, x1 = 2 * j + 4 >= W ? W - 1 : 2 * j + 4;
+    bool any = false;
+    for (int x = x0; x <= x1; ++x) any = any || row[x] >= 127;
+    T[idx] = any;
+}
+
+template <int R, int RX, bool POOLX>
+__global__ __launch_bounds__(256) void need_pool_kernel(const uint8_t *__restrict__ src, uint8_t *__restrict__ dst, const int hs, const int ws, const int hd,
+                                                        const int wd, const int64_t total) {
+    const int64_t idx = (int64_t)blockIdx.x * 256 + threadIdx.x;
+    if (idx >= total) return;
+    const int j = (int)(idx % wd), i = (int)((idx / wd) % hd);
+    const uint8_t *img = src + (idx / ((int64_t)wd * hd)) * hs * ws;
+    const int y0 = 2 * i - R < 0 ? 0 : 2 * i - R, y1 = 2 * i + 1 + R >= hs ? hs - 1 : 2 * i + 1 + R;
+    const int x0 = !POOLX ? j : (2 * j - RX < 0 ? 0 : 2 * j - RX), x1 = !POOLX ? j : (2 * j + 1 + RX >= ws ? ws - 1 : 2 * j + 1 + RX);
+    bool any = false;
+    for (int y = y0; y <= y1; ++y)
+        for (int x = x0; x <= x1; ++x) any = any || img[(int64_t)y * ws + x] != 0;
+    dst[idx] = any;
+}
+
+__global__ __launch_bounds__(256) void need_cells_kernel(const uint8_t *__restrict__ mask, uint8_t *__restrict__ cells, const int H, const int W, const int ch,
+                                                         const int cw, const int64_t total) {
+    const int64_t idx = (int64_t)blockIdx.x * 256 + threadIdx.x;
+    if (idx >= total) return;
+    const int cx = (int)(idx % cw), cy = (int)((idx / cw) % ch);
+    const uint8_t *img = mask + (idx / ((int64_t)cw * ch)) * H * W;
+    const int y1 = cy * 8 + 8 > H ? H : cy * 8 + 8, x1 = cx * 32 + 32 > W ? W : cx * 32 + 32;
+    bool any = false;
+    for (int y = cy * 8; y < y1; ++y)
+        for (int x = cx * 32; x < x1; ++x) any = any || img[(int64_t)y * W + x] >= 127;
+    cells[idx] = any;
+}
+
+struct NeedLevels {
+    const uint8_t *S[3];
+    uint8_t *flag[3];
+    int h[3], w[3];
+    int32_t *list[3], *start[3], *count[3];
+};
+
+__global__ __launch_bounds__(256) void need_flags_kernel(const NeedLevels lv, const int B) {
+    const int l = blockIdx.y, h = lv.h[l], w = lv.w[l];
+    const int bw = (w + 7) >> 3, bpi = ((h + 7) >> 3) * bw;
+    const int idx = blockIdx.x * 256 + threadIdx.x;
+    if (idx >= B * bpi) return;
+    const int b = idx / bpi, t = idx - b * bpi;
+    const int by = t / bw, bx = t - by * bw;
+    const uint8_t *img = lv.S[l] + (int64_t)b * h * w;
+    const int y1 = by * 8 + 8 > h ? h : by * 8 + 8, x1 = bx * 8 + 8 > w ? w : bx * 8 + 8;
+    bool any = false;
+    for (int y = by * 8; y < y1; ++y)
+        for (int x = bx * 8; x < x1; ++x) any = any || img[y * w + x] != 0;
+    lv.flag[l][idx] = any;
+}
+
+__global__ __launch_bounds__(256) void need_count_kernel(const NeedLevels lv) {
+    const int l = blockIdx.y, b = blockIdx.x;
+    const int bpi = ((lv.h[l] + 7) >> 3) * ((lv.w[l] + 7) >> 3);
+    const uint8_t *flag = lv.flag[l] + (int64_t)b * bpi;
+    int n = 0;
+    for (int t = threadIdx.x; t < bpi; t += 256) n += flag[t];
+    __shared__ int wsum[4];
+    for (int o = 32; o > 0; o >>= 1) n += __shfl_xor(n, o);
+    if ((threadIdx.x & 63) == 0) wsum[threadIdx.x >> 6] = n;
+    __syncthreads();
+    if (threadIdx.x == 0) lv.count[l][b] = wsum[0] + wsum[1] + wsum[2] + wsum[3];
+}
+
+__global__ __launch_bounds__(256) void need_fill_kernel(const NeedLevels lv, const int B) {
+    const int l = blockIdx.y, b = blockIdx.x;
+    const int bpi = ((lv.h[l] + 7) >> 3) * ((lv.w[l] + 7) >> 3);
+    const uint8_t *flag = lv.flag[l] + (int64_t)b * bpi;
+    int base = 0;
+    for (int i = 0; i < b; ++i) base += lv.count[l][i];
+    if (threadIdx.x == 0) {
+        lv.start[l][b] = base;
+        if (b == B - 1) lv.start[l][B] = base + lv.count[l][b];
+    }
+    __shared__ int wsum[4];
+    const int lane = threadIdx.x & 63, wave = threadIdx.x >> 6;
+    int32_t *out = lv.list[l];
+    for (int t0 = 0; t0 < bpi; t0 += 256) {
+        const int t = t0 + threadIdx.x;
+        const bool live = t < bpi && flag[t] != 0;
+        const unsigned long long bal = __ballot(live);
+        const int before = __popcll(bal & ((1ull << lane) - 1ull));
+        __syncthreads();
+        if (lane == 0) wsum[wave] = __popcll(bal);
+        __syncthreads();
+        int pos = base + before;
+        for (int i = 0; i < wave; ++i) pos += wsum[i];
+        if (live) out[pos] = b * bpi + t;
+        base += wsum[0] + wsum[1] + wsum[2] + wsum[3];
+    }
+}
+
+struct Sizes {
+    int64_t T, S[3], F[3], counts, total;
+};
+Sizes sizes_of(int B, int H, int W) {
+    Sizes z;
+    z.counts = ((int64_t)3 * B * 4 + 15) / 16 * 16;
+    z.T = ((int64_t)B * H * (W / 2) + 15) / 16 * 16;
+    z.total = z.counts + z.T;
+    for (int l = 0; l < 3; ++l) {
+        const int h = H >> (3 - l), w = W >> (3 - l);
+        z.S[l] = ((int64_t)B * h * w + 15) / 16 * 16;
+        z.F[l] = ((int64_t)B * ((h + 7) / 8) * ((w + 7) / 8) + 15) / 16 * 16;
+        z.total += z.S[l] + z.F[l];
+    }
+    return z;
+}
+
+}
+
+extern "C" int64_t mit_lama_tail_need_work(int B, int H, int W) {
+    if (B <= 0 || H <= 0 || W <= 0) return 0;
+    return sizes_of(B, H, W).total;
+}
+
+extern "C" int mit_lama_tail_need(const uint8_t *mask_dev, int B, int H, int W, uint8_t *cells_dev, int32_t *list0_dev, int32_t *start0_dev,
+                                  int32_t *list1_dev, int32_t *start1_dev, int32_t *list2_dev, int32_t *start2_dev, uint8_t *work_dev, void *stream) {
+    if (!mask_dev || !cells_dev || !list0_dev || !start0_dev || !list1_dev || !start1_dev || !list2_dev || !start2_dev || !work_dev)
+        return mit_set_error("mit_lama_tail_need: null pointer");
+    if (B <= 0 || B > 65535 || H <= 0 || W <= 0 || (H & 7) || (W & 7)) return mit_set_error("mit_lama_tail_need: need 0 < B < 65536 and H, W multiples of 8 (got %d x %d x %d)", B, H, W);
+    if ((int64_t)B * H * W > 0x7fffffffLL) return mit_set_error("mit_lama_tail_need: B * H * W must stay below 2^31");
+    if (reinterpret_cast<uintptr_t>(work_dev) & 15) return mit_set_error("mit_lama_tail_need: work must be 16-byte aligned");
+    hipStream_t s = reinterpret_cast<hipStream_t>(stream);
+    const Sizes z = sizes_of(B, H, W);
+    int32_t *counts = reinterpret_cast<int32_t *>(work_dev);
+    uint8_t *T = work_dev + z.counts;
+    uint8_t *S0 = T + z.T, *S1 = S0 + z.S[0], *S2 = S1 + z.S[1];
+    uint8_t *F0 = S2 + z.S[2], *F1 = F0 + z.F[0], *F2 = F1 + z.F[1];
+    auto blocks = [](int64_t n) { return dim3((unsigned)((n + 255) / 256)); };
+    const int ch = H / 8, cw = (W + 31) / 32;
+    int64_t n = (int64_t)B * ch * cw;
+    hipLaunchKernelGGL(need_cells_kernel, blocks(n), dim3(256), 0, s, mask_dev, cells_dev, H, W, ch, cw, n);
+    n = (int64_t)B * H * (W / 2);
+    hipLaunchKernelGGL(need_rows_kernel, blocks(n), dim3(256), 0, s, mask_dev, T, W, W / 2, n);
+    n = (int64_t)B * (H / 2) * (W / 2);
+    hipLaunchKernelGGL((need_pool_kernel<3, 0, false>), blocks(n), dim3(256), 0, s, T, S2, H, W / 2, H / 2, W / 2, n);
+    n = (int64_t)B * (H / 4) * (W / 4);
+    hipLaunchKernelGGL((need_pool_kernel<1, 1, true>), blocks(n), dim3(256), 0, s, S2, S1, H / 2, W / 2, H / 4, W / 4, n);
+    n = (int64_t)B * (H / 8) * (W / 8);
+    hipLaunchKernelGGL((need_pool_kernel<1, 1, true>), blocks(n), dim3(256), 0, s, S1, S0, H / 4, W / 4, H / 8, W / 8, n);
+    NeedLevels lv;
+    const uint8_t *Sl[3] = {S0, S1, S2};
+    uint8_t *Fl[3] = {F0, F1, F2};
+    int32_t *lists[3] = {list0_dev, list1_dev, list2_dev}, *starts[3] = {start0_dev, start1_dev, start2_dev};
+    for (int l = 0; l < 3; ++l) {
+        lv.S[l] = Sl[l], lv.flag[l] = Fl[l], lv.h[l] = H >> (3 - l), lv.w[l] = W >> (3 - l);
+        lv.list[l] = lists[l], lv.start[l] = starts[l], lv.count[l] = counts + l * B;
+    }
+    hipLaunchKernelGGL(need_flags_kernel, dim3((unsigned)((z.F[2] + 255) / 256), 3), dim3(256), 0, s, lv, B);
+    hipLaunchKernelGGL(need_count_kernel, dim3(B, 3), dim3(256), 0, s, lv);
+    hipLaunchKernelGGL(need_fill_kernel, dim3(B, 3), dim3(256), 0, s, lv, B);
+    MIT_CHECK_LAUNCH("mit_lama_tail_need");
+    return 0;
+}
diff --git a/manga_image_translator_amd/lama.py b/manga_image_translator_amd/lama.py
--- a/manga_image_translator_amd/lama.py
+++ b/manga_image_translator_amd/lama.py
@@ -164,12 +164,45 @@
         return self._direct
 
 
+def _dilate(m: np.ndarray, r: int) -> np.ndarray:
+    p = np.pad(m, ((0, 0), (r, r), (r, r)))
+    H, W = m.shape[1:]
+    return np.any([p[:, dy:dy + H, dx:dx + W] for dy in range(2 * r + 1) for dx in range(2 * r + 1)], axis=0)
+
+
+def _pool2(m: np.ndarray) -> np.ndarray:
+    m = np.pad(m, ((0, 0), (0, m.shape[1] % 2), (0, m.shape[2] % 2)))
+    return m[:, 0::2, 0::2] | m[:, 0::2, 1::2] | m[:, 1::2, 0::2] | m[:, 1::2, 1::2]
+
+
+def _blocks_any(m: np.ndarray, bh: int, bw: int) -> np.ndarray:
+    B, H, W = m.shape
+    p = np.pad(m, ((0, 0), (0, -H % bh), (0, -W % bw)))
+    return p.reshape(B, p.shape[1] // bh, bh, p.shape[2] // bw, bw).any(axis=(2, 4))
+
+
+def tail_need_numpy(mask: np.ndarray) -> dict:
+    need = np.asarray(mask) >= 127
+    out = dict(cells=_blocks_any(need, 8, 32).astype(np.uint8), sub={}, need_out={}, blocks={}, list={}, start={})
+    need = _dilate(need, 3)
+    for L in (2, 1, 0):
+        out["need_out"][L] = need
+        sub = _pool2(need)
+        blk = _blocks_any(sub, 8, 8)
+        out["sub"][L], out["blocks"][L] = sub, blk
+        out["list"][L] = np.flatnonzero(blk.reshape(-1)).astype(np.int32)
+        out["start"][L] = np.concatenate([[0], np.cumsum(blk.reshape(blk.shape[0], -1).sum(1))]).astype(np.int32)
+        need = _dilate(sub, 1)
+    return out
+
+
 class LamaEngine(ops.Engine):
 
     def __init__(self, gen_sd: Dict[str, torch.Tensor], mpe_sd: Optional[Dict[str, torch.Tensor]] = None,
                  n_blocks: int = 9, device="cuda", fft_h: bool = True, winograd: bool = True, fft_w: bool = True,
-                 row_packed_stem: bool = True):
+                 row_packed_stem: bool = True, masked_tail: bool = True):
         super().__init__(device)
+        self.masked_tail = masked_tail
         self.winograd = winograd
         self.fft_h = fft_h
         self.fft_w = fft_w
@@ -368,6 +401,21 @@
         ffc.st_out(t2, out=out[..., LOCAL_C:], pre=P, post=res_g, nprod=nprod)
         self._dbg_put("s2_out_global", out[..., LOCAL_C:])
 
+    def _tail_need(self, mask_u8: torch.Tensor):
+        B, H, W = mask_u8.shape
+        lib = _lib.load()
+        cells = self._buf("need_cells", B, H // 8, (W + 31) // 32, dtype=torch.uint8)
+        work = self._buf("need_work", int(lib.mit_lama_tail_need_work(B, H, W)), dtype=torch.uint8)
+        live = []
+        for L in range(3):
+            h, w = H >> (3 - L), W >> (3 - L)
+            live.append((self._buf(f"need_list{L}", B * ((h + 7) // 8) * ((w + 7) // 8), dtype=torch.int32),
+                         self._buf(f"need_start{L}", B + 1, dtype=torch.int32)))
+        _lib.check(lib.mit_lama_tail_need(mask_u8.data_ptr(), B, H, W, cells.data_ptr(), live[0][0].data_ptr(), live[0][1].data_ptr(),
+                                          live[1][0].data_ptr(), live[1][1].data_ptr(), live[2][0].data_ptr(), live[2][1].data_ptr(),
+                                          work.data_ptr(), C.c_void_p(ops.current_stream())), "mit_lama_tail_need")
+        return live, cells
+
     @torch.no_grad()
     def forward(self, img_u8: torch.Tensor, mask_u8: torch.Tensor, taps: Optional[dict] = None, composite: bool = True,
                 precision: str = "fp32") -> torch.Tensor:
@@ -435,21 +483,25 @@
             self._ffc(c2, T, X, X, nprod)
             if taps is not None:
                 taps[f"block{i}"] = X.clone()
+        live = [None, None, None]
+        cells = None
+        if self.masked_tail and composite and taps is None and self._dbg is None:
+            live, cells = self._tail_need(mask_u8)
         u1 = self._buf("d2", B, H // 4, W // 4, 256)
-        self.ups[0](X, out=u1, nprod=nprod)
+        self.ups[0](X, out=u1, nprod=nprod, live=live[0])
         u2 = self._buf("d1", B, H // 2, W // 2, 128)
-        self.ups[1](u1, out=u2, nprod=nprod)
+        self.ups[1](u1, out=u2, nprod=nprod, live=live[1])
         pred = self._buf("pred", B, H, W, 3)
         if self.planar_tail:
             P = self.planar_tail
             pm = P == 4 and H % 2 == 0 and W % 2 == 0
             u3 = self._buf("full64", 64 // P, B, H, W, P)
-            self.ups[2](u2, out=u3, planes=64 // P, parity_major=pm, nprod=nprod)
-            self.out_conv(u3, out=pred, parity_major=pm)
+            self.ups[2](u2, out=u3, planes=64 // P, parity_major=pm, nprod=nprod, live=live[2])
+            self.out_conv(u3, out=pred, parity_major=pm, cells=cells)
         else:
             u3 = self._buf("full64", B, H, W, 64)
-            self.ups[2](u2, out=u3, nprod=nprod)
-            self.out_conv(u3, out=pred)
+            self.ups[2](u2, out=u3, nprod=nprod, live=live[2])
+            self.out_conv(u3, out=pred, cells=cells)
         if taps is not None:
             taps["pred"] = pred.clone()
         out = torch.empty(B, H, W, 3, dtype=torch.uint8, device=self.device)
diff --git a/manga_image_translator_amd/lib.py b/manga_image_translator_amd/lib.py
--- a/manga_image_translator_amd/lib.py
+++ b/manga_image_translator_amd/lib.py
@@ -4,7 +4,7 @@
 from pathlib import Path
 
 MIT_MAX_TAPS = 64
-MIT_ABI_VERSION = 20
+MIT_ABI_VERSION = 21
 
 ACT_NONE, ACT_RELU, ACT_LEAKY, ACT_SILU, ACT_SIGMOID, ACT_GELU = range(6)
 ACT_POST_FIRST = 0x100
@@ -69,7 +69,9 @@
         ("lut2", C.c_void_p),
         ("lut_ld", C.c_int64),
         ("nprod", C.c_int32),
-        ("_pad1", C.c_int32),
+        ("live_img0", C.c_int32),
+        ("live_blocks", C.c_void_p),
+        ("live_start", C.c_void_p),
     ]
 
 
@@ -187,7 +189,9 @@
     "mit_gemm_mode_get": (C.c_int, []),
     "mit_gemm_split_min_tiles": (C.c_int64, [C.c_int64]),
     "mit_conv_small_cout": (C.c_int, [C.c_void_p, C.c_int64, C.c_int64, C.c_void_p, C.c_void_p, C.c_void_p, C.c_void_p, C.c_int64, C.c_int, C.c_int,
-                                      C.c_int, C.c_int, C.c_int, C.c_int, C.c_int, C.c_int, C.c_float, C.c_void_p]),
+                                      C.c_int, C.c_int, C.c_int, C.c_int, C.c_int, C.c_int, C.c_float, C.c_void_p, C.c_void_p]),
+    "mit_lama_tail_need_work": (C.c_int64, [C.c_int, C.c_int, C.c_int]),
+    "mit_lama_tail_need": (C.c_int, [C.c_void_p, C.c_int, C.c_int, C.c_int] + [C.c_void_p] * 9),
     "mit_convnext_mlp_supported": (C.c_int, [C.c_int]),
     "mit_convnext_mlp": (C.c_int, [C.c_void_p, C.c_int64, C.c_int, C.c_int, C.c_void_p, C.c_void_p, C.c_void_p, C.c_int64, C.c_void_p, C.c_void_p,
                                    C.c_void_p, C.c_int64, C.c_void_p, C.c_int64, C.c_void_p]),
diff --git a/manga_image_translator_amd/ops.py b/manga_image_translator_amd/ops.py
--- a/manga_image_translator_amd/ops.py
+++ b/manga_image_translator_amd/ops.py
@@ -121,7 +121,8 @@
                    pre: Optional[MitTensorMap] = None, post: Optional[MitTensorMap] = None,
                    scale: Optional[torch.Tensor] = None, bias: Optional[torch.Tensor] = None, act: int = ACT_NONE,
                    alpha: float = 0.0, Z: int = 1, zdiv: int = 1, a_zs: Tuple[int, int] = (0, 0),
-                   w_zs: Tuple[int, int] = (0, 0), nprod: int = 0) -> MitConvGemm:
+                   w_zs: Tuple[int, int] = (0, 0), nprod: int = 0,
+                   live: Optional[Tuple[torch.Tensor, torch.Tensor]] = None) -> MitConvGemm:
     if len(taps) == 0 or len(taps) > MIT_MAX_TAPS:
         raise ValueError(f"ntaps {len(taps)} out of range")
     d = MitConvGemm()
@@ -148,6 +149,11 @@
     d.bias = _ptr(bias)
     d.act, d.act_alpha = act, alpha
     d.nprod = int(nprod)
+    if live is not None:
+        blocks, start = live
+        if blocks.dtype != torch.int32 or start.dtype != torch.int32 or start.numel() < NB + 1:
+            raise ValueError("conv_gemm_desc: live = (int32 block ids, int32 [NB + 1] prefix)")
+        d.live_blocks, d.live_start = blocks.data_ptr(), start.data_ptr()
     return d
 
 
@@ -489,7 +495,7 @@
         self.w_pairs = (w4.reshape(kh * kw, Cin // 4, 4, 4).permute(0, 1, 3, 2).to(device).contiguous() if Cout <= 3 else None)
         self.bias = None if bias is None else bias.detach().to(torch.float32).to(device).contiguous()
 
-    def __call__(self, x: torch.Tensor, out: torch.Tensor, parity_major: bool = False) -> torch.Tensor:
+    def __call__(self, x: torch.Tensor, out: torch.Tensor, parity_major: bool = False, cells: Optional[torch.Tensor] = None) -> torch.Tensor:
         plane = 0
         if x.dim() == 5:
             pc = x.shape[4]
@@ -512,9 +518,11 @@
         lib = _lib.load()
         if parity_major and not plane:
             raise ValueError("ConvSmallCout: parity_major without planar input")
+        if cells is not None and (cells.dtype != torch.uint8 or tuple(cells.shape) != (B, (H + 7) // 8, (W + 31) // 32) or not cells.is_contiguous()):
+            raise ValueError(f"ConvSmallCout: cells must be contiguous u8 [{B}, {(H + 7) // 8}, {(W + 31) // 32}]")
         _lib.check(lib.mit_conv_small_cout(x.data_ptr(), x.stride(2), -plane if parity_major else plane, self.w4.data_ptr(), _ptr(self.w_pairs), _ptr(self.bias), out.data_ptr(),
                                            out.stride(2), B, H, W, self.Cin, self.Cout, self.k, self.pad_mode, self.act,
-                                           self.alpha, C.c_void_p(current_stream())), "mit_conv_small_cout")
+                                           self.alpha, _ptr(cells), C.c_void_p(current_stream())), "mit_conv_small_cout")
         return out
 
 
@@ -600,7 +608,8 @@
     def out_hw(self, H: int, W: int) -> Tuple[int, int]:
         return ((H - 1) * self.s - 2 * self.p + self.k[0] + self.op, (W - 1) * self.s - 2 * self.p + self.k[1] + self.op)
 
-    def descs(self, x: torch.Tensor, out: torch.Tensor, planes: int = 0, parity_major: bool = False, nprod: int = 0) -> List[MitConvGemm]:
+    def descs(self, x: torch.Tensor, out: torch.Tensor, planes: int = 0, parity_major: bool = False, nprod: int = 0,
+              live: Optional[Tuple[torch.Tensor, torch.Tensor]] = None) -> List[MitConvGemm]:
         split = nhi = 0
         if planes:
             if out.dim() != 5 or out.shape[0] != planes or out.shape[4] * planes != self.Cout or not out.is_contiguous():
@@ -620,6 +629,8 @@
         ds = []
         for py, px, pk in self.sub:
             ov = out[:, py::self.s, px::self.s]
+            if live is not None and (ov.shape[1] * self.s != Ho or ov.shape[2] * self.s != Wo):
+                raise ValueError("ConvTranspose2d: a live-block list needs an output size that is a multiple of the stride")
             if ov.shape[1] == 0 or ov.shape[2] == 0:
                 continue
             if nprod:
@@ -632,15 +643,15 @@
                 a=x, NB=B, Hi=H, Wi=W, Cin=self.Cin, a_strides=(x.stride(0), x.stride(1), x.stride(2)),
                 Ho=ov.shape[1], Wo=ov.shape[2], sy=1, sx=1, taps=pk.taps, pad_mode=PAD_ZERO, w=pk.w, ldw=pk.Np,
                 Kw=pk.Kp, Nw=pk.Np, N=self.Cout, c=tensor_map(ov, nsplit=split, nhi=nhi), scale=self.scale, bias=self.bias, act=self.act,
-                alpha=self.alpha, nprod=nprod))
+                alpha=self.alpha, nprod=nprod, live=live))
         return ds
 
     def __call__(self, x: torch.Tensor, out: Optional[torch.Tensor] = None, cfg: int = -1, planes: int = 0, parity_major: bool = False,
-                 nprod: int = 0) -> torch.Tensor:
+                 nprod: int = 0, live: Optional[Tuple[torch.Tensor, torch.Tensor]] = None) -> torch.Tensor:
         if out is None:
             Ho, Wo = self.out_hw(x.shape[1], x.shape[2])
             out = (torch.empty(planes, x.shape[0], Ho, Wo, self.Cout // planes, dtype=torch.float32, device=x.device) if planes else
                    torch.empty(x.shape[0], Ho, Wo, self.Cout, dtype=torch.float32, device=x.device))
-        for d in self.descs(x, out, planes, parity_major, nprod):
+        for d in self.descs(x, out, planes, parity_major, nprod, live):
             launch_conv_gemm(d, cfg)
         return out
```

After: 46.86 (median of 6 runs). 1.06x the previous value.
